# Dreycey/PhageFilter

Measured on AMD Instinct MI355X. Metric: reads/sec classified (150 bp, 1024-leaf SBT) at 1/2/4/8 MI355X; bit-exact vs CPU, higher is better.
Workload: dtype u64

## Files before the change

### include/pfq.h

```cpp
#ifndef PFQ_H
#define PFQ_H

#include <stdint.h>

#ifdef __cplusplus
extern "C" {
#endif

typedef enum pfq_status {
    PFQ_OK = 0,
    PFQ_ERR_ARG = -1,
    PFQ_ERR_IO = -2,
    PFQ_ERR_FORMAT = -3,
    PFQ_ERR_UNSUPPORTED = -4,
    PFQ_ERR_DEVICE = -5,
    PFQ_ERR_STATE = -6
} pfq_status;

typedef struct pfq_tree pfq_tree;

typedef struct pfq_info {
    uint64_t kmer_size;
    uint64_t nbits;
    uint32_t num_hashes;
// ... 157 lines not shown
                     float threshold, uint32_t flags, pfq_segments *out);
int pfq_query_frames_device(pfq_tree *tree, const uint8_t *d_seq, const uint64_t *d_offsets, uint64_t n_seqs, uint64_t total_bytes,
                            uint32_t frame, uint32_t step, float threshold, uint32_t flags, void *stream, pfq_segments *out);

#define PFQ_TEXT_FASTA 0
#define PFQ_TEXT_FASTQ 1
#define PFQ_TEXT_FINAL 1u
#define PFQ_TEXT_WANT_RECORDS 2u
enum { PFQ_TEXT_END = 0, PFQ_TEXT_LIMIT = 1, PFQ_TEXT_MORE = 2, PFQ_TEXT_SLOW = 3 };
typedef struct pfq_text {
    uint64_t n_records;
    uint64_t consumed;
    uint64_t n_bases;
    uint32_t stop;
    const uint64_t *rec_begin;
} pfq_text;
int pfq_text_parse(pfq_tree *tree, const uint8_t *text, uint64_t len, uint64_t limit, int format, uint32_t flags, pfq_text *out);
int pfq_text_query(pfq_tree *tree, float threshold, uint32_t flags, pfq_hits *hits);
int pfq_debug_text_csr(pfq_tree *tree, uint8_t *seq_out, uint64_t *off_out);

#define PFQ_PREP_PAIRED 1u
#define PFQ_PREP_WANT_READS 2u
enum { PFQ_PREP_KEPT = 0, PFQ_PREP_SHORT = 1, PFQ_PREP_N = 2, PFQ_PREP_COMPLEXITY = 3, PFQ_PREP_MATE = 4 };
typedef struct pfq_prep_params {
    uint32_t trim_quality;
    uint32_t trim_window;
    uint32_t poly_x;
    uint32_t min_length;
    uint32_t max_n;
    uint32_t min_complexity;
    uint32_t flags;
} pfq_prep_params;
typedef struct pfq_prep {
    uint64_t n_reads, n_kept, bases_in, bases_kept, n_trimmed;
    uint64_t n_reason[5];
    const uint32_t *begin, *len, *reason;
    const uint32_t *kept;
} pfq_prep;
int pfq_prep_reads(pfq_tree *tree, const uint8_t *seq, const uint8_t *qual, const uint64_t *offsets, const uint8_t *has_qual,
                   uint64_t n_reads, const pfq_prep_params *params, pfq_prep *out);
int pfq_prep_query(pfq_tree *tree, float threshold, uint32_t flags, pfq_hits *hits);
int pfq_debug_prep_csr(pfq_tree *tree, uint8_t *seq_out, uint64_t *off_out);
int pfq_debug_last_prep(pfq_tree *tree, double *ms);

typedef struct pfq_similarity {
    uint64_t n_a, n_b;
    const uint32_t *shared_bits;
    const uint64_t *bits_a, *bits_b;
    const double *kmers_a, *kmers_b;
    const double *shared_kmers, *jaccard;
} pfq_similarity;
int pfq_tree_similarity(pfq_tree *a, const uint32_t *leaves_a, uint64_t n_a,
                        pfq_tree *b, const uint32_t *leaves_b, uint64_t n_b, pfq_similarity *out);

int pfq_tree_recluster(pfq_tree *src, pfq_tree **out);
typedef struct pfq_merge {
    uint32_t node, left, right, round, n_leaves, pad_;
    uint64_t score_sum, pairs;
} pfq_merge;
int pfq_tree_merges(pfq_tree *tree, const pfq_merge **merges, uint64_t *n, uint32_t *rounds);

int pfq_leaf_counts(pfq_tree *tree, const char *const **tax_ids, const uint64_t **counts, uint64_t *n_leaves);
int pfq_save_leaf_counts(pfq_tree *tree, const char *csv_path);

int pfq_leaf_counts_export(pfq_tree *tree, uint64_t *d_dst, void *stream);
int pfq_leaf_counts_import(pfq_tree *tree, const uint64_t *d_src, void *stream);
int pfq_leaf_counts_reset(pfq_tree *tree);
int pfq_leaf_counts_export_delta(pfq_tree *tree, uint64_t *d_dst, void *stream);
int pfq_leaf_counts_import_delta(pfq_tree *tree, const uint64_t *d_src, void *stream);

int pfq_device_count(int *n);

int pfq_trees_allreduce_counts(pfq_tree *const *trees, uint32_t n_trees);
uint32_t pfq_last_allreduce_ranks(void);


int pfq_set_option(pfq_tree *tree, const char *name, const char *value);

#define PFQ_CAPACITY_N 12
int pfq_debug_last_capacity(pfq_tree *tree, uint64_t *out, uint64_t n);

int pfq_tile_lists_info(pfq_tree *tree, uint64_t out[4]);
int pfq_debug_tile_list(pfq_tree *tree, uint64_t col, uint64_t tile, uint32_t *out, uint64_t n);


typedef struct pfq_stats {
    uint64_t n_reads, n_candidates, n_hits, n_allhit_reads;
    uint64_t algorithmic_bytes;
    uint32_t path;
    uint32_t n_slices;
    uint32_t tile_mode;
    uint32_t n_fallback_pairs;
    uint64_t n_chunks, tile_entries;
    uint32_t tile_passes_launched, tile_passes_needed;
    uint32_t leaf_groups;
    uint32_t coarse_cols;
    uint32_t coarse_probes;
    uint32_t tile_bin_build;
    uint64_t group_reads;
    uint32_t pair_stage;
} pfq_stats;
int pfq_last_stats(pfq_tree *tree, pfq_stats *out);
int pfq_set_path(pfq_tree *tree, int path);

typedef struct pfq_profile {
    uint64_t calls;
    double classify_ms;
    double bucket_ms;
    double bin_ms;
    double test_ms;
    double verify_ms;
    double finalize_ms;
} pfq_profile;
int pfq_profile_begin(pfq_tree *tree, uint32_t max_calls);
int pfq_profile_end(pfq_tree *tree, pfq_profile *out);

int pfq_debug_kmer_indices(pfq_tree *tree, const uint8_t *seq, uint64_t len, uint64_t *out_idx, uint64_t *n_kmers);
int pfq_debug_last_similarity(pfq_tree *a, double *kernel_ms, uint32_t *slices);
int pfq_debug_last_recluster(pfq_tree *src, double *ms, uint64_t *nn_bytes, uint32_t *rounds);
int pfq_debug_node_filter(pfq_tree *tree, uint64_t node, uint64_t *out_words, uint64_t n_words);

int pfq_synth_genomes_device(uint8_t *d_out, uint64_t n_genomes, uint64_t genome_len, uint64_t seed_base,
                             void *stream);
int pfq_synth_reads_device(uint8_t *d_out, uint64_t first_read, uint64_t n_reads, uint64_t read_len,
                           const uint8_t *d_genomes, uint64_t genome_len, uint64_t n_genomes, uint64_t seed,
                           void *stream);

int pfq_host_alloc(uint64_t bytes, void **out);
int pfq_host_free(void *p);

const char *pfq_last_error(void);
const char *pfq_version(void);

#ifdef __cplusplus
}
#endif
#endif
```

### phagefilter_amd/_ffi.py

```python
from __future__ import annotations

import ctypes as C
import os

_HERE = os.path.dirname(os.path.abspath(__file__))
LIB_PATH = os.environ.get("PFQ_LIBPFQ") or os.path.join(_HERE, "libpfq.so")

SYMBOLS = [
    "pfq_tree_open", "pfq_tree_open_subtree", "pfq_db_shard_count", "pfq_tree_create", "pfq_tree_insert", "pfq_tree_build_balanced", "pfq_tree_build_balanced_device",
    "pfq_tree_build_balanced_subtree_device", "pfq_trees_allreduce_counts", "pfq_last_allreduce_ranks", "pfq_device_count", "pfq_set_option", "pfq_tree_save", "pfq_tree_info",
    "pfq_tree_prune", "pfq_tree_close", "pfq_query_batch", "pfq_query_batch_device", "pfq_last_hit_scores", "pfq_leaf_counts",
    "pfq_tree_clades", "pfq_clade_counts", "pfq_last_lca",
    "pfq_tree_set_taxonomy", "pfq_tree_taxa", "pfq_taxon_counts", "pfq_last_taxa", "pfq_last_best_rows", "pfq_db_leaf_ids", "pfq_taxonomy_read", "pfq_taxonomy_nodes",
    "pfq_abundance_estimate", "pfq_abundance_reset", "pfq_abundance_absorb",
    "pfq_coverage_get", "pfq_coverage_reset", "pfq_coverage_absorb",
    "pfq_tree_set_sweep", "pfq_sweep_get", "pfq_sweep_reset", "pfq_sweep_absorb",
    "pfq_query_frames", "pfq_query_frames_device",
    "pfq_text_parse", "pfq_text_query", "pfq_debug_text_csr",
    "pfq_prep_reads", "pfq_prep_query", "pfq_debug_prep_csr", "pfq_debug_last_prep",
    "pfq_tree_similarity", "pfq_tree_recluster", "pfq_tree_merges",
    "pfq_save_leaf_counts", "pfq_leaf_counts_export", "pfq_leaf_counts_import", "pfq_leaf_counts_reset",
    "pfq_leaf_counts_export_delta", "pfq_leaf_counts_import_delta",
    "pfq_last_stats", "pfq_set_path", "pfq_profile_begin", "pfq_profile_end", "pfq_debug_kmer_indices", "pfq_debug_node_filter", "pfq_debug_last_capacity", "pfq_debug_last_similarity", "pfq_debug_last_recluster",
    "pfq_tile_lists_info", "pfq_debug_tile_list",
    "pfq_synth_genomes_device",
    "pfq_synth_reads_device", "pfq_host_alloc", "pfq_host_free", "pfq_last_error", "pfq_version",
]


class PfqError(RuntimeError):
    def __init__(self, code: int, msg: str):
        super().__init__(f"libpfq error {code}: {msg}")
        self.code = code


class Info(C.Structure):
    _fields_ = [("kmer_size", C.c_uint64), ("nbits", C.c_uint64), ("num_hashes", C.c_uint32),
                ("largest_expected_genome", C.c_uint32), ("false_pos_rate", C.c_float),
                ("superset_verified", C.c_uint32), ("seed1", C.c_uint64), ("seed2", C.c_uint64),
                ("n_nodes", C.c_uint64), ("n_leaves", C.c_uint64), ("n_filters", C.c_uint64),
                ("device_bytes", C.c_uint64), ("shard_first_leaf", C.c_uint64), ("tree_leaves", C.c_uint64)]


class Hits(C.Structure):
    _fields_ = [("n_reads", C.c_uint64), ("offsets", C.POINTER(C.c_uint64)), ("leaves", C.POINTER(C.c_uint32))]


class Stats(C.Structure):
    _fields_ = [("n_reads", C.c_uint64), ("n_candidates", C.c_uint64), ("n_hits", C.c_uint64),
                ("n_allhit_reads", C.c_uint64), ("algorithmic_bytes", C.c_uint64), ("path", C.c_uint32),
                ("n_slices", C.c_uint32), ("tile_mode", C.c_uint32), ("n_fallback_pairs", C.c_uint32),
                ("n_chunks", C.c_uint64), ("tile_entries", C.c_uint64), ("tile_passes_launched", C.c_uint32),
                ("tile_passes_needed", C.c_uint32), ("leaf_groups", C.c_uint32), ("coarse_cols", C.c_uint32),
                ("coarse_probes", C.c_uint32), ("tile_bin_build", C.c_uint32), ("group_reads", C.c_uint64),
                ("pair_stage", C.c_uint32)]


class Profile(C.Structure):
    _fields_ = [("calls", C.c_uint64), ("classify_ms", C.c_double), ("bucket_ms", C.c_double), ("bin_ms", C.c_double),
                ("test_ms", C.c_double), ("verify_ms", C.c_double), ("finalize_ms", C.c_double)]


class Clade(C.Structure):
    _fields_ = [("parent", C.c_uint32), ("depth", C.c_uint32), ("first_leaf", C.c_uint32), ("n_leaves", C.c_uint32),
                ("name", C.c_char_p)]


class Taxon(C.Structure):
    _fields_ = [("parent", C.c_uint32), ("depth", C.c_uint32), ("first_rank", C.c_uint32), ("n_leaves", C.c_uint32),
                ("leaf", C.c_uint32), ("name", C.c_char_p)]


class TaxonomyFile(C.Structure):
    _fields_ = [("n_taxa", C.c_uint64), ("taxon_parent", C.POINTER(C.c_uint32)), ("taxon_names", C.POINTER(C.c_char_p)),
                ("n_leaves", C.c_uint64), ("leaf_taxon", C.POINTER(C.c_uint32)), ("lines_considered", C.c_uint64),
                ("lines_other", C.c_uint64), ("leaves_without_line", C.c_uint64)]


class Abundance(C.Structure):
    _fields_ = [("n_leaves", C.c_uint64), ("mass", C.POINTER(C.c_uint64)), ("unique", C.POINTER(C.c_uint64)),
                ("n_units", C.c_uint64), ("n_unhit", C.c_uint64), ("n_unique", C.c_uint64), ("n_ambiguous", C.c_uint64),
                ("n_all_leaves", C.c_uint64), ("n_entries", C.c_uint64), ("last_delta", C.c_uint64),
                ("iterations", C.c_uint32), ("converged", C.c_uint32)]


class Coverage(C.Structure):
    _fields_ = [("n_leaves", C.c_uint64), ("n_units", C.c_uint64), ("precision", C.c_uint32),
                ("registers", C.POINTER(C.c_uint8)),
                ("units", C.POINTER(C.c_uint64)), ("matched", C.POINTER(C.c_uint64)), ("filter_bits", C.POINTER(C.c_uint64)),
                ("distinct", C.POINTER(C.c_double)), ("genome_kmers", C.POINTER(C.c_double))]


class Sweep(C.Structure):
    _fields_ = [("n_thresholds", C.c_uint32), ("thresholds", C.POINTER(C.c_float)), ("n_leaves", C.c_uint64), ("n_units", C.c_uint64),
                ("leaf_units", C.POINTER(C.c_uint64)), ("leaf_unique", C.POINTER(C.c_uint64)),
                ("units_hit", C.POINTER(C.c_uint64)), ("units_unique", C.POINTER(C.c_uint64)), ("entries", C.POINTER(C.c_uint64)),
                ("genomes_hit", C.POINTER(C.c_uint64))]


class Segment(C.Structure):
    _fields_ = [(f, C.c_uint32) for f in ("leaf", "first_frame", "n_frames", "begin", "end", "match_begin", "match_end", "kmers",
                                          "matched", "longest_run")]


class Segments(C.Structure):
    _fields_ = [("n_seqs", C.c_uint64), ("n_frames", C.c_uint64), ("offsets", C.POINTER(C.c_uint64)), ("seg", C.POINTER(Segment))]


class Text(C.Structure):
    _fields_ = [("n_records", C.c_uint64), ("consumed", C.c_uint64), ("n_bases", C.c_uint64), ("stop", C.c_uint32),
                ("rec_begin", C.POINTER(C.c_uint64))]


class PrepParams(C.Structure):
    _fields_ = [(f, C.c_uint32) for f in ("trim_quality", "trim_window", "poly_x", "min_length", "max_n", "min_complexity", "flags")]


class Prep(C.Structure):
    _fields_ = [("n_reads", C.c_uint64), ("n_kept", C.c_uint64), ("bases_in", C.c_uint64), ("bases_kept", C.c_uint64),
                ("n_trimmed", C.c_uint64), ("n_reason", C.c_uint64 * 5),
                ("begin", C.POINTER(C.c_uint32)), ("len", C.POINTER(C.c_uint32)), ("reason", C.POINTER(C.c_uint32)),
                ("kept", C.POINTER(C.c_uint32))]


class Similarity(C.Structure):
    _fields_ = [("n_a", C.c_uint64), ("n_b", C.c_uint64), ("shared_bits", C.POINTER(C.c_uint32)),
                ("bits_a", C.POINTER(C.c_uint64)), ("bits_b", C.POINTER(C.c_uint64)),
                ("kmers_a", C.POINTER(C.c_double)), ("kmers_b", C.POINTER(C.c_double)),
                ("shared_kmers", C.POINTER(C.c_double)), ("jaccard", C.POINTER(C.c_double))]


class Merge(C.Structure):
    _fields_ = [("node", C.c_uint32), ("left", C.c_uint32), ("right", C.c_uint32), ("round", C.c_uint32), ("n_leaves", C.c_uint32),
                ("pad_", C.c_uint32), ("score_sum", C.c_uint64), ("pairs", C.c_uint64)]


WANT_HITS = 1
WANT_SCORES = 2
# ... 31 lines not shown
    L.pfq_version.restype = C.c_char_p
    L.pfq_tree_open.argtypes = [C.c_char_p, C.c_int, C.POINTER(vp)]
    L.pfq_tree_open_subtree.argtypes = [C.c_char_p, C.c_int, C.c_uint64, C.c_uint64, C.POINTER(vp)]
    L.pfq_db_shard_count.argtypes = [C.c_char_p, C.c_uint64, u64p]
    L.pfq_tree_build_balanced.argtypes = [vp, vp, C.c_uint64, C.POINTER(C.c_char_p), C.c_uint64, C.c_uint64,
                                          C.c_uint32, C.c_uint64, C.c_uint64, C.c_float, C.c_uint32, C.c_int,
                                          C.POINTER(vp)]
    L.pfq_tree_build_balanced_device.argtypes = [vp, C.c_uint64, C.c_uint64, C.POINTER(C.c_char_p), C.c_uint64,
                                                 C.c_uint64, C.c_uint32, C.c_uint64, C.c_uint64, C.c_float, C.c_uint32,
                                                 C.c_int, C.POINTER(vp)]
    L.pfq_tree_build_balanced_subtree_device.argtypes = [vp, C.c_uint64, C.c_uint64, C.POINTER(C.c_char_p), C.c_uint64,
                                                         C.c_uint64, C.c_uint32, C.c_uint64, C.c_uint64, C.c_float, C.c_uint32,
                                                         C.c_uint64, C.c_uint64, C.c_int, C.POINTER(vp)]
    L.pfq_trees_allreduce_counts.argtypes = [C.POINTER(vp), C.c_uint32]
    L.pfq_last_allreduce_ranks.restype = C.c_uint32
    L.pfq_set_option.argtypes = [vp, C.c_char_p, C.c_char_p]
    L.pfq_tree_create.argtypes = [C.c_uint64, C.c_float, C.c_uint32, C.c_uint64, C.c_uint64, C.c_uint64, C.c_int, C.POINTER(vp)]
    L.pfq_tree_insert.argtypes = [vp, vp, C.c_uint64, C.c_char_p, C.c_char_p]
    L.pfq_host_alloc.argtypes = [C.c_uint64, C.POINTER(vp)]
    L.pfq_host_free.argtypes = [vp]
    L.pfq_tree_save.argtypes = [vp, C.c_char_p]
    L.pfq_tree_info.argtypes = [vp, C.POINTER(Info)]
    L.pfq_tree_prune.argtypes = [vp, C.c_uint64]
    L.pfq_tree_close.argtypes = [vp]
    L.pfq_tree_close.restype = None
    L.pfq_query_batch.argtypes = [vp, vp, vp, C.c_uint64, C.c_float, C.c_uint32, C.POINTER(Hits)]
    L.pfq_query_batch_device.argtypes = [vp, vp, vp, C.c_uint64, C.c_uint64, C.c_float, C.c_uint32, vp, C.POINTER(Hits)]
    L.pfq_last_hit_scores.argtypes = [vp, C.POINTER(C.POINTER(C.c_uint32)), u64p]
    L.pfq_tree_clades.argtypes = [vp, C.POINTER(C.POINTER(Clade)), u64p]
    L.pfq_clade_counts.argtypes = [vp, C.POINTER(u64p), C.POINTER(u64p), u64p]
    L.pfq_last_lca.argtypes = [vp, C.POINTER(C.POINTER(C.c_uint32)), u64p]
    u32p = C.POINTER(C.c_uint32)
    L.pfq_tree_set_taxonomy.argtypes = [vp, C.c_uint64, vp, C.POINTER(C.c_char_p), vp]
    L.pfq_tree_taxa.argtypes = [vp, C.POINTER(C.POINTER(Taxon)), u64p]
    L.pfq_taxon_counts.argtypes = [vp, C.POINTER(u64p), C.POINTER(u64p), C.POINTER(u64p), u64p]
    L.pfq_last_taxa.argtypes = [vp, C.POINTER(u32p), u64p]
    L.pfq_last_best_rows.argtypes = [vp, C.POINTER(Hits)]
    L.pfq_db_leaf_ids.argtypes = [C.c_char_p, C.POINTER(C.POINTER(C.c_char_p)), u64p]
    L.pfq_taxonomy_read.argtypes = [C.c_char_p, C.POINTER(C.c_char_p), C.c_uint64, C.POINTER(TaxonomyFile)]
    L.pfq_taxonomy_nodes.argtypes = [C.c_uint64, C.POINTER(C.c_char_p), C.c_uint64, vp, C.POINTER(C.c_char_p), vp,
                                     C.POINTER(C.POINTER(Taxon)), u64p]
    L.pfq_abundance_estimate.argtypes = [vp, C.c_uint32, C.c_uint64, C.POINTER(Abundance)]
    L.pfq_abundance_reset.argtypes = [vp]
    L.pfq_abundance_absorb.argtypes = [vp, vp]
    L.pfq_coverage_get.argtypes = [vp, C.POINTER(Coverage)]
    L.pfq_coverage_reset.argtypes = [vp]
    L.pfq_coverage_absorb.argtypes = [vp, vp]
    L.pfq_tree_set_sweep.argtypes = [vp, C.POINTER(C.c_float), C.c_uint32]
    L.pfq_sweep_get.argtypes = [vp, C.POINTER(Sweep)]
    L.pfq_sweep_reset.argtypes = [vp]
    L.pfq_sweep_absorb.argtypes = [vp, vp]
    L.pfq_query_frames.argtypes = [vp, vp, vp, C.c_uint64, C.c_uint32, C.c_uint32, C.c_float, C.c_uint32, C.POINTER(Segments)]
    L.pfq_query_frames_device.argtypes = [vp, vp, vp, C.c_uint64, C.c_uint64, C.c_uint32, C.c_uint32, C.c_float, C.c_uint32, vp,
                                          C.POINTER(Segments)]
    L.pfq_text_parse.argtypes = [vp, vp, C.c_uint64, C.c_uint64, C.c_int, C.c_uint32, C.POINTER(Text)]
    L.pfq_text_query.argtypes = [vp, C.c_float, C.c_uint32, C.POINTER(Hits)]
    L.pfq_debug_text_csr.argtypes = [vp, vp, vp]
    L.pfq_prep_reads.argtypes = [vp, vp, vp, vp, vp, C.c_uint64, C.POINTER(PrepParams), C.POINTER(Prep)]
    L.pfq_prep_query.argtypes = [vp, C.c_float, C.c_uint32, C.POINTER(Hits)]
    L.pfq_debug_prep_csr.argtypes = [vp, vp, vp]
    L.pfq_debug_last_prep.argtypes = [vp, C.POINTER(C.c_double)]
    L.pfq_tree_similarity.argtypes = [vp, vp, C.c_uint64, vp, vp, C.c_uint64, C.POINTER(Similarity)]
    L.pfq_debug_last_similarity.argtypes = [vp, C.POINTER(C.c_double), C.POINTER(C.c_uint32)]
    L.pfq_tree_recluster.argtypes = [vp, C.POINTER(vp)]
    L.pfq_tree_merges.argtypes = [vp, C.POINTER(C.POINTER(Merge)), u64p, C.POINTER(C.c_uint32)]
    L.pfq_debug_last_recluster.argtypes = [vp, C.POINTER(C.c_double), u64p, C.POINTER(C.c_uint32)]
    L.pfq_leaf_counts.argtypes = [vp, C.POINTER(C.POINTER(C.c_char_p)), C.POINTER(u64p), u64p]
    L.pfq_save_leaf_counts.argtypes = [vp, C.c_char_p]
    L.pfq_leaf_counts_export.argtypes = [vp, vp, vp]
    L.pfq_leaf_counts_import.argtypes = [vp, vp, vp]
    L.pfq_leaf_counts_export_delta.argtypes = [vp, vp, vp]
    L.pfq_leaf_counts_import_delta.argtypes = [vp, vp, vp]
    L.pfq_leaf_counts_reset.argtypes = [vp]
    L.pfq_last_stats.argtypes = [vp, C.POINTER(Stats)]
    L.pfq_set_path.argtypes = [vp, C.c_int]
    L.pfq_profile_begin.argtypes = [vp, C.c_uint32]
    L.pfq_profile_end.argtypes = [vp, C.POINTER(Profile)]
    L.pfq_debug_kmer_indices.argtypes = [vp, vp, C.c_uint64, vp, u64p]
    L.pfq_debug_node_filter.argtypes = [vp, C.c_uint64, vp, C.c_uint64]
    L.pfq_debug_last_capacity.argtypes = [vp, vp, C.c_uint64]
    if hasattr(L, "pfq_tile_lists_info"):
        L.pfq_tile_lists_info.argtypes = [vp, vp]
        L.pfq_debug_tile_list.argtypes = [vp, C.c_uint64, C.c_uint64, vp, C.c_uint64]
    L.pfq_synth_genomes_device.argtypes = [vp, C.c_uint64, C.c_uint64, C.c_uint64, vp]
    L.pfq_synth_reads_device.argtypes = [vp, C.c_uint64, C.c_uint64, C.c_uint64, vp, C.c_uint64, C.c_uint64,
                                         C.c_uint64, vp]
    _lib = L
    return L


def check(rc: int) -> None:
    if rc != 0:
        raise PfqError(rc, lib().pfq_last_error().decode(errors="replace"))


def source_stamp() -> str:
    import glob
    import hashlib
    h = hashlib.sha256()
    csrc = os.path.join(_HERE, "csrc")
    files = sorted(glob.glob(os.path.join(csrc, "*.hip")) + glob.glob(os.path.join(csrc, "*.cpp")) +
                   glob.glob(os.path.join(csrc, "*.h")) + [os.path.join(os.path.dirname(_HERE), "include", "pfq.h")])
    for f in files:
        h.update(os.path.basename(f).encode())
        with open(f, "rb") as fh:
            h.update(fh.read())
    return h.hexdigest()[:16]
```

### phagefilter_amd/csrc/pfq_host.cpp

```cpp
#include <hip/hip_runtime.h>
#include <rccl/rccl.h>
#include <dlfcn.h>

#include <algorithm>
#include <thread>
#include <mutex>
#include <atomic>
#include <cerrno>
#include <cmath>
#include <cstdio>
#include <cstring>
#include <fstream>
#include <map>
#include <memory>
#include <string>
#include <unordered_set>
#include <vector>

#include "../../include/pfq.h"
#include "pfq_kernels.h"
#include "pfq_taxonomy.h"

namespace {

thread_local std::string g_err;
int fail(int code, const std::string &msg) {
    g_err = msg;
    return code;
}
#define HIP_TRY(expr)                                                                                        \
    do {                                                                                                     \
        hipError_t e_ = (expr);                                                                              \
        if (e_ != hipSuccess)                                                                                \
            return fail(PFQ_ERR_DEVICE, std::string(#expr) + ": " + hipGetErrorString(e_) + " (" __FILE__ ":" + \
                                            std::to_string(__LINE__) + ")");                                 \
    } while (0)
#define PFQ_TRY(expr)              \
    do {                           \
        int rc_ = (expr);          \
        if (rc_ != PFQ_OK) return rc_; \
    } while (0)

struct Node {
    int32_t left = -1, right = -1, parent = -1;
    std::string bf_path;
    bool has_tax = false;
    std::string tax_id;
    uint64_t mapped_reads = 0;
    uint64_t base_reads = 0;
    uint32_t filter = 0;
    uint32_t depth = 0;
    bool is_leaf() const { return left < 0 && right < 0; }
};

template <typename T>
struct DevBuf {
    T *p = nullptr;
    size_t n = 0;
    ~DevBuf() { release(); }
    void release() {
        if (p) (void)hipFree(p);
        p = nullptr;
        n = 0;
    }
    hipError_t ensure(size_t want) {
        if (want <= n) return hipSuccess;
        release();
        hipError_t e = hipMalloc(&p, want * sizeof(T));
        if (e == hipSuccess) n = want;
        return e;
    }
    size_t bytes() const { return n * sizeof(T); }
};
template <typename T>
struct HostBuf {
    T *p = nullptr;
    size_t cap = 0;
    ~HostBuf() { if (p) (void)hipHostFree(p); }
    hipError_t ensure(size_t want) {
        const size_t bytes = want * sizeof(T), grown = bytes + bytes / 4 + 4096;
        if (bytes <= cap) return hipSuccess;
        if (p) (void)hipHostFree(p);
        p = nullptr;
        cap = 0;
        hipError_t e = hipHostMalloc((void **)&p, grown, hipHostMallocDefault);
        if (e == hipSuccess) cap = grown;
        return e;
    }
};

struct Knobs {
    long long record_gb = -1, tile_gb = -1, tile_entries = -1, slice_kb = -1;
    long long verify_blocks = -1, verify_chunk = -1, verify_sub = -1, verify_threads = -1, bin_blocks = -1, test_blocks = -1;
    long long tile = -1, tile_counts = -1, no_tail_batch = -1, split_records = -1, bin_narrow = -1, bin_wide = -1, bin_debug = -1, block = -1, batch_emit = -1;
    long long coarse = -1, coarse_cols = -1, coarse_probes = -1, group_log2 = -1, screen_recs = -1, coarse_min_leaves = -1, greedy_host = -1;
    long long pair_slots = -1, guard_slots = -1, miss_words = -1, kmiss_bytes = -1, hit_slots = -1;
    long long abund_slots = -1, abund_blocks = -1, abund_lds = -1;
    long long cover_p = -1, cover_blocks = -1;
    long long frame_piece = -1;
    long long sim_slices = -1, sim_naive = -1, sim_time = -1;
    long long cluster_time = -1;
    long long text_tile = -1;
    long long sweep_lds = -1;
    long long tile_lists = -1;
    long long tile_stream = -1;
};
struct KnobName {
    const char *name;
    long long Knobs::*field;
};
const KnobName KNOBS[] = {
    {"PFQ_RECORD_GB", &Knobs::record_gb},       {"PFQ_TILE_GB", &Knobs::tile_gb},
    {"PFQ_TILE_ENTRIES", &Knobs::tile_entries}, {"PFQ_SLICE_KB", &Knobs::slice_kb},
    {"PFQ_VERIFY_BLOCKS", &Knobs::verify_blocks}, {"PFQ_VERIFY_CHUNK", &Knobs::verify_chunk},
    {"PFQ_VERIFY_SUB", &Knobs::verify_sub},     {"PFQ_VERIFY_THREADS", &Knobs::verify_threads},
    {"PFQ_BIN_BLOCKS", &Knobs::bin_blocks},     {"PFQ_TEST_BLOCKS", &Knobs::test_blocks},
    {"PFQ_TILE", &Knobs::tile},                 {"PFQ_TILE_COUNTS", &Knobs::tile_counts},
    {"PFQ_NO_TAIL_BATCH", &Knobs::no_tail_batch}, {"PFQ_BIN_NARROW", &Knobs::bin_narrow},
    {"PFQ_BIN_WIDE", &Knobs::bin_wide},         {"PFQ_SPLIT_RECORDS", &Knobs::split_records},
#ifdef PFQ_EXPERIMENTS
    {"PFQ_BIN_DEBUG", &Knobs::bin_debug},
#endif
    {"PFQ_BLOCK", &Knobs::block},               {"PFQ_BATCH_EMIT", &Knobs::batch_emit},
    {"PFQ_COARSE", &Knobs::coarse},             {"PFQ_COARSE_COLS", &Knobs::coarse_cols},
    {"PFQ_COARSE_PROBES", &Knobs::coarse_probes}, {"PFQ_GROUP_LOG2", &Knobs::group_log2},
    {"PFQ_SCREEN_RECS", &Knobs::screen_recs},   {"PFQ_COARSE_MIN_LEAVES", &Knobs::coarse_min_leaves},
    {"PFQ_GREEDY_HOST", &Knobs::greedy_host},
    {"PFQ_PAIR_SLOTS", &Knobs::pair_slots},     {"PFQ_GUARD_SLOTS", &Knobs::guard_slots},
    {"PFQ_MISS_WORDS", &Knobs::miss_words},     {"PFQ_KMISS_BYTES", &Knobs::kmiss_bytes},
    {"PFQ_HIT_SLOTS", &Knobs::hit_slots},
    {"PFQ_ABUND_SLOTS", &Knobs::abund_slots},   {"PFQ_ABUND_BLOCKS", &Knobs::abund_blocks},
    {"PFQ_ABUND_LDS", &Knobs::abund_lds},
    {"PFQ_COVER_P", &Knobs::cover_p},           {"PFQ_COVER_BLOCKS", &Knobs::cover_blocks},
    {"PFQ_FRAME_PIECE", &Knobs::frame_piece},
    {"PFQ_SIM_SLICES", &Knobs::sim_slices},     {"PFQ_SIM_NAIVE", &Knobs::sim_naive},
    {"PFQ_SIM_TIME", &Knobs::sim_time},         {"PFQ_CLUSTER_TIME", &Knobs::cluster_time},
    {"PFQ_TEXT_TILE", &Knobs::text_tile},       {"PFQ_SWEEP_LDS", &Knobs::sweep_lds},
    {"PFQ_TILE_LISTS", &Knobs::tile_lists},     {"PFQ_TILE_STREAM", &Knobs::tile_stream},
};
bool set_knob(Knobs &k, const char *name, const char *value) {
    for (const KnobName &kn : KNOBS)
        if (!strcmp(kn.name, name)) {
            k.*(kn.field) = (value && *value) ? strtoll(value, nullptr, 10) : -1;
            return true;
        }
    return false;
}
Knobs knobs_from_env() {
    Knobs k;
    for (const KnobName &kn : KNOBS)
        if (const char *e = getenv(kn.name)) set_knob(k, kn.name, e);
    return k;
}

}

namespace {
std::atomic<long> g_open_trees{0};
void release_communicators();
}

enum CursorSlot {
    CUR_HIT = 0,
    CUR_PAIR = 1,
    CUR_TILE_ENTRIES = 2,
    CUR_CHUNKS_FLAGGED = 3,
    CUR_LONG = 4,
    CUR_MISS_WORDS = 5,
    CUR_DIRTY = 6,
    CUR_OPEN = 7,
    CUR_GUARD = 8,
    CUR_KMISS = 9,
    CUR_TAIL_SHAPES = 10,
    CUR_TAIL_WORK = 11,
    CUR_TILE_LIST = 12,
    CUR_TILE_DENSE = 13,
    CUR_N = 14,
    CUR_ALLOC = 16,
};
static_assert(CUR_N <= CUR_ALLOC, "an attempt clears CUR_ALLOC slots");
static_assert(CUR_HIT == 0 && CUR_PAIR == 1, "read_hits reads slots 0 and 1 with one 16-byte copy");
static_assert(CUR_TAIL_WORK == CUR_TAIL_SHAPES + 1, "k_tail_records finds its work counter at shapes[2]");
static_assert(CUR_TILE_DENSE == CUR_TILE_LIST + 1, "k_tile_test finds its dense counter at tile_list_stats[1]");
enum HintSlot {
    HINT_PAIRS = 0,
    HINT_TILE_ENTRIES = 1,
    HINT_DIRTY = 2,
    HINT_SORTED = 3,
    HINT_CANDIDATES = 4,
    HINT_PLAN = 5,
    HINT_N = 8,
};
static_assert(CUR_TILE_ENTRIES == CUR_PAIR + 1 && HINT_TILE_ENTRIES == HINT_PAIRS + 1, "one 16-byte copy fills both hints");

struct pfq_tree {
    pfq_tree() { ++g_open_trees; }
    pfq_tree(const pfq_tree &) = delete;
    ~pfq_tree() {
        if (--g_open_trees == 0) release_communicators();
    }
    int device = 0;
    Knobs knobs = knobs_from_env();
    std::vector<Node> nodes;
    int32_t root = -1;
    float false_pos_rate = 0.001f;
    uint32_t largest_expected_genome = 0;
    uint64_t kmer_size = 0, nbits = 0, seed1 = 0, seed2 = 0, n_words = 0;
    uint32_t num_hashes = 0;
    std::vector<std::string> filter_paths;
    std::unordered_set<std::string> path_set;
    std::vector<uint8_t> edge_ok;
    bool superset_all = true;
    uint64_t shard_first_leaf = 0, tree_leaves = 0;
    bool is_shard = false;
    unsigned long long *h_pair_cursor = nullptr;
    hipEvent_t hint_ev = nullptr;
    uint64_t hint_reads = 0, hint_entry_cap = 0, passes_hint = 1;
    double pairs_per_read = 1.0, hits_per_read = 1.0;
    double dirty_frac = 1.0;
    bool hint_counts = false;
    uint32_t last_sub_log2 = 0;
    bool topology_dirty = false;
    uint64_t internal_counter = 0;
    size_t n_rows = 0, row_capacity = 0;
    DevBuf<uint32_t> d_build;
    DevBuf<unsigned long long> d_dist;
    DevBuf<pfq::TopoNode> d_topo;
    DevBuf<int> d_walk;
    bool topo_on_device = false;
    bool topo_pending = false;
    DevBuf<uint8_t> d_gseq[4];
    hipEvent_t gseq_free[4] = {nullptr, nullptr, nullptr, nullptr};
    hipEvent_t gseq_copied[4] = {nullptr, nullptr, nullptr, nullptr};
    uint8_t *h_gseq[4] = {nullptr, nullptr, nullptr, nullptr};
    size_t h_gseq_n[4] = {0, 0, 0, 0};
    uint32_t gseq_next = 0;
    int greedy_blocks = 0;
    uint32_t walk_seq = 0;
    int insert_err = PFQ_OK;
    std::string insert_err_msg;

    pfq::HashParams hp{};
    DevBuf<uint64_t> d_bits;
    bool layout_valid = false;
    std::vector<int32_t> leaves;
    std::vector<uint32_t> col_row;
    std::vector<uint32_t> guard_off, guard_col;
    uint32_t rw = 1, rw_log2 = 0, n_cols = 0;
    uint64_t leaf_cap = 0, guard_cap = 0;
    uint32_t n_groups = 1;
    uint32_t group_log2 = 11;
    uint64_t group_stride = 0;
    bool coarse_valid = false;
    uint32_t coarse_cols = 0, coarse_rw = 0, coarse_rw_log2 = 0;
    double coarse_fill = 0.0;
    DevBuf<uint32_t> d_Sc, d_cgrp, d_glists, d_glong;
    DevBuf<unsigned int> d_gcur;
    uint32_t last_coarse_cols = 0, last_coarse_probes = 0, last_leaf_groups = 0;
    DevBuf<uint32_t> d_S, d_col_row, d_guard_off, d_guard_col;
    DevBuf<uint32_t> d_tile_list_row, d_tile_lists;
    uint32_t tile_list_cols = 0;
    void drop_tile_lists() {
        d_tile_list_row.release();
        d_tile_lists.release();
        tile_list_cols = 0;
    }
    DevBuf<uint32_t> d_owner, d_owner_sorted, d_gfail;
    DevBuf<unsigned long long> d_counts;
    DevBuf<unsigned long long> d_counts_base, d_counts_delta;
    DevBuf<unsigned long long> d_stats, d_cursors;
    unsigned int *cur_lo(CursorSlot s) const { return reinterpret_cast<unsigned int *>(d_cursors.p + s); }
    unsigned int *cur_hi(CursorSlot s) const { return cur_lo(s) + 1; }
    DevBuf<uint32_t> d_entries, d_pair_chunk, d_leaf_chunk0, d_flag_list;
    DevBuf<pfq::ChunkDesc> d_chunks;
    DevBuf<unsigned int> d_gfill, d_binq;
    DevBuf<uint8_t> d_kmiss;
    DevBuf<uint8_t> d_kall;
    DevBuf<uint8_t> d_T, d_failb;
    bool tables_valid = false;
    double cand_per_read = 1.0;
    bool have_cand_hint = false;
    uint32_t last_block_mode = 0;
    DevBuf<uint32_t> d_round_k0, d_n_rounds, d_pair_kpos;
    uint32_t last_tile_mode = 0, last_passes = 1;
    uint32_t last_sort = 0;
    bool last_tile_stream = false;
    uint32_t last_tile_bin = 0;
    DevBuf<uint2> d_hit_pairs, d_pairs, d_sorted;
    DevBuf<uint32_t> d_bucket, d_fail;
    DevBuf<unsigned int> d_queue;
    DevBuf<uint8_t> d_allhit, d_seq, d_seq2;
    DevBuf<uint64_t> d_off2;
    hipStream_t copy_stream = nullptr;
    hipEvent_t in_free[2] = {nullptr, nullptr};
    bool in_used[2] = {false, false};
    int in_slot = 0;
    DevBuf<unsigned long long> d_miss_words;
    DevBuf<uint32_t> d_miss_pos, d_bucket_w;
    DevBuf<uint32_t> d_long;
    DevBuf<uint4> d_recs;
    DevBuf<uint4> d_meta;
    DevBuf<uint64_t> d_off;
    DevBuf<unsigned long long> d_counts_snapshot;
    hipStream_t last_stream = nullptr;
    bool have_last_stream = false;
    hipEvent_t last_done = nullptr;
    int force_path = -1;
    std::vector<hipEvent_t> prof_ev;
    size_t prof_cap = 0, prof_used = 0;
    std::vector<uint8_t> prof_bucketed;
    uint32_t last_path = 0, last_slices = 1;
    uint64_t last_n_reads = 0;
    uint64_t last_pair_cap = 0, last_guard_cap = 0, last_miss_cap = 0, last_kmiss_cap = 0, last_hit_cap0 = 0, last_hit_cursor0 = 0;
    uint64_t last_nb = 0;
    uint32_t last_attempts = 0;
    std::vector<std::string> out_tax;
    std::vector<const char *> out_tax_ptr;
    std::vector<uint64_t> out_counts;
    DevBuf<uint32_t> d_hit_cnt, d_hit_leaves;
    DevBuf<unsigned long long> d_hit_sums, d_hit_off;
    HostBuf<uint64_t> h_hit_off;
    HostBuf<uint32_t> h_hit_leaves;
    DevBuf<uint32_t> d_hit_scores;
    HostBuf<uint32_t> h_hit_scores;
    bool scores_valid = false;
    uint64_t scores_n = 0;
    DevBuf<unsigned long long> d_pair_sink, d_frag_off, d_pair_misc;
    DevBuf<uint32_t> d_frag_leaves, d_pair_long;
    bool lca_valid = false;
    std::vector<pfq_clade> clades;
    std::vector<std::string> clade_names;
    uint32_t top_clade = 0;
    DevBuf<uint32_t> d_leaf_clade, d_gap_min, d_lca, d_lca_long;
    DevBuf<unsigned long long> d_clade_here, d_lca_misc;
    DevBuf<uint2> d_lca_span;
    std::vector<uint64_t> out_here, out_below;
    DevBuf<unsigned long long> d_ab_start, d_ab_unique, d_ab_cur, d_ab_a, d_ab_b, d_ab_delta;
    DevBuf<uint32_t> d_ab_len, d_ab_entries;
    uint64_t ab_rows = 0, ab_entries = 0, ab_units = 0, ab_unhit = 0, ab_unique = 0, ab_all = 0;
    bool ab_incomplete = false;
    std::vector<uint64_t> out_mass, out_unique;
    DevBuf<uint8_t> d_cov_regs;
    DevBuf<unsigned long long> d_cov_cnt;
    uint32_t cov_p = 0;
    uint64_t cov_units = 0;
    bool cov_bits_valid = false;
    std::vector<uint64_t> cov_bits, out_cov_units, out_cov_matched;
    std::vector<uint8_t> out_cov_regs;
    std::vector<double> out_cov_distinct, out_cov_genome;
    DevBuf<uint32_t> d_fr_cnt, d_fr_def, d_fr_seq, d_fr_start, d_fr_segseq, d_fr_queue;
    DevBuf<unsigned long long> d_fr_seq0, d_fr_defoff, d_fr_sums, d_fr_segpos, d_fr_seqseg, d_fr_pieceoff, d_fr_misc;
    DevBuf<uint64_t> d_fr_foff;
    DevBuf<uint8_t> d_fr_bytes;
    DevBuf<pfq::Segment> d_fr_segs;
    DevBuf<pfq::FramePart> d_fr_parts;
    HostBuf<uint64_t> h_fr_off;
    HostBuf<pfq_segment> h_fr_segs;
    std::vector<uint32_t> out_sim_shared;
    std::vector<uint64_t> out_sim_bits_a, out_sim_bits_b;
    std::vector<double> out_sim_kmers_a, out_sim_kmers_b, out_sim_shared_kmers, out_sim_jaccard;
    float sim_kernel_ms = 0.0f;
    uint32_t sim_slices = 0;
    std::vector<pfq_merge> merges;
    uint32_t merge_rounds = 0;
    float cluster_ms[3] = {0.0f, 0.0f, 0.0f};
    uint64_t cluster_nn_bytes = 0;
// ... 1241 lines not shown
                t.tables_valid = true;
            }
            HIP_TRY(hipMemsetAsync(t.d_failb.p, 0, t.d_failb.n, st));
        }
        return PFQ_OK;
    }
    int guards_and_tails() {
        ga = pfq::GuardArgs{};
        if (guard_pairs) {
            ga.pairs = t.d_pairs.p + t.leaf_cap;
            ga.cap = t.guard_cap;
            if (kn.guard_slots >= 0) ga.cap = std::min<uint64_t>(ga.cap, (uint64_t)kn.guard_slots);
            t.last_guard_cap = ga.cap;
            ga.cursor = t.d_cursors.p + CUR_GUARD;
            ga.slot0 = (uint32_t)t.leaf_cap;
            ga.owner = t.d_owner.p;
            ga.gfail = t.d_gfail.p;
            pfq::launch_expand_guards(a, ga, 2048, st);
        }
        if (a.batch_tails || a.split_recs) pfq::launch_tail_records(a, t.cur_lo(CUR_TAIL_SHAPES), 2048, st);
        if (ev) HIP_TRY(hipEventRecord(ev[1], st));
        return PFQ_OK;
    }
    int bucket_sort() {
        pfq::launch_bucket_scan(cnt, off, cur, (uint32_t)nb, st);
        if (pair_miss) pfq::launch_bucket_scan(cntw, offw, curw, (uint32_t)nb, st);
        t.last_sort = pfq::launch_bucket_scatter(t.d_pairs.p, t.d_cursors.p + CUR_PAIR, a.pair_cap, off, cur, (uint32_t)nb, sub_log2, t.d_sorted.p,
                                                 recs ? t.d_meta.p : nullptr, d_off, block_mode ? nullptr : t.d_col_row.p, offw, curw,
                                                 pair_miss ? t.d_miss_pos.p : nullptr, (uint32_t)t.kmer_size,
                                                 guard_pairs ? t.d_owner.p : nullptr, guard_pairs ? t.d_owner_sorted.p : nullptr,
                                                 block_mode ? 2u : 0u, st);
        if (guard_pairs)
            pfq::launch_bucket_scatter(ga.pairs, ga.cursor, ga.cap, off, cur, (uint32_t)nb, sub_log2, t.d_sorted.p,
                                       recs ? t.d_meta.p : nullptr, d_off, t.d_col_row.p, offw, curw,
                                       counts_mode ? t.d_miss_pos.p : nullptr, (uint32_t)t.kmer_size,
                                       t.d_owner.p + t.leaf_cap, t.d_owner_sorted.p, 0u, st);
        if (ev) HIP_TRY(hipEventRecord(ev[2], st));
        return PFQ_OK;
    }
    int setup_verify() {
        v = pfq::VerifyArgs{};
        v.hp = t.hp;
        v.seq = d_seq;
        v.off = d_off;
        v.bits = t.d_bits.p;
        v.col_row = t.d_col_row.p;
        v.n_words = t.n_words;
        v.sorted = t.d_sorted.p;
        v.n_pairs_ptr = off + nb;
        v.fail = t.d_fail.p;
        v.recs = recs;
        v.miss_words = pair_miss ? t.d_miss_words.p : nullptr;
        v.miss_pos = pair_miss ? t.d_miss_pos.p : nullptr;
        v.meta = t.d_meta.p;
        v.n_slices = n_slices;
        uint64_t sb = (t.n_words * 64 + n_slices - 1) / n_slices;
        v.slice_bits = (uint32_t)((sb + 63) & ~63ull);
        v.queue = t.d_queue.p;
        vblocks = 512;
        v.chunk = 1;
        if (kn.verify_blocks >= 0) vblocks = std::max(8, (int)kn.verify_blocks & ~7);
        if (kn.verify_chunk >= 0) v.chunk = (uint32_t)std::max(1, (int)kn.verify_chunk);
        v.n_sub = 8;
        if (kn.verify_sub >= 0) v.n_sub = (uint32_t)std::min(16, std::max(1, (int)kn.verify_sub));
        vthreads = 512;
        if (kn.verify_threads >= 0) vthreads = std::min(1024, std::max(64, (int)kn.verify_threads & ~63));
        if (!recs) { vthreads = 256; vblocks = 1024; v.chunk = 4; }
        return PFQ_OK;
    }
    int tile_stage() {
        const uint32_t tile_log2 = block_mode ? pfq::TILE_LOG2_BLOCK : (counts_mode ? pfq::TILE_LOG2_COUNTS : pfq::TILE_LOG2);
        const uint32_t n_tiles = (uint32_t)((t.n_words * 64 + (1ull << tile_log2) - 1) >> tile_log2);
        const uint32_t chunk_log2 = pfq::CHUNK_PAIRS_LOG2;
        bool tile_counts = true;
        if (kn.tile_counts >= 0) tile_counts = kn.tile_counts != 0;
        bool tile_mode = recs && (!counts_mode || tile_counts) && (block_mode || n_tiles < 256);
        if (kn.tile >= 0) tile_mode = tile_mode && kn.tile != 0;
        if (hipMemGetInfo(&mem_free, &mem_total) != hipSuccess) { (void)hipGetLastError(); mem_free = 0; }
        uint64_t tile_budget = std::min<uint64_t>(64ull << 30, (uint64_t)((double)(mem_free + t.d_entries.bytes()) * 0.8));
        if (kn.tile_gb >= 0) tile_budget = (uint64_t)kn.tile_gb << 30;
        t.last_tile_mode = 0;
        t.last_tile_bin = 0;
        t.last_tile_stream = false;
        if (tile_mode) {
            const uint64_t max_chunks = nc + ((t.leaf_cap + t.guard_cap) >> chunk_log2) + 2;
            uint64_t want = (uint64_t)((double)total_bytes * t.num_hashes * 1.13 * std::max(1.0, t.pairs_per_read)) +
                            max_chunks * n_tiles * 544ull;
            if (want * 4 > tile_budget) want = tile_budget / 4;
            if (kn.tile_entries >= 0) want = std::max<uint64_t>(1, (uint64_t)kn.tile_entries);
            uint64_t kmiss_cap = counts_mode ? std::min<uint64_t>(((uint64_t)((double)total_bytes * std::max(1.0, 1.3 * t.pairs_per_read)) + 16 * max_chunks + 64) * (block_mode ? 8u : 1u),
                                                                      block_mode ? (48ull << 30) : 0xfffffff0ull) & ~15ull : 0;
            if (counts_mode && kn.kmiss_bytes >= 0) kmiss_cap = std::min<uint64_t>(kmiss_cap, (uint64_t)kn.kmiss_bytes & ~15ull);
            bool ok = soft_ensure(t.d_entries, want) && soft_ensure(t.d_pair_chunk, t.d_pairs.n) && soft_ensure(t.d_flag_list, t.d_pairs.n) &&
                      soft_ensure(t.d_leaf_chunk0, nc + 1) && soft_ensure(t.d_chunks, max_chunks) && soft_ensure(t.d_gfill, max_chunks * n_tiles) && soft_ensure(t.d_binq, 256);
            if (ok && counts_mode)
                ok = soft_ensure(t.d_kmiss, kmiss_cap) && soft_ensure(t.d_round_k0, max_chunks * pfq::MAX_ROUNDS) &&
                     soft_ensure(t.d_n_rounds, max_chunks) && soft_ensure(t.d_pair_kpos, t.d_pairs.n);
            if (ok && counts_mode && block_mode) ok = soft_ensure(t.d_kall, (kmiss_cap >> 3) + 64);
            if (!ok) {
                tile_mode = false;
            } else {
                HIP_TRY(hipMemsetAsync(t.d_gfill.p, 0, max_chunks * n_tiles * 4, st));
                HIP_TRY(hipMemsetAsync(t.d_binq.p, 0, 256 * 4, st));
                pfq::TileArgs ta{};
                ta.hp = t.hp;
                ta.bits = t.d_bits.p;
                ta.n_words = t.n_words;
                ta.chunk_log2 = chunk_log2;
                if (block_mode) {
                    ta.blocks = 1;
                    if (counts_mode) ta.kall = t.d_kall.p;
                    ta.bits = reinterpret_cast<const uint64_t *>(t.d_T.p);
                    ta.n_words = t.n_words * 8;
                    ta.failb = t.d_failb.p;
                }
                ta.recs = recs;
                ta.meta = t.d_meta.p;
                ta.col_row = t.d_col_row.p;
                ta.bucket_off = off;
                ta.sub_log2 = sub_log2;
                ta.n_leaves = (uint32_t)(block_mode ? n_blocks : nc);
                ta.n_tiles = n_tiles;
                ta.chunks = t.d_chunks.p;
                ta.max_chunks = (uint32_t)max_chunks;
                ta.leaf_chunk0 = t.d_leaf_chunk0.p;
                ta.pair_chunk = t.d_pair_chunk.p;
                ta.n_chunks = t.cur_lo(CUR_CHUNKS_FLAGGED);
                ta.n_flagged = t.cur_hi(CUR_CHUNKS_FLAGGED);
                ta.flag_list = t.d_flag_list.p;
                ta.flag_cap = (uint32_t)std::min<uint64_t>(t.d_flag_list.n, 0xffffffffu);
                ta.entry_cursor = t.d_cursors.p + CUR_TILE_ENTRIES;
                ta.entry_cap = std::min<uint64_t>(want, t.d_entries.n) & ~31ull;
                ta.entries = t.d_entries.p;
                ta.gfill = t.d_gfill.p;
                ta.fail = t.d_fail.p;
                ta.n_pairs_ptr = off + nb;
                if (!counts_mode && !block_mode) {
                    ta.tile_list_stats = t.d_cursors.p + CUR_TILE_LIST;
                    if (t.tile_list_cols && kn.tile_lists != 0) {
                        ta.tile_list_row = t.d_tile_list_row.p;
                        ta.tile_lists = t.d_tile_lists.p;
                        ta.tile_stream = t.tile_list_cols == t.n_cols && kn.tile_stream != 0;
                    }
                }
                if (counts_mode) {
                    ta.counts = 1;
                    ta.threshold = threshold;
                    ta.kmiss = t.d_kmiss.p;
                    ta.kmiss_cap = kmiss_cap;
                    t.last_kmiss_cap = kmiss_cap;
                    ta.kmiss_used = t.d_cursors.p + CUR_KMISS;
                    ta.round_k0 = t.d_round_k0.p;
                    ta.n_rounds = t.d_n_rounds.p;
                    ta.pair_kpos = t.d_pair_kpos.p;
                    HIP_TRY(hipMemsetAsync(t.d_n_rounds.p, 0, max_chunks * 4, st));
                }
                int bin_blocks = 512, test_blocks = 512;
                if (kn.bin_blocks >= 0) bin_blocks = std::max(1, (int)kn.bin_blocks);
                if (kn.test_blocks >= 0) test_blocks = std::max(1, (int)kn.test_blocks);
                ta.bin_shape = kn.bin_narrow > 0 ? (uint32_t)kn.bin_narrow : (kn.bin_wide > 0 ? 2u : 0u);
                ta.debug = kn.bin_debug > 0 ? (uint32_t)kn.bin_debug : 0u;
                pfq::launch_tile_plan(ta, st);
                uint64_t n_passes = std::min<uint64_t>(std::max<uint64_t>(1, t.passes_hint), 256);
                if (block_mode) {
                    HIP_TRY(hipMemcpyAsync(t.h_pair_cursor + HINT_PLAN, t.d_cursors.p + CUR_TILE_ENTRIES, 8, hipMemcpyDeviceToHost, st));
                    HIP_TRY(hipStreamSynchronize(st));
                    n_passes = ta.entry_cap ? std::min<uint64_t>(std::max<uint64_t>(1, (t.h_pair_cursor[HINT_PLAN] + ta.entry_cap - 1) / ta.entry_cap), 256) : 1;
                }
                for (uint64_t p = 0; p < n_passes; ++p) {
                    ta.pass = (uint32_t)p;
                    ta.bin_queue = t.d_binq.p + p;
                    t.last_tile_bin = pfq::launch_tile_bin(ta, bin_blocks, st);
                    if (p == 0 && ev) HIP_TRY(hipEventRecord(ev[3], st));
                    pfq::launch_tile_test(ta, test_blocks, st);
                    t.last_tile_stream = ta.tile_stream != 0;
                }
                v.pair_chunk = t.d_pair_chunk.p;
                v.chunks = t.d_chunks.p;
                v.entry_cursor = t.d_cursors.p + CUR_TILE_ENTRIES;
                v.entry_cap = ta.entry_cap;
                v.launched_passes = (uint32_t)n_passes;
                if (pair_miss) {
                    pfq::FinalizeArgs pf{};
                    pf.hp = t.hp;
                    pf.threshold = threshold;
                    pf.fail = t.d_fail.p;
                    binned_miss(pf, (uint32_t)n_passes);
                    pfq::launch_prefix_open(pf, t.d_meta.p, off + nb, t.d_fail.p, st);
                }
                t.hint_entry_cap = ta.entry_cap;
                t.last_passes = (uint32_t)std::max<uint64_t>(n_passes, 1);
                if (ev) HIP_TRY(hipEventRecord(ev[4], st));
                v.only_flagged = 1;
                v.n_flagged = ta.n_flagged;
                v.flag_list = t.d_flag_list.p;
                v.flag_cap = ta.flag_cap;
                t.last_tile_mode = 1;
            }
        }
        if (ev && !t.last_tile_mode) {
            HIP_TRY(hipEventRecord(ev[3], st));
            HIP_TRY(hipEventRecord(ev[4], st));
        }
        return PFQ_OK;
    }
    void binned_miss(pfq::FinalizeArgs &f, uint32_t launched_passes) const {
        f.kmiss = t.d_kmiss.p;
        f.pair_kpos = t.d_pair_kpos.p;
        f.pair_chunk = t.d_pair_chunk.p;
        f.chunks = t.d_chunks.p;
        f.launched_passes = launched_passes;
    }
    pfq::FinalizeArgs finalize_args() const {
        pfq::FinalizeArgs f{};
        f.hp = t.hp;
        f.off = d_off;
        f.sorted = t.d_sorted.p;
        f.bucket_off = off;
        f.sub_log2 = sub_log2;
        f.threshold = threshold;
        f.counts = count_dst();
        f.hit_pairs = a.hit_pairs;
        f.hit_cap = hit_cap;
        f.hit_cursor = t.d_cursors.p + CUR_HIT;
        f.stats = t.d_stats.p;
        return f;
    }
    int finish_blocks() {
        a.S = t.d_S.p;
        a.col0 = 0;
        a.n_leaves = (uint32_t)std::min<size_t>(2048, nl);
        if (counts_mode && t.last_tile_mode) {
            pfq::FinalizeArgs cf{};
            cf.hp = t.hp;
            cf.off = d_off;
            cf.sorted = t.d_sorted.p;
            cf.threshold = threshold;
            cf.fail = t.d_fail.p;
            cf.kall = t.d_kall.p;
            binned_miss(cf, v.launched_passes);
            pfq::launch_block_count(cf, off + nb, t.d_failb.p, st);
        }
        pfq::launch_block_fallback(a, t.d_sorted.p, off + nb, t.d_fail.p, t.d_failb.p, t.d_pair_chunk.p,
                                   t.last_tile_mode ? t.d_chunks.p : nullptr, v.launched_passes,
                                   t.last_tile_mode ? v.n_flagged : nullptr, t.last_tile_mode ? v.flag_list : nullptr, v.flag_cap, st);
        if (with_guards) pfq::launch_block_guards(a, t.d_sorted.p, off + nb, t.d_failb.p, st);
        if (ev) HIP_TRY(hipEventRecord(ev[5], st));
        pfq::FinalizeArgs f = finalize_args();
        f.failb = t.d_failb.p;
        f.c0 = 0;
        f.c1 = (uint32_t)nc;
        pfq::launch_finalize(f, st);
        if (ev) HIP_TRY(hipEventRecord(ev[6], st));
        t.last_block_mode = 1;
        if (t.last_tile_mode) t.last_tile_mode = 2;
        t.hint_counts = false;
        return PFQ_OK;
    }
    int finish_pairs() {
// ... 2732 lines not shown
            const ncclResult_t rc0 = r.CommInitAll(fresh.data(), (int)devs.size(), devs.data());
            if (rc0 != ncclSuccess) return fail(PFQ_ERR_DEVICE, std::string("ncclCommInitAll: ") + r.GetErrorString(rc0));
            it = comm_cache.emplace(devs, std::move(fresh)).first;
        }
        std::vector<ncclComm_t> &comms = it->second;
        ncclResult_t rc = r.GroupStart();
        for (size_t i = 0; i < devs.size() && rc == ncclSuccess; ++i) {
            (void)hipSetDevice(devs[i]);
            unsigned long long *buf = by_dev[devs[i]][0]->d_counts_delta.p;
            rc = r.AllReduce(buf, buf, nl, ncclUint64, ncclSum, comms[i], nullptr);
        }
        const ncclResult_t rc_end = r.GroupEnd();
        if (rc == ncclSuccess) rc = rc_end;
        hipError_t he = hipSuccess;
        for (size_t i = 0; i < devs.size(); ++i) {
            (void)hipSetDevice(devs[i]);
            const hipError_t e = hipDeviceSynchronize();
            if (he == hipSuccess) he = e;
        }
        if (rc != ncclSuccess || he != hipSuccess) {
            for (auto c : comms) (void)r.CommDestroy(c);
            comm_cache.erase(it);
        }
        if (rc != ncclSuccess) return fail(PFQ_ERR_DEVICE, std::string("ncclAllReduce: ") + r.GetErrorString(rc));
        if (he != hipSuccess) return fail(PFQ_ERR_DEVICE, std::string("all-reduce of the leaf counters: ") + hipGetErrorString(he));
        g_last_ranks = (uint32_t)devs.size();
    }
    for (auto &kv : by_dev) {
        HIP_TRY(hipSetDevice(kv.first));
        const unsigned long long *total = kv.second[0]->d_counts_delta.p;
        for (size_t q = 0; q < kv.second.size(); ++q) {
            pfq_tree &t = *kv.second[q];
            pfq::launch_counts_op(t.d_counts.p, t.d_counts_base.p, total, nl, false, nullptr);
            HIP_TRY(hipMemcpyAsync(t.d_counts_base.p, t.d_counts.p, (size_t)nl * 8, hipMemcpyDeviceToDevice, nullptr));
        }
        HIP_TRY(hipGetLastError());
        HIP_TRY(hipDeviceSynchronize());
    }
    return PFQ_OK;
}

int pfq_leaf_counts_reset(pfq_tree *tree) {
    if (!tree) return fail(PFQ_ERR_ARG, "null argument");
    PFQ_TRY(use_device(tree->device));
    PFQ_TRY(build_layout(*tree));
    HIP_TRY(hipDeviceSynchronize());
    if (!tree->leaves.empty()) {
        HIP_TRY(hipMemset(tree->d_counts.p, 0, tree->leaves.size() * 8));
        HIP_TRY(hipMemset(tree->d_counts_base.p, 0, tree->leaves.size() * 8));
        if (tree->lca_valid) HIP_TRY(hipMemset(tree->d_clade_here.p, 0, tree->clades.size() * 8));
        PFQ_TRY(tax_zero(*tree));
    }
    for (auto &nd : tree->nodes) nd.mapped_reads = nd.base_reads = 0;
    abund_clear(*tree);
    cover_clear(*tree);
    PFQ_TRY(sweep_zero(*tree));
    return PFQ_OK;
}

int pfq_last_stats(pfq_tree *tree, pfq_stats *out) {
    if (!tree || !out) return fail(PFQ_ERR_ARG, "null argument");
    PFQ_TRY(use_device(tree->device));
    pfq_tree &t = *tree;
    memset(out, 0, sizeof *out);
    if (!t.d_stats.p) return PFQ_OK;
    PFQ_TRY(wait_last_call(t));
    unsigned long long h[pfq::ST_N];
    HIP_TRY(hipMemcpy(h, t.d_stats.p, sizeof h, hipMemcpyDeviceToHost));
    out->n_reads = t.last_n_reads;
    out->n_candidates = h[pfq::ST_CANDIDATES];
    out->n_hits = h[pfq::ST_HITS];
    out->n_allhit_reads = h[pfq::ST_ALLHIT];
    out->algorithmic_bytes = h[pfq::ST_ALG_BYTES];
    out->path = t.last_path;
    out->n_slices = t.last_slices;
    out->tile_mode = t.last_tile_mode;
    out->tile_bin_build = t.last_tile_bin;
    if (t.d_cursors.p) {
        unsigned long long c[CUR_TAIL_SHAPES + 1];
        HIP_TRY(hipMemcpy(c, t.d_cursors.p, sizeof c, hipMemcpyDeviceToHost));
        const uint32_t shapes = t.last_path ? (uint32_t)c[CUR_TAIL_SHAPES] : 0u;
        out->pair_stage = t.last_sort | ((shapes & 7u) << 4) | ((shapes & pfq::TAIL_SHAPE_FULL) ? 4u : 0u) |
                          ((t.last_path && h[pfq::ST_BATCHED]) ? 8u : 0u) | ((t.last_path && t.last_tile_mode && t.last_tile_stream) ? 0x80u : 0u);
        out->n_chunks = (uint32_t)c[CUR_CHUNKS_FLAGGED];
        out->n_fallback_pairs = (uint32_t)(c[CUR_CHUNKS_FLAGGED] >> 32);
        out->tile_entries = c[CUR_TILE_ENTRIES];
        if (t.last_tile_mode && t.hint_entry_cap) {
            out->tile_passes_launched = t.last_passes;
            out->tile_passes_needed = (uint32_t)std::max<uint64_t>(1, (c[CUR_TILE_ENTRIES] + t.hint_entry_cap - 1) / t.hint_entry_cap);
        }
    }
    out->leaf_groups = t.last_leaf_groups;
    out->coarse_cols = t.last_coarse_cols;
    out->coarse_probes = t.last_coarse_probes;
    out->group_reads = h[pfq::ST_LISTED];
    return PFQ_OK;
}
int pfq_profile_begin(pfq_tree *tree, uint32_t max_calls) {
    if (!tree) return fail(PFQ_ERR_ARG, "null argument");
    PFQ_TRY(use_device(tree->device));
    pfq_tree &t = *tree;
    while (t.prof_ev.size() < PROF_EV * (size_t)max_calls) {
        hipEvent_t e;
        HIP_TRY(hipEventCreate(&e));
        t.prof_ev.push_back(e);
    }
    t.prof_cap = max_calls;
    t.prof_used = 0;
    t.prof_bucketed.assign(max_calls, 0);
    return PFQ_OK;
}
int pfq_profile_end(pfq_tree *tree, pfq_profile *out) {
    if (!tree || !out) return fail(PFQ_ERR_ARG, "null argument");
    PFQ_TRY(use_device(tree->device));
    pfq_tree &t = *tree;
    memset(out, 0, sizeof *out);
    PFQ_TRY(wait_last_call(t));
    for (size_t c = 0; c < t.prof_used; ++c) {
        hipEvent_t *ev = &t.prof_ev[PROF_EV * c];
        float ms = 0;
        HIP_TRY(hipEventElapsedTime(&ms, ev[0], ev[1]));
        out->classify_ms += ms;
        if (t.prof_bucketed[c]) {
            HIP_TRY(hipEventElapsedTime(&ms, ev[1], ev[2]));
            out->bucket_ms += ms;
            HIP_TRY(hipEventElapsedTime(&ms, ev[2], ev[3]));
            out->bin_ms += ms;
            HIP_TRY(hipEventElapsedTime(&ms, ev[3], ev[4]));
            out->test_ms += ms;
            HIP_TRY(hipEventElapsedTime(&ms, ev[4], ev[5]));
            out->verify_ms += ms;
            HIP_TRY(hipEventElapsedTime(&ms, ev[5], ev[6]));
            out->finalize_ms += ms;
        }
    }
    out->calls = t.prof_used;
    t.prof_cap = t.prof_used = 0;
    return PFQ_OK;
}
int pfq_set_option(pfq_tree *tree, const char *name, const char *value) {
    if (!tree || !name) return fail(PFQ_ERR_ARG, "null argument");
    if (!strcmp(name, "PFQ_COVER_P")) {
        Knobs k = tree->knobs;
        set_knob(k, name, value);
        if (k.cover_p != -1 && (k.cover_p < (long long)pfq::COVER_P_MIN || k.cover_p > (long long)pfq::COVER_P_MAX))
            return fail(PFQ_ERR_ARG, std::string("PFQ_COVER_P must be 4..16, not ") + value);
        if (tree->d_cov_regs.p && cover_precision(k) != tree->cov_p) {
            if (tree->cov_units)
                return fail(PFQ_ERR_STATE, "PFQ_COVER_P cannot change while the coverage sketch holds units (precision " + std::to_string(tree->cov_p) +
                                           "); pfq_coverage_reset empties it");
            PFQ_TRY(use_device(tree->device));
            HIP_TRY(hipDeviceSynchronize());
            cover_clear(*tree);
        }
    }
    if (!strcmp(name, "PFQ_TEXT_TILE") && value && *value) {
        const long long v = strtoll(value, nullptr, 10);
        if (v < (long long)pfq::TEXT_TILE_MIN || v > (long long)pfq::TEXT_TILE_DEFAULT || (v & (v - 1)))
            return fail(PFQ_ERR_ARG, std::string("PFQ_TEXT_TILE must be a power of two from 256 to 8192, not ") + value);
    }
    if (!strcmp(name, "PFQ_FRAME_PIECE") && value && *value) {
        const long long v = strtoll(value, nullptr, 10);
        if (v <= 0 || v % 64 || v > (1ll << 30)) return fail(PFQ_ERR_ARG, std::string("PFQ_FRAME_PIECE must be a positive multiple of 64 up to 2^30, not ") + value);
    }
    if (!set_knob(tree->knobs, name, value)) return fail(PFQ_ERR_ARG, std::string("unknown option ") + name);
    if (!strcmp(name, "PFQ_COARSE") || !strcmp(name, "PFQ_COARSE_COLS") || !strcmp(name, "PFQ_GROUP_LOG2") || !strcmp(name, "PFQ_COARSE_MIN_LEAVES") ||
        !strcmp(name, "PFQ_TILE_LISTS")) {
        if (tree->layout_valid) {
            PFQ_TRY(use_device(tree->device));
            PFQ_TRY(sync_counts_to_nodes(*tree));
            tree->layout_valid = false;
            tree->drop_tile_lists();
        }
    }
    return PFQ_OK;
}
int pfq_set_path(pfq_tree *tree, int path) {
    if (!tree || path < -1 || path > 1) return fail(PFQ_ERR_ARG, "bad argument");
    tree->force_path = path;
    return PFQ_OK;
}

int pfq_debug_last_capacity(pfq_tree *tree, uint64_t *out, uint64_t n) {
    if (!tree || (n && !out)) return fail(PFQ_ERR_ARG, "null argument");
    PFQ_TRY(use_device(tree->device));
    pfq_tree &t = *tree;
    uint64_t v[PFQ_CAPACITY_N] = {};
    if (t.d_cursors.p) {
        PFQ_TRY(wait_last_call(t));
        unsigned long long c[CUR_KMISS + 1];
        HIP_TRY(hipMemcpy(c, t.d_cursors.p, sizeof c, hipMemcpyDeviceToHost));
        uint32_t sorted = 0;
        if (t.last_nb && t.d_bucket.n > 2 * t.last_nb) HIP_TRY(hipMemcpy(&sorted, t.d_bucket.p + 2 * t.last_nb, 4, hipMemcpyDeviceToHost));
        const uint64_t w[PFQ_CAPACITY_N] = {c[CUR_PAIR], t.last_pair_cap, c[CUR_GUARD], t.last_guard_cap, c[CUR_MISS_WORDS], t.last_miss_cap, c[CUR_KMISS], t.last_kmiss_cap,
                                            t.last_hit_cursor0, t.last_hit_cap0, t.last_attempts, sorted};
        if (t.last_path) memcpy(v, w, sizeof v);
        else v[8] = w[8], v[9] = w[9], v[10] = w[10];
    }
    for (uint64_t i = 0; i < n && i < PFQ_CAPACITY_N; ++i) out[i] = v[i];
    return PFQ_OK;
}

int pfq_tile_lists_info(pfq_tree *tree, uint64_t out[4]) {
    if (!tree || !out) return fail(PFQ_ERR_ARG, "null argument");
    PFQ_TRY(use_device(tree->device));
    pfq_tree &t = *tree;
    PFQ_TRY(build_layout(t));
    out[0] = t.tile_list_cols;
    out[1] = t.tile_list_cols ? t.d_tile_lists.bytes() : 0;
    out[2] = out[3] = 0;
    if (t.d_cursors.p) {
        PFQ_TRY(wait_last_call(t));
        unsigned long long c[2];
        HIP_TRY(hipMemcpy(c, t.d_cursors.p + CUR_TILE_LIST, sizeof c, hipMemcpyDeviceToHost));
        out[2] = c[0];
        out[3] = c[1];
    }
    return PFQ_OK;
}
int pfq_debug_tile_list(pfq_tree *tree, uint64_t col, uint64_t tile, uint32_t *out, uint64_t n) {
    if (!tree || (n && !out)) return fail(PFQ_ERR_ARG, "null argument");
    PFQ_TRY(use_device(tree->device));
    pfq_tree &t = *tree;
    PFQ_TRY(build_layout(t));
    const uint64_t n_tiles = (t.n_words * 64 + (1ull << pfq::TILE_LOG2) - 1) >> pfq::TILE_LOG2;
    if (col >= t.n_cols || tile >= n_tiles) return fail(PFQ_ERR_ARG, "column / tile out of range");
    uint32_t row = pfq::TILE_LIST_NONE;
    if (t.tile_list_cols) HIP_TRY(hipMemcpy(&row, t.d_tile_list_row.p + col, 4, hipMemcpyDeviceToHost));
    if (row == pfq::TILE_LIST_NONE) return fail(PFQ_ERR_STATE, "column " + std::to_string(col) + " has no position slots (its tiles are loaded dense)");
    HIP_TRY(hipMemcpy(out, t.d_tile_lists.p + (row * n_tiles + tile) * pfq::TILE_LIST_CAP, std::min<uint64_t>(n, pfq::TILE_LIST_CAP) * 4, hipMemcpyDeviceToHost));
    return PFQ_OK;
}

int pfq_debug_kmer_indices(pfq_tree *tree, const uint8_t *seq, uint64_t len, uint64_t *out_idx, uint64_t *n_kmers) {
    if (!tree || !n_kmers || (len && !seq)) return fail(PFQ_ERR_ARG, "null argument");
    PFQ_TRY(use_device(tree->device));
    pfq_tree &t = *tree;
    uint64_t n = (t.kmer_size >= 1 && len >= t.kmer_size) ? len - t.kmer_size + 1 : 0;
    *n_kmers = n;
    if (!n || !out_idx) return PFQ_OK;
    DevBuf<uint8_t> d_s;
    DevBuf<uint64_t> d_o;
    HIP_TRY(d_s.ensure(len + 16));
    HIP_TRY(d_o.ensure(n * t.num_hashes));
    HIP_TRY(hipMemcpy(d_s.p, seq, len, hipMemcpyHostToDevice));
    pfq::launch_debug_indices(t.hp, d_s.p, len, d_o.p, nullptr);
    HIP_TRY(hipGetLastError());
    HIP_TRY(hipMemcpy(out_idx, d_o.p, n * t.num_hashes * 8, hipMemcpyDeviceToHost));
    return PFQ_OK;
}

int pfq_debug_node_filter(pfq_tree *tree, uint64_t node, uint64_t *out_words, uint64_t n_words) {
    if (!tree || !out_words) return fail(PFQ_ERR_ARG, "null argument");
    PFQ_TRY(use_device(tree->device));
    PFQ_TRY(finish_topology(*tree));
    if (node >= tree->nodes.size() || n_words != tree->n_words) return fail(PFQ_ERR_ARG, "node / n_words out of range");
    HIP_TRY(hipMemcpy(out_words, tree->d_bits.p + (uint64_t)tree->nodes[node].filter * tree->n_words, n_words * 8,
                      hipMemcpyDeviceToHost));
    return PFQ_OK;
}

int pfq_synth_genomes_device(uint8_t *d_out, uint64_t n_genomes, uint64_t genome_len, uint64_t seed_base, void *stream) {
    if (!d_out) return fail(PFQ_ERR_ARG, "null argument");
    pfq::launch_synth_genomes(d_out, n_genomes, genome_len, seed_base, (hipStream_t)stream);
    HIP_TRY(hipGetLastError());
    return PFQ_OK;
}
int pfq_synth_reads_device(uint8_t *d_out, uint64_t first_read, uint64_t n_reads, uint64_t read_len, const uint8_t *d_genomes,
                           uint64_t genome_len, uint64_t n_genomes, uint64_t seed, void *stream) {
    if (!d_out) return fail(PFQ_ERR_ARG, "null argument");
    pfq::launch_synth_reads(d_out, first_read, n_reads, read_len, d_genomes, genome_len, n_genomes, seed, (hipStream_t)stream);
    HIP_TRY(hipGetLastError());
    return PFQ_OK;
}

}
```

### phagefilter_amd/csrc/pfq_kernels.h

```cpp
#pragma once
#include <hip/hip_runtime.h>
#include <stdint.h>

#include "pfq_device.h"

namespace pfq {

#ifdef PFQ_EXPERIMENTS
#define PFQ_DEBUG_BITS(a) ((a).debug)
#else
#define PFQ_DEBUG_BITS(a) 0u
#endif
constexpr uint32_t PAIR_RESERVE = 32, MISS_RESERVE = 256;
enum StatSlot { ST_CANDIDATES = 0, ST_HITS = 1, ST_ALLHIT = 2, ST_ALG_BYTES = 3, ST_DEFERRED = 4, ST_LISTED = 5 , ST_BATCHED = 6 , ST_N = 8 };

struct QueryArgs {
    HashParams hp;
    const uint8_t *seq;
    const uint64_t *off;
    uint64_t n_reads;
    float threshold;
    const uint32_t *S;
    const uint32_t *S_all;
    uint64_t group_stride;
// ... 46 lines not shown
    uint32_t list_cap;
    uint32_t n_probes;
    uint32_t scr_extra;
    uint32_t total_leaves;
};
void launch_coarse(const QueryArgs &a, const CoarseArgs &ca, bool counts_mode, int blocks, hipStream_t st);
void launch_row_popcount(const uint64_t *bits, uint64_t n_words, const uint32_t *d_rows, uint32_t n_rows, unsigned long long *d_out, hipStream_t st);

struct GuardArgs {
    uint2 *pairs;
    uint64_t cap;
    unsigned long long *cursor;
    uint32_t slot0;
    uint32_t *owner;
    uint32_t *gfail;
};
void launch_expand_guards(const QueryArgs &a, const GuardArgs &ga, int blocks, hipStream_t st);

struct ChunkDesc;
struct VerifyArgs {
    HashParams hp;
    const uint8_t *seq;
    const uint64_t *off;
    const uint64_t *bits;
    const uint32_t *col_row;
    uint64_t n_words;
    const uint2 *sorted;
    const uint4 *meta;
    const uint32_t *n_pairs_ptr;
    uint32_t *fail;
    uint32_t n_slices, slice_bits;
    unsigned int *queue;
    uint32_t n_sub;
    uint32_t only_flagged;
    uint32_t flag_cap;
    const uint32_t *pair_chunk;
    const struct ChunkDesc *chunks;
    const unsigned long long *entry_cursor;
    uint64_t entry_cap;
    uint32_t launched_passes;
    const unsigned int *n_flagged;
    const uint32_t *flag_list;
    const uint4 *recs;
    unsigned long long *miss_words;
    const uint32_t *miss_pos;
    uint32_t chunk;
};

struct FinalizeArgs {
    HashParams hp;
    const uint64_t *off;
    const uint2 *sorted;
    const uint32_t *bucket_off;
    uint32_t sub_log2;
    const uint32_t *fail;
    const unsigned long long *miss_words;
    const uint32_t *miss_pos;
    float threshold;
    uint32_t c0, c1;
    uint32_t guards;
    const uint32_t *owner_sorted;
    uint32_t *gfail;
    unsigned long long *counts;
    uint2 *hit_pairs;
    uint64_t hit_cap;
    unsigned long long *hit_cursor;
    unsigned long long *stats;
    unsigned long long *n_dirty;
    const uint8_t *failb;
    const uint8_t *kmiss;
    const uint8_t *kall;
    const uint32_t *pair_kpos;
    const uint32_t *pair_chunk;
    const ChunkDesc *chunks;
    uint32_t launched_passes;
};

constexpr uint32_t TILE_LOG2 = 20;
constexpr uint32_t CHUNK_PAIRS_LOG2 = 10;
constexpr uint32_t MAX_TILES = 1024;
constexpr uint32_t TILE_LOG2_COUNTS = 19;
constexpr uint32_t ROUND_KMERS_LOG2 = 11;
constexpr uint32_t MAX_ROUNDS = 256;
constexpr uint32_t TILE_LOG2_BLOCK = 17;
constexpr uint32_t BLOCK_LEAVES_LOG2 = 3;
struct ChunkDesc {
    uint32_t row;
    uint32_t first;
    uint32_t n;
    uint32_t cap;
    uint64_t base;
    uint32_t leaf;
    uint32_t pass;
    uint32_t kbase;
    uint32_t kwords;
    uint32_t mask;
    uint32_t pad_;
};
struct TileArgs {
    uint32_t pass;
    HashParams hp;
    const uint64_t *bits;
    uint64_t n_words;
    const uint4 *recs;
    const uint4 *meta;
    const uint32_t *col_row;
    const uint32_t *bucket_off;
    uint32_t sub_log2, n_leaves, n_tiles;
    uint32_t bin_shape;
    uint32_t debug;
    ChunkDesc *chunks;
    uint32_t max_chunks;
    uint32_t *leaf_chunk0;
    uint32_t *pair_chunk;
    unsigned int *n_chunks;
    unsigned long long *entry_cursor;
    uint64_t entry_cap;
    uint32_t *entries;
    unsigned int *gfill;
    unsigned int *bin_queue;
    uint32_t *fail;
    unsigned int *n_flagged;
    uint32_t *flag_list;
    uint32_t flag_cap;
    const uint32_t *n_pairs_ptr;
    uint32_t blocks;
    uint32_t chunk_log2;
    uint8_t *failb;
    float threshold;
    uint32_t counts;
    uint8_t *kmiss;
    uint64_t kmiss_cap;
    unsigned long long *kmiss_used;
    uint8_t *kall;
    uint32_t *round_k0;
    uint32_t *n_rounds;
    uint32_t *pair_kpos;
    const uint32_t *tile_list_row;
    const uint32_t *tile_lists;
    unsigned long long *tile_list_stats;
    uint32_t tile_stream;
};
constexpr uint32_t TILE_LIST_CAP = 8192;
constexpr uint32_t TILE_LIST_NONE = 0xffffffffu;
void launch_tile_list_count(const uint64_t *bits, uint64_t n_words, const uint32_t *col_row, uint32_t n_cols, uint32_t n_tiles, uint32_t *col_max,
                            hipStream_t st);
void launch_tile_list_fill(const uint64_t *bits, uint64_t n_words, const uint32_t *col_row, const uint32_t *list_cols, uint32_t n_list_cols, uint32_t n_tiles,
                           uint32_t *lists, hipStream_t st);
void launch_tile_plan(const TileArgs &a, hipStream_t st);
uint32_t launch_tile_bin(const TileArgs &a, int blocks, hipStream_t st);
void launch_tile_test(const TileArgs &a, int blocks, hipStream_t st);

void launch_classify(const QueryArgs &a, bool defer, bool counts_mode, int blocks, hipStream_t st);
constexpr uint32_t TAIL_SHAPE_4 = 1, TAIL_SHAPE_16 = 2, TAIL_SHAPE_32 = 4, TAIL_SHAPE_FULL = 8;
void launch_tail_records(const QueryArgs &a, unsigned int *shapes, int blocks, hipStream_t st);
void launch_bucket_scan(const uint32_t *bucket_cnt, uint32_t *bucket_off, uint32_t *bucket_cur, uint32_t n, hipStream_t st);
constexpr uint32_t SORT_SLICED = 1, SORT_PER_PAIR = 2;
uint32_t launch_bucket_scatter(const uint2 *pairs, const unsigned long long *n_pairs_ptr, uint64_t pair_cap,
                               const uint32_t *bucket_off, uint32_t *bucket_cur, uint32_t n_buckets, uint32_t sub_log2, uint2 *sorted,
                               uint4 *meta, const uint64_t *read_off, const uint32_t *col_row, const uint32_t *words_off,
                               uint32_t *words_cur, uint32_t *miss_pos, uint32_t kmer_size, const uint32_t *owner,
                               uint32_t *owner_sorted, uint32_t key_mode, hipStream_t st);
void launch_block_tables(const uint64_t *bits, uint64_t n_words, const uint32_t *d_col_row, uint32_t n_leaves, uint8_t *T, hipStream_t st);
void launch_block_fallback(const QueryArgs &a, const uint2 *sorted, const uint32_t *n_pairs_ptr, const uint32_t *fail, uint8_t *failb,
                           const uint32_t *pair_chunk, const ChunkDesc *chunks, uint32_t launched_passes, const unsigned int *n_flagged,
                           const uint32_t *flag_list, uint32_t flag_cap, hipStream_t st);
void launch_block_count(const FinalizeArgs &a, const uint32_t *n_pairs_ptr, uint8_t *failb, hipStream_t st);
void launch_block_guards(const QueryArgs &a, const uint2 *sorted, const uint32_t *n_pairs_ptr, uint8_t *failb, hipStream_t st);
void launch_verify(const VerifyArgs &a, int blocks, int threads, hipStream_t st);
void launch_collect_open(const uint32_t *fail, const uint32_t *n_pairs_ptr, uint32_t *list, uint32_t cap, unsigned int *n_out, hipStream_t st);
void launch_finalize(const FinalizeArgs &a, hipStream_t st);
void launch_prefix_open(const FinalizeArgs &a, const uint4 *meta, const uint32_t *n_pairs_ptr, uint32_t *fail, hipStream_t st);

void launch_insert(const HashParams &hp, const uint8_t *d_genomes, const uint64_t *d_goff, uint32_t n_genomes,
                   const uint32_t *d_leaf_row, uint64_t *bits, uint64_t n_words, hipStream_t st);
void launch_insert_one(const HashParams &hp, const uint8_t *d_genome, uint64_t len, uint32_t row, uint64_t *bits, uint64_t n_words, hipStream_t st);
struct TopoNode {
    int32_t left, right;
    uint32_t row;
    uint32_t pad_;
};
constexpr int GREEDY_MAX_BLOCKS = 256;
constexpr uint32_t GREEDY_SYNC_STRIDE = 4096, GREEDY_SYNC_LINES = 49;
void launch_greedy_insert(uint64_t *bits, uint64_t n_words, TopoNode *topo, int *state, unsigned long long *sync, int leaf_node, int internal_node,
                          uint32_t new_row, uint32_t int_row, uint32_t seq, int blocks, hipStream_t st);
void launch_union(uint64_t *bits, uint64_t n_words, const uint32_t *d_triples, uint32_t n_triples, hipStream_t st);
constexpr uint32_t INSERT_STEP_BLOCKS = 1024;
void launch_insert_step(uint64_t *bits, uint64_t n_words, uint32_t cur_row, uint32_t new_row, uint32_t left_row,
                        uint32_t right_row, unsigned long long *d_out, hipStream_t st);
void launch_superset(const uint64_t *bits, uint64_t n_words, const uint32_t *d_edges , uint32_t n_edges,
                     uint32_t *d_fail, hipStream_t st);
void launch_transpose(const uint64_t *bits, uint64_t n_words, const uint32_t *d_col_row, uint32_t n_cols, uint32_t *S,
                      uint32_t rw, uint64_t group_stride, uint32_t group_log2, hipStream_t st);
void launch_counts_op(unsigned long long *dst, const unsigned long long *a, const unsigned long long *b, uint32_t n, bool subtract, hipStream_t st);
void launch_hits_csr(const uint2 *d_pairs, uint64_t n_pairs, const uint8_t *d_allhit, uint64_t n_reads, uint32_t n_leaves, bool any_allhit,
                     uint32_t *d_cnt, unsigned long long *d_sums, unsigned long long *d_off, hipStream_t st);
void launch_hits_fill(const uint2 *d_pairs, uint64_t n_pairs, const uint8_t *d_allhit, uint64_t n_reads, const unsigned long long *d_off,
                      uint32_t *d_cnt, uint32_t *d_leaves, hipStream_t st);
void launch_hit_scores(const HashParams &hp, const uint8_t *d_seq, const uint64_t *d_off, uint64_t n_reads, float threshold,
                       const unsigned long long *d_hit_off, const uint32_t *d_hit_leaves, const uint32_t *d_col_row, const uint64_t *d_bits,
                       uint64_t n_words, uint32_t *d_scores, hipStream_t st);
void launch_pair_combine(const unsigned long long *d_hit_off, const uint32_t *d_hit_leaves, const uint8_t *d_allhit, uint64_t n_frag, bool both,
                         uint32_t n_leaves, bool list_all, uint32_t *d_cnt, uint32_t *d_long, unsigned long long *d_misc, unsigned long long *d_sums,
                         unsigned long long *d_frag_off, hipStream_t st);
void launch_pair_fill(const unsigned long long *d_hit_off, const uint32_t *d_hit_leaves, const uint8_t *d_allhit, uint64_t n_frag, bool both,
                      uint32_t n_leaves, const uint32_t *d_long, const unsigned long long *d_misc, const unsigned long long *d_frag_off,
                      uint32_t *d_frag_leaves, hipStream_t st);
void launch_pair_leaf_counts(const uint32_t *d_frag_leaves, const unsigned long long *d_total, const unsigned long long *d_misc, uint32_t n_leaves,
                             uint64_t max_entries, unsigned long long *d_counts, hipStream_t st);
void launch_pair_scores(const HashParams &hp, const uint8_t *d_seq, const uint64_t *d_off, uint64_t n_frag, float threshold, bool both,
                        const unsigned long long *d_frag_off, const uint32_t *d_frag_leaves, const uint32_t *d_col_row, const uint64_t *d_bits,
                        uint64_t n_words, uint32_t *d_scores, hipStream_t st);
constexpr uint32_t LCA_NO_CLADE = 0xffffffffu;
struct LcaTables {
    uint32_t n_leaves, n_clades, top_clade;
    const uint32_t *leaf_clade, *gap_min;
    unsigned long long *here;
};
void launch_lca_pairs(const uint2 *d_pairs, uint64_t n_pairs, const uint8_t *d_allhit, uint64_t n_reads, uint2 *d_span, const LcaTables &tb,
                      uint32_t *d_lca, hipStream_t st);
void launch_lca_rows(const unsigned long long *d_off, const uint32_t *d_leaves, uint64_t n_units, const uint8_t *d_allhit, int pair_mode,
                     const LcaTables &tb, uint32_t *d_lca, hipStream_t st);
void launch_lca_best(const unsigned long long *d_off, const uint32_t *d_leaves, const uint32_t *d_scores, uint64_t n_units, uint2 *d_span,
                     uint32_t *d_long, unsigned long long *d_n_long, const LcaTables &tb, uint32_t *d_lca, hipStream_t st);
void launch_best_rows(const unsigned long long *d_off, const uint32_t *d_leaves, const uint32_t *d_scores, uint64_t n_units, uint32_t *d_cnt,
// ... 180 lines not shown
```

### phagefilter_amd/csrc/pfq_kernels.hip

```cpp
#include "pfq_kernels.h"

#include <atomic>

namespace pfq {

__device__ __forceinline__ uint32_t xcc_id() { return __builtin_amdgcn_s_getreg((31u << 11) | 20u) & 0xFu; }

__device__ __forceinline__ void lds_barrier() {
    __builtin_amdgcn_fence(__ATOMIC_RELEASE, "workgroup", "local");
    __builtin_amdgcn_s_barrier();
    __builtin_amdgcn_fence(__ATOMIC_ACQUIRE, "workgroup", "local");
}

__device__ __forceinline__ unsigned long long bcast_u64(unsigned long long v, int src) {
    return ((unsigned long long)bcast_u32((uint32_t)(v >> 32), src) << 32) | bcast_u32((uint32_t)v, src);
}

constexpr uint32_t SCREEN_ROUNDS = 2;
constexpr uint32_t SCREEN_KMERS = 4;
constexpr uint32_t PAIR_CHUNK = 32;
static_assert(PAIR_CHUNK == PAIR_RESERVE && 256u == MISS_RESERVE, "the host sizes the buffers' slack by these");
constexpr uint32_t SCREEN_EXTRA = 8;
constexpr uint32_t NPLANES = 16;

// ... 1824 lines not shown
            for (int dd = 1; dd < 64; dd <<= 1) {
                const unsigned long long o = __shfl_up(incl, dd);
                if ((int)lane >= dd) incl += o;
            }
            if (have) {
                if ((run + incl) * 16u <= a.kmiss_cap) a.chunks[c].kbase = (uint32_t)(run + incl - need);
                else a.chunks[c].cap = 0;
            }
            run += __shfl(incl, 63);
        }
        if (lane == 0) *a.kmiss_used = run * 16u < a.kmiss_cap ? run * 16u : a.kmiss_cap;
    }
    unsigned long long total = 0;
    for (uint32_t c = lane; c < n_chunks; c += 64) total += (unsigned long long)a.chunks[c].cap * a.n_tiles;
    for (int dd = 32; dd > 0; dd >>= 1) total += __shfl_xor(total, dd);
    if (total <= a.entry_cap) {
        unsigned long long run = 0;
        for (uint32_t c0 = 0; c0 < n_chunks; c0 += 64) {
            const uint32_t c = c0 + lane;
            const uint32_t cap = c < n_chunks ? a.chunks[c].cap : 0u;
            const unsigned long long need = (unsigned long long)cap * a.n_tiles;
            unsigned long long incl = need;
            for (int dd = 1; dd < 64; dd <<= 1) {
                const unsigned long long o = __shfl_up(incl, dd);
                if ((int)lane >= dd) incl += o;
            }
            if (cap) {
                a.chunks[c].base = run + incl - need;
                a.chunks[c].pass = 0;
            }
            run += __shfl(incl, 63);
        }
        if (lane == 0) *a.entry_cursor = run;
        return;
    }
    unsigned long long off = 0;
    uint32_t pass = 0;
    for (uint32_t c0 = 0; c0 < n_chunks; c0 += 64) {
        const uint32_t c = c0 + lane;
        const uint32_t cap = c < n_chunks ? a.chunks[c].cap : 0u;
        const unsigned long long need = (unsigned long long)cap * a.n_tiles;
        unsigned long long my_off = 0;
        uint32_t my_pass = 0;
        for (int i = 0; i < 64; ++i) {
            const unsigned long long ni = ((unsigned long long)bcast_u32((uint32_t)(need >> 32), i) << 32) | bcast_u32((uint32_t)need, i);
            if (ni == 0) continue;
            if (off + ni > a.entry_cap) {
                ++pass;
                off = 0;
            }
            if ((int)lane == i) {
                my_off = off;
                my_pass = pass;
            }
            off += ni;
        }
        if (cap) {
            a.chunks[c].base = my_off;
            a.chunks[c].pass = my_pass;
        }
    }
    if (lane == 0) *a.entry_cursor = (unsigned long long)pass * a.entry_cap + off;
}
__global__ void __launch_bounds__(256) k_zero16(uint4 *p, const unsigned long long *n_bytes) {
    const uint64_t n = (*n_bytes + 15) >> 4;
    for (uint64_t i = (uint64_t)blockIdx.x * blockDim.x + threadIdx.x; i < n; i += (uint64_t)gridDim.x * blockDim.x) p[i] = make_uint4(0, 0, 0, 0);
}
void launch_tile_plan(const TileArgs &a, hipStream_t st) {
    if (!a.n_leaves) return;
    hipLaunchKernelGGL(k_tile_plan, dim3(a.n_leaves), dim3(256), 0, st, a);
    hipLaunchKernelGGL(k_tile_assign, dim3(1), dim3(64), 0, st, a);
    if (a.counts) hipLaunchKernelGGL(k_zero16, dim3(2048), dim3(256), 0, st, reinterpret_cast<uint4 *>(a.kmiss), a.kmiss_used);
    if (a.counts && a.blocks) (void)hipMemsetAsync(a.kall, 0, (a.kmiss_cap >> 3) + 16, st);
}

constexpr uint32_t ENTRY_PAD = 0xffffffffu;
constexpr uint32_t ROUND_PAIRS = 32;
__device__ __forceinline__ void flag_fallback(const TileArgs &a, uint32_t e) {
    if (!(atomicOr(&a.fail[e], 2u) & 2u)) {
        const uint32_t pos = atomicAdd(a.n_flagged, 1u);
        if (pos < a.flag_cap) a.flag_list[pos] = e;
    }
}
template <uint32_t BIN_WAVES, uint32_t BIN_CAP, uint32_t MODE>
__global__ void __launch_bounds__(BIN_WAVES * 64) k_tile_bin(TileArgs a) {
    constexpr bool COUNTS = MODE == 1 || MODE == 3, BLK = MODE == 2;
    constexpr uint32_t TL = MODE == 1 ? TILE_LOG2_COUNTS : (MODE >= 2 ? TILE_LOG2_BLOCK : TILE_LOG2);
    constexpr uint32_t BIN_STRIDE = BIN_CAP + 4;
    constexpr uint32_t WPI = 2;
    const uint32_t NT = (a.n_tiles + 63u) & ~63u;
    const uint32_t DUMMY = NT;
    extern __shared__ uint32_t s_dyn[];
    __shared__ uint32_t s_chunk;
    uint32_t *cnt = s_dyn, *fillp = s_dyn + NT + 64, *bins = fillp + NT;
    const uint32_t lane = lane_id(), wave = threadIdx.x >> 6;
    const uint32_t d = (uint32_t)a.hp.nbits, dw = d - (uint32_t)a.hp.w64, k = a.hp.k, nh = a.hp.num_hashes;
    const uint32_t n_chunks = *a.n_chunks < a.max_chunks ? *a.n_chunks : a.max_chunks;
    uint32_t KB = (uint32_t)(((uint64_t)(BIN_CAP < 128 ? BIN_CAP / 2 : BIN_CAP - BIN_CAP / 4) * a.n_tiles) / nh);
    if (KB > WPI * BIN_WAVES * WIN_KMERS) KB = WPI * BIN_WAVES * WIN_KMERS;
    if (COUNTS && KB > (1u << ROUND_KMERS_LOG2)) KB = 1u << ROUND_KMERS_LOG2;
    if (KB == 0) KB = 1;
    for (uint32_t t = threadIdx.x; t < NT + 64; t += blockDim.x) cnt[t] = 0;
    while (true) {
        __syncthreads();
        if (threadIdx.x == 0) s_chunk = atomicAdd(a.bin_queue, 1u);
        for (uint32_t t = threadIdx.x; t < NT; t += blockDim.x) fillp[t] = 0;
        __syncthreads();
        const uint32_t c = s_chunk;
        if (c >= n_chunks) break;
        const ChunkDesc dsc = a.chunks[c];
        if (dsc.cap == 0) {
            if (a.pass == 0)
                for (uint32_t i = threadIdx.x; i < dsc.n; i += blockDim.x) flag_fallback(a, dsc.first + i);
            continue;
        }
        if (dsc.pass != a.pass) continue;
        uint32_t *bucket0 = a.entries + dsc.base;
        const uint32_t KBc = (BLK && dsc.n < 512u && KB > 3u) ? KB / 4u : KB;
        struct Round {
            uint32_t p, P, K, incl, start;
            unsigned long long koff, qb;
            bool partial;
        };
        auto compose = [&](uint32_t p, unsigned long long koff, const uint4 &m) {
            Round r;
            r.p = p;
            r.koff = koff;
            const bool cand = lane < ROUND_PAIRS && p + lane < dsc.n;
            const uint32_t n_all = cand ? m.z - k + 1u : 0u, n_bin = (MODE == 1 && cand) ? prefix_kmers(a.threshold, n_all, k) : n_all;
            const unsigned long long n64 = cand ? (unsigned long long)n_bin - (lane == 0 ? koff : 0ull) : 0ull;
            const uint32_t n_l = (uint32_t)(n64 > KBc ? KBc + 1u : n64);
            uint32_t incl = n_l;
            for (uint32_t sft = 1; sft < ROUND_PAIRS; sft <<= 1) {
                const uint32_t o = (uint32_t)__shfl_up((int)incl, (int)sft);
                if (lane >= sft) incl += o;
            }
            r.incl = incl;
            r.start = incl - n_l;
            r.P = (uint32_t)__popcll(ballot64(cand && incl <= KBc));
            r.partial = r.P == 0 && p < dsc.n;
            if (r.partial) {
                r.P = 1;
                r.K = KBc;
            } else r.K = r.P ? bcast_u32(incl, (int)r.P - 1) : 0u;
            r.qb = (((unsigned long long)m.y << 32) | m.x) + (lane == 0 ? koff : 0ull) - (unsigned long long)(incl - n_l);
            return r;
        };
        auto load_meta = [&](uint32_t p) {
            const uint32_t i = p + lane % ROUND_PAIRS;
            return a.meta[dsc.first + (i < dsc.n ? i : dsc.n - 1u)];
        };
        auto load_recs = [&](const Round &r, uint4 (&rec)[WPI], uint32_t (&local)[WPI], bool (&valid)[WPI]) {
#pragma unroll
            for (uint32_t u = 0; u < WPI; ++u) {
                const uint32_t f0 = (wave + u * BIN_WAVES) * WIN_KMERS, f = f0 + lane;
                valid[u] = f < r.K;
                uint32_t j0 = (uint32_t)__popcll(ballot64(lane < r.P && r.incl <= f0));
                if (j0 >= r.P) j0 = r.P ? r.P - 1 : 0;
                uint32_t j = j0;
                unsigned long long qb = bcast_u64(r.qb, (int)j0);
                for (uint32_t t = j0; t + 1 < r.P; ++t) {
                    const uint32_t e = bcast_u32(r.incl, (int)t);
                    if (e > f0 + 63u) break;
                    const unsigned long long qn = bcast_u64(r.qb, (int)t + 1);
                    if (f >= e) {
                        j = t + 1;
                        qb = qn;
                    }
                }
                rec[u] = a.recs[valid[u] ? qb + f : bcast_u64(r.qb, 0)];
                local[u] = (COUNTS ? f : r.p + j) << TL;
            }
        };
        auto settle = [&](uint4 (&rec)[WPI], const bool (&valid)[WPI], uint4 &m) {
#pragma unroll
            for (uint32_t u = 0; u < WPI; ++u) {
                asm volatile("" : "+v"(rec[u].x), "+v"(rec[u].y), "+v"(rec[u].z), "+v"(rec[u].w));
                if (!valid[u]) rec[u] = make_uint4(0, 0, 0, 0);
            }
            asm volatile("" : "+v"(m.x), "+v"(m.y), "+v"(m.z));
        };
        uint4 m_nxt = load_meta(0);
        Round cur = compose(0, 0, m_nxt);
        uint4 rec[WPI];
        uint32_t local[WPI];
        bool valid[WPI];
        load_recs(cur, rec, local, valid);
        {
            const uint32_t p1 = cur.partial ? cur.p : cur.p + cur.P;
            m_nxt = load_meta(p1);
        }
        settle(rec, valid, m_nxt);
        uint32_t rho = 0, k0 = 0;
        while (cur.p < dsc.n) {
            if (COUNTS) {
                if (rho >= MAX_ROUNDS) {
                    for (uint32_t i = cur.p + threadIdx.x; i < dsc.n; i += blockDim.x) flag_fallback(a, dsc.first + i);
                    break;
                }
                if (threadIdx.x == 0) a.round_k0[(uint64_t)c * MAX_ROUNDS + rho] = k0;
                if (wave == 0 && lane < cur.P && (lane > 0 || cur.koff == 0)) a.pair_kpos[dsc.first + cur.p + lane] = k0 + (cur.partial ? 0u : cur.start);
            }
            const uint32_t p1 = cur.partial ? cur.p : cur.p + cur.P;
            const Round nxt = compose(p1, cur.partial ? cur.koff + KBc : 0ull, m_nxt);
            uint4 rec_n[WPI];
            uint32_t local_n[WPI];
            bool valid_n[WPI];
            load_recs(nxt, rec_n, local_n, valid_n);
            m_nxt = load_meta(nxt.partial ? nxt.p : nxt.p + nxt.P);
            if (!(PFQ_DEBUG_BITS(a) & 2u)) {
                RecordIter1 rit[WPI];
                uint32_t cbase[WPI];
#pragma unroll
                for (uint32_t u = 0; u < WPI; ++u) {
                    rit[u].init(rec[u], d, dw);
                    cbase[u] = valid[u] ? 0u : DUMMY + lane;
                }
                auto put = [&](const uint32_t (&ix)[WPI]) {
                    uint32_t tile[WPI], slot[WPI];
#pragma unroll
                    for (uint32_t u = 0; u < WPI; ++u) tile[u] = ix[u] >> TL;
#pragma unroll
                    for (uint32_t u = 0; u < WPI; ++u) slot[u] = atomicAdd(&cnt[cbase[u] + tile[u]], 1u);
#pragma unroll
                    for (uint32_t u = 0; u < WPI; ++u)
                        if (valid[u]) bins[tile[u] * BIN_STRIDE + min(slot[u], BIN_CAP - 1u)] = local[u] | (ix[u] & ((1u << TL) - 1u));
                    if (BLK) {
#pragma unroll
                        for (uint32_t u = 0; u < WPI; ++u)
                            if (valid[u] && slot[u] >= BIN_CAP && !(PFQ_DEBUG_BITS(a) & 8u)) flag_fallback(a, dsc.first + (local[u] >> TL));
                    }
                };
                uint32_t ix[WPI];
#pragma unroll
                for (uint32_t u = 0; u < WPI; ++u) ix[u] = rit[u].i0;
                put(ix);
                if (nh > 1) {
#pragma unroll
                    for (uint32_t u = 0; u < WPI; ++u) ix[u] = rit[u].g;
                    put(ix);
                }
                if (nh > 2) {
#pragma unroll
                    for (uint32_t u = 0; u < WPI; ++u) ix[u] = rit[u].x;
                    put(ix);
                }
                for (uint32_t i = 3; i < nh; ++i) {
#pragma unroll
                    for (uint32_t u = 0; u < WPI; ++u) ix[u] = rit[u].step(d);
                    put(ix);
                }
            }
            lds_barrier();
            const uint32_t flush_p = cur.p, flush_P = cur.P, flush_K = cur.K;
            cur = nxt;
            settle(rec_n, valid_n, m_nxt);
#pragma unroll
            for (uint32_t u = 0; u < WPI; ++u) {
                rec[u] = rec_n[u];
                local[u] = local_n[u];
                valid[u] = valid_n[u];
            }
            constexpr uint32_t LPT = BIN_CAP <= 256 ? 8 : 16, TPW = 64 / LPT, STEP = LPT * 4;
            for (uint32_t t0 = wave * TPW; t0 < a.n_tiles; t0 += BIN_WAVES * TPW) {
                const uint32_t t = t0 + lane / LPT, sl = lane % LPT;
                const bool have = t < a.n_tiles;
                const uint32_t cn = have ? cnt[t] : 0u, pos = have ? fillp[t] : 0u;
                const uint32_t cc = cn < BIN_CAP ? cn : BIN_CAP, c4 = (cc + 3u) & ~3u;
                uint32_t *row = bins + t * BIN_STRIDE;
                if (sl < c4 - cc) row[cc + sl] = COUNTS ? row[cc - 1u] : ENTRY_PAD;
                __builtin_amdgcn_wave_barrier();
                const uint32_t room = pos < dsc.cap ? dsc.cap - pos : 0u, wr = c4 < room ? c4 : room;
                uint32_t *dst = bucket0 + (uint64_t)(have ? t : 0u) * dsc.cap + pos;
                constexpr uint32_t FB = BIN_CAP < 128 ? 2 : 5;
                const uint32_t wr_eff = (PFQ_DEBUG_BITS(a) & 1u) ? 0u : wr;
                for (uint32_t i0 = sl * 4u; i0 < wr; i0 += STEP * FB) {
                    uint4 v[FB];
#pragma unroll
                    for (uint32_t u = 0; u < FB; ++u)
                        v[u] = *reinterpret_cast<const uint4 *>(row + min(i0 + u * STEP, BIN_STRIDE - 4u));
#pragma unroll
                    for (uint32_t u = 0; u < FB; ++u)
                        asm volatile("" : "+v"(v[u].x), "+v"(v[u].y), "+v"(v[u].z), "+v"(v[u].w));
                    if (COUNTS) {
#pragma unroll
                        for (uint32_t u = 0; u < FB; ++u) {
                            v[u].x |= (rho & 3u) << 30;
                            v[u].y |= ((rho >> 2) & 3u) << 30;
                            v[u].z |= ((rho >> 4) & 3u) << 30;
                            v[u].w |= ((rho >> 6) & 3u) << 30;
                        }
                    }
#pragma unroll
                    for (uint32_t u = 0; u < FB; ++u)
                        if (i0 + u * STEP < wr_eff) *reinterpret_cast<uint4 *>(dst + i0 + u * STEP) = v[u];
                }
                if (!COUNTS && !(PFQ_DEBUG_BITS(a) & 16u))
                    for (uint32_t i = wr + sl; i < cc; i += LPT) flag_fallback(a, dsc.first + (row[i] >> TL));
                if (!BLK && (cn > BIN_CAP || (COUNTS && wr < cc))) {
                    for (uint32_t i = sl; i < flush_P; i += LPT) flag_fallback(a, dsc.first + flush_p + i);
                }
                __builtin_amdgcn_wave_barrier();
                if (have && sl == 0 && cn) {
                    fillp[t] = pos + c4;
                    cnt[t] = 0;
                }
            }
            lds_barrier();
            k0 += flush_K;
            ++rho;
        }
        if (COUNTS && threadIdx.x == 0) a.n_rounds[c] = rho;
        for (uint32_t t = threadIdx.x; t < a.n_tiles; t += blockDim.x) a.gfill[(uint64_t)c * a.n_tiles + t] = fillp[t];
    }
}
static bool first_on_device(std::atomic<uint64_t> &done) {
    int dev = 0;
    (void)hipGetDevice(&dev);
    const uint64_t bit = 1ull << (dev & 63);
    return !(done.fetch_or(bit) & bit);
}
template <uint32_t W, uint32_t CAP>
static void launch_tile_bin_shape(const TileArgs &a, int blocks, size_t lds, hipStream_t st) {
    static std::atomic<uint64_t> attr_done{0};
    if (first_on_device(attr_done)) {
        (void)hipFuncSetAttribute(reinterpret_cast<const void *>(k_tile_bin<W, CAP, 0>), hipFuncAttributeMaxDynamicSharedMemorySize, 150 * 1024);
        (void)hipFuncSetAttribute(reinterpret_cast<const void *>(k_tile_bin<W, CAP, 1>), hipFuncAttributeMaxDynamicSharedMemorySize, 150 * 1024);
        (void)hipFuncSetAttribute(reinterpret_cast<const void *>(k_tile_bin<W, CAP, 2>), hipFuncAttributeMaxDynamicSharedMemorySize, 150 * 1024);
        (void)hipFuncSetAttribute(reinterpret_cast<const void *>(k_tile_bin<W, CAP, 3>), hipFuncAttributeMaxDynamicSharedMemorySize, 150 * 1024);
    }
    if (a.counts && a.blocks) hipLaunchKernelGGL((k_tile_bin<W, CAP, 3>), dim3(blocks), dim3(W * 64), lds, st, a);
    else if (a.counts) hipLaunchKernelGGL((k_tile_bin<W, CAP, 1>), dim3(blocks), dim3(W * 64), lds, st, a);
    else if (a.blocks) hipLaunchKernelGGL((k_tile_bin<W, CAP, 2>), dim3(blocks), dim3(W * 64), lds, st, a);
    else hipLaunchKernelGGL((k_tile_bin<W, CAP, 0>), dim3(blocks), dim3(W * 64), lds, st, a);
}
uint32_t launch_tile_bin(const TileArgs &a, int blocks, hipStream_t st) {
    const size_t nt = (a.n_tiles + 63u) & ~63u;
    auto lds_of = [&](size_t cap) { return (2 * nt + 64 + (size_t)a.n_tiles * (cap + 4)) * 4; };
    if (a.bin_shape == 3 && lds_of(256) <= 74 * 1024) {
        launch_tile_bin_shape<8, 256>(a, blocks, lds_of(256), st);
        return 8u << 16 | 256u;
    } else if (lds_of(2048) <= 148 * 1024 && a.bin_shape == 0) {
        launch_tile_bin_shape<16, 2048>(a, (blocks + 1) / 2, lds_of(2048), st);
        return 16u << 16 | 2048u;
    } else if (lds_of(1024) <= 148 * 1024 && a.bin_shape == 0) {
        launch_tile_bin_shape<16, 1024>(a, (blocks + 1) / 2, lds_of(1024), st);
        return 16u << 16 | 1024u;
    } else if (lds_of(512) <= 148 * 1024 && a.bin_shape == 0) {
        launch_tile_bin_shape<16, 512>(a, (blocks + 1) / 2, lds_of(512), st);
        return 16u << 16 | 512u;
    } else if (lds_of(256) <= 148 * 1024 && a.bin_shape != 1) {
        launch_tile_bin_shape<16, 256>(a, (blocks + 1) / 2, lds_of(256), st);
        return 16u << 16 | 256u;
    } else if (lds_of(128) <= 148 * 1024) {
        launch_tile_bin_shape<8, 128>(a, blocks, lds_of(128), st);
        return 8u << 16 | 128u;
    } else {
        launch_tile_bin_shape<16, 60>(a, (blocks + 1) / 2, lds_of(60), st);
        return 16u << 16 | 60u;
    }
}

constexpr uint32_t TEST_LOADS = 4;
constexpr uint32_t TEST_GROUP = 32;
template <uint32_t MODE, uint32_t DEPTH = 0, bool CARRY = false>
__global__ void __launch_bounds__(1024) k_tile_test(TileArgs a) {
    constexpr bool SLOTS = DEPTH != 0;
    static_assert(!SLOTS || MODE == 0, "the slots-only build is a build of MODE 0");
    constexpr uint32_t NSET = SLOTS ? 3 : 2;
    constexpr bool COUNTS = MODE == 1 || MODE == 3, BLK = MODE == 2, BLKC = MODE == 3;
    constexpr uint32_t TL = MODE == 1 ? TILE_LOG2_COUNTS : (MODE >= 2 ? TILE_LOG2_BLOCK : TILE_LOG2);
    constexpr uint32_t TILE_BYTES = MODE >= 2 ? (1u << TL) : (1u << (TL - 3));
    constexpr uint32_t TV = TILE_BYTES / 8192u;
    constexpr uint32_t CL = CHUNK_PAIRS_LOG2;
    constexpr uint32_t TG = (BLK || BLKC) ? 16 : TEST_GROUP;
    constexpr uint32_t RK = COUNTS ? MAX_ROUNDS : 1u;
    extern __shared__ uint32_t s_tile[];
    __shared__ uint32_t s_pref[NSET][TG + 1], s_first[NSET][TG], s_misc[NSET][2], s_kbase[2][TG], s_mask[2][TG];
    const uint32_t n_cols = a.n_leaves;
    auto col_of = [&](uint32_t li) { return li; };
    __shared__ uint32_t s_failed[COUNTS ? 1 : (BLK ? (TG << (CL - 2)) : (TG << (CL - 5)))];
    constexpr uint32_t N_FAILED = COUNTS ? 0 : (BLK ? (TG << (CL - 2)) : (TG << (CL - 5)));
    __shared__ uint32_t s_rk0[COUNTS ? TG : 1][RK];
    __shared__ unsigned long long s_base[NSET][TG];
    const uint32_t tile_words = TILE_BYTES / 4u;
    const uint64_t n_words32 = a.n_words * 2;
    const uint64_t n_tasks = (uint64_t)n_cols * a.n_tiles;
    const uint32_t n_chunks = *a.n_chunks < a.max_chunks ? *a.n_chunks : a.max_chunks;
    auto chunk0_of = [&](uint32_t col) {
        if constexpr (SLOTS) return ((const __attribute__((address_space(4))) uint32_t *)a.leaf_chunk0)[col];
        else return a.leaf_chunk0[col_of(col)];
    };
    auto valid_task = [&](uint64_t task) {
        while (task < n_tasks && chunk0_of((uint32_t)(task / a.n_tiles)) == 0xffffffffu) task += gridDim.x;
        return task;
    };
    auto describe = [&](uint32_t buf, uint32_t leaf, uint32_t t, uint32_t g0) {
        const uint32_t i = threadIdx.x, c = g0 + i;
        ChunkDesc dsc{};
        const bool mine = i < TG && c < n_chunks && (dsc = a.chunks[c], dsc.leaf == leaf);
        const bool usable = mine && dsc.cap != 0 && dsc.pass == a.pass;
        uint32_t fill = usable ? a.gfill[(uint64_t)c * a.n_tiles + t] : 0u;
        if (fill > dsc.cap) fill = dsc.cap;
        uint32_t incl = fill;
        for (uint32_t sft = 1; sft < TG; sft <<= 1) {
            const uint32_t o = (uint32_t)__shfl_up((int)incl, (int)sft);
            if (i >= sft) incl += o;
        }
        if (i < TG) {
            s_pref[buf][i + 1] = incl;
            s_first[buf][i] = dsc.first;
            s_kbase[buf][i] = dsc.kbase;
            s_mask[buf][i] = dsc.mask;
            s_base[buf][i] = dsc.base + (uint64_t)t * dsc.cap;
        }
        const uint64_t mm = ballot64(mine);
        if (i == 0) {
            s_pref[buf][0] = 0;
            s_misc[buf][0] = (uint32_t)__popcll(mm);
        }
    };
    auto tile_loads = [&](uint32_t leaf, uint32_t t, uint2 (&v)[TV]) {
        const uint32_t *src = reinterpret_cast<const uint32_t *>(a.bits + (uint64_t)((BLK || BLKC) ? leaf : a.col_row[leaf]) * a.n_words);
        const uint64_t w0 = (uint64_t)t * tile_words;
#pragma unroll
        for (uint32_t u = 0; u < TV; ++u) {
            const uint32_t i = threadIdx.x * 2 + u * 2048u;
            v[u] = (w0 + i + 1 < n_words32) ? *reinterpret_cast<const uint2 *>(src + w0 + i) : make_uint2(0, 0);
        }
    };
    auto tile_store = [&](const uint2 (&v)[TV]) {
#pragma unroll
        for (uint32_t u = 0; u < TV; ++u) *reinterpret_cast<uint2 *>(s_tile + threadIdx.x * 2 + u * 2048u) = v[u];
        if (!COUNTS)
            for (uint32_t i = threadIdx.x; i < N_FAILED; i += blockDim.x) s_failed[i] = 0;
    };
    constexpr bool LISTS = MODE == 0;
    const bool lists_on = LISTS && a.tile_list_row != nullptr && a.tile_lists != nullptr;
    auto list_row = [&](uint32_t leaf) { return lists_on ? a.tile_list_row[leaf] : TILE_LIST_NONE; };
    auto list_loads = [&](uint32_t lrow, uint32_t t, uint2 (&v)[TV]) {
        const uint4 *slot = reinterpret_cast<const uint4 *>(a.tile_lists + ((uint64_t)lrow * a.n_tiles + t) * TILE_LIST_CAP);
        const uint4 l0 = slot[threadIdx.x], l1 = slot[TILE_LIST_CAP / 8u + threadIdx.x];
        v[0] = make_uint2(l0.x, l0.y);
        v[1] = make_uint2(l0.z, l0.w);
        v[2] = make_uint2(l1.x, l1.y);
        v[3] = make_uint2(l1.z, l1.w);
    };
    uint32_t pl[8] = {TILE_LIST_NONE, TILE_LIST_NONE, TILE_LIST_NONE, TILE_LIST_NONE, TILE_LIST_NONE, TILE_LIST_NONE, TILE_LIST_NONE, TILE_LIST_NONE};
    bool cur_list = false;
    uint32_t n_list = 0, n_dense = 0;
    auto list_store = [&](const uint2 (&v)[TV]) {
        if (cur_list) {
#pragma unroll
            for (uint32_t j = 0; j < 8; ++j)
                if (pl[j] < (1u << TL)) atomicAnd(&s_tile[pl[j] >> 5], ~(1u << (pl[j] & 31u)));
        } else {
#pragma unroll
            for (uint32_t u = 0; u < TV; ++u) *reinterpret_cast<uint2 *>(s_tile + threadIdx.x * 2 + u * 2048u) = make_uint2(0, 0);
        }
        for (uint32_t i = threadIdx.x; i < N_FAILED; i += blockDim.x) s_failed[i] = 0;
        __syncthreads();
#pragma unroll
        for (uint32_t j = 0; j < 4; ++j) {
            pl[2 * j] = v[j].x;
            pl[2 * j + 1] = v[j].y;
        }
#pragma unroll
        for (uint32_t j = 0; j < 8; ++j)
            if (pl[j] < (1u << TL)) atomicOr(&s_tile[pl[j] >> 5], 1u << (pl[j] & 31u));
        cur_list = true;
        ++n_list;
    };
    constexpr uint32_t RK_TPC = 1024u / TG, RK_V = TG / 16u;
    auto rk_loads = [&](uint32_t g0, uint4 (&rk)[2]) {
        const uint32_t c = g0 + threadIdx.x / RK_TPC, r0 = (threadIdx.x % RK_TPC) * 4u * RK_V;
        rk[0] = rk[1] = make_uint4(0, 0, 0, 0);
        if (COUNTS && c < n_chunks && r0 < a.n_rounds[c]) {
            const uint4 *src = reinterpret_cast<const uint4 *>(a.round_k0 + (uint64_t)c * MAX_ROUNDS + r0);
            rk[0] = src[0];
            if (RK_V > 1) rk[1] = src[1];
        }
    };
    auto rk_store = [&](const uint4 (&rk)[2]) {
        if (COUNTS) {
            static_assert(!COUNTS || TG == 32 || TG == 16, "1024 threads fetch 256 rounds of TG chunks in one or two 16-byte loads each");
            uint4 *dst = reinterpret_cast<uint4 *>(&s_rk0[threadIdx.x / RK_TPC][(threadIdx.x % RK_TPC) * 4u * RK_V]);
            dst[0] = rk[0];
            if (RK_V > 1) dst[1] = rk[1];
        }
    };
    auto stream = [&](uint32_t buf) {
        const uint32_t total = s_pref[buf][TG];
        uint32_t ci = 0;
        for (uint32_t v0 = threadIdx.x * 4u; v0 < total; v0 += blockDim.x * 4u * TEST_LOADS) {
            uint4 en[TEST_LOADS];
            uint32_t first[TEST_LOADS], cidx[TEST_LOADS];
            bool have[TEST_LOADS];
#pragma unroll
            for (uint32_t u = 0; u < TEST_LOADS; ++u) {
                const uint32_t v = v0 + u * blockDim.x * 4u;
                en[u] = make_uint4(ENTRY_PAD, ENTRY_PAD, ENTRY_PAD, ENTRY_PAD);
                first[u] = 0;
                cidx[u] = 0;
                have[u] = v < total;
                if (have[u]) {
                    while (v >= s_pref[buf][ci + 1]) ++ci;
                    en[u] = *reinterpret_cast<const uint4 *>(a.entries + s_base[buf][ci] + (v - s_pref[buf][ci]));
                    first[u] = s_first[buf][ci];
                    cidx[u] = COUNTS ? ci : ci << CL;
                }
            }
#pragma unroll
            for (uint32_t u = 0; u < TEST_LOADS; ++u) {
                const uint32_t ev[4] = {en[u].x, en[u].y, en[u].z, en[u].w};
                if (BLKC) {
                    if (!have[u]) continue;
                    const uint32_t mk = s_mask[buf][cidx[u]];
                    uint32_t bad[4], any = 0;
#pragma unroll
                    for (uint32_t c = 0; c < 4; ++c) {
                        bad[c] = mk & ~(uint32_t)reinterpret_cast<const uint8_t *>(s_tile)[ev[c] & ((1u << TL) - 1u)];
                        any |= bad[c];
                    }
                    if (any) {
                        const uint32_t rho = (ev[0] >> 30) | ((ev[1] >> 30) << 2) | ((ev[2] >> 30) << 4) | ((ev[3] >> 30) << 6);
                        const uint64_t k0 = (uint64_t)s_kbase[buf][cidx[u]] * 16u + (uint64_t)s_rk0[cidx[u]][rho] * 8u;
#pragma unroll
                        for (uint32_t c = 0; c < 4; ++c) {
                            if (!bad[c]) continue;
                            const uint64_t kq = (k0 >> 3) + ((ev[c] >> TL) & ((1u << ROUND_KMERS_LOG2) - 1u));
                            if (bad[c] == mk) a.kall[kq] = 1;
                            else
                                for (uint32_t m = bad[c]; m; m &= m - 1u) a.kmiss[kq * 8u + (uint32_t)__ffs((int)m) - 1u] = 1;
                        }
                    }
                } else if (COUNTS) {
                    if (!have[u]) continue;
                    uint32_t bad = 0;
#pragma unroll
                    for (uint32_t c = 0; c < 4; ++c) {
                        const uint32_t off = ev[c] & ((1u << TL) - 1u);
                        bad |= (((s_tile[off >> 5] >> (off & 31u)) & 1u) ^ 1u) << c;
                    }
                    if (bad) {
                        const uint32_t rho = (ev[0] >> 30) | ((ev[1] >> 30) << 2) | ((ev[2] >> 30) << 4) | ((ev[3] >> 30) << 6);
                        const uint32_t kb = s_rk0[cidx[u]][rho], wb = s_kbase[buf][cidx[u]];
#pragma unroll
                        for (uint32_t c = 0; c < 4; ++c) {
                            if (!((bad >> c) & 1u)) continue;
                            a.kmiss[(uint64_t)wb * 16u + kb + ((ev[c] >> TL) & ((1u << ROUND_KMERS_LOG2) - 1u))] = 1;
                        }
                    }
                } else if (BLK) {
                    if (!have[u]) continue;
#pragma unroll
                    for (uint32_t c = 0; c < 4; ++c) {
                        const uint32_t off = ev[c] & ((1u << TL) - 1u);
                        const uint32_t bad = ev[c] != ENTRY_PAD ? s_mask[buf][cidx[u] >> CL] & ~(uint32_t)reinterpret_cast<const uint8_t *>(s_tile)[off] : 0u;
                        if (bad) {
                            const uint32_t lp = (ev[c] >> TL) & ((1u << CL) - 1u), fb = cidx[u] + lp, sh = 8u * (fb & 3u);
                            if (bad & ~(s_failed[fb >> 2] >> sh)) {
                                const uint32_t fresh = bad & ~(atomicOr(&s_failed[fb >> 2], bad << sh) >> sh);
                                for (uint32_t m = fresh; m; m &= m - 1u) a.failb[((uint64_t)(first[u] + lp) << 3) + (uint32_t)__ffs((int)m) - 1u] = 1;
                            }
                        }
                    }
                } else {
#pragma unroll
                    for (uint32_t c = 0; c < 4; ++c) {
                        const uint32_t off = ev[c] & ((1u << TL) - 1u);
                        if (ev[c] != ENTRY_PAD && !((s_tile[off >> 5] >> (off & 31u)) & 1u)) {
                            const uint32_t lp = ev[c] >> TL, fb = cidx[u] + lp;
                            if (!(atomicOr(&s_failed[fb >> 5], 1u << (fb & 31u)) & (1u << (fb & 31u)))) atomicOr(&a.fail[first[u] + lp], 1u);
                        }
                    }
                }
            }
        }
    };

    if constexpr (SLOTS) {
        constexpr uint32_t STEP = 1024u * 4u * TEST_LOADS;
        uint4 en[DEPTH][TEST_LOADS];
        uint32_t pk[DEPTH];
        uint32_t ci = 0;
#pragma unroll
        for (uint32_t j = 0; j < DEPTH; ++j) {
            pk[j] = 0;
#pragma unroll
            for (uint32_t u = 0; u < TEST_LOADS; ++u) en[j][u] = make_uint4(ENTRY_PAD, ENTRY_PAD, ENTRY_PAD, ENTRY_PAD);
        }
        auto issue = [&](uint32_t j, uint32_t set, uint32_t step, uint32_t total) {
            uint32_t word = 0;
#pragma unroll
            for (uint32_t u = 0; u < TEST_LOADS; ++u) {
                const uint32_t v = step * STEP + u * 4096u + threadIdx.x * 4u;
                const bool have = v < total;
                if (have)
                    while (v >= s_pref[set][ci + 1]) ++ci;
                const uint64_t at = have ? s_base[set][ci] + (v - s_pref[set][ci]) : 0ull;
                en[j][u] = *reinterpret_cast<const uint4 *>(a.entries + at);
                word |= (have ? 0x80u | ci : 0u) << (8u * u);
            }
            pk[j] = word;
        };
        auto test = [&](uint32_t j, uint32_t set) {
#pragma unroll
            for (uint32_t u = 0; u < TEST_LOADS; ++u) {
                const uint32_t w = pk[j] >> (8u * u);
                if (!(w & 0x80u)) continue;
                const uint32_t ev[4] = {en[j][u].x, en[j][u].y, en[j][u].z, en[j][u].w};
#pragma unroll
                for (uint32_t c = 0; c < 4; ++c) {
                    const uint32_t off = ev[c] & ((1u << TL) - 1u);
                    if (ev[c] != ENTRY_PAD && !((s_tile[off >> 5] >> (off & 31u)) & 1u)) {
                        const uint32_t b = w & 31u, lp = ev[c] >> TL, fb = (b << CL) + lp;
                        if (!(atomicOr(&s_failed[fb >> 5], 1u << (fb & 31u)) & (1u << (fb & 31u)))) atomicOr(&a.fail[s_first[set][b] + lp], 1u);
                    }
                }
            }
        };
        static_assert(TEST_GROUP <= 32, "a step's word has 5 bits per bucket");
        struct Described {
            uint32_t first, cap, base_lo, base_hi, leaf, pass;
            uint32_t fill;
            bool in;
        };
        static_assert(sizeof(ChunkDesc) == 48 && offsetof(ChunkDesc, first) == 4 && offsetof(ChunkDesc, cap) == 12 && offsetof(ChunkDesc, base) == 16 &&
                          offsetof(ChunkDesc, leaf) == 24 && offsetof(ChunkDesc, pass) == 28,
                      "describe_loads reads a ChunkDesc as 32-bit words");
        auto describe_loads = [&](uint32_t t, uint32_t g) {
            Described d{};
            const uint32_t i = threadIdx.x < TG ? threadIdx.x : 0u;
            d.in = threadIdx.x < TG && g + i < n_chunks;
            const uint32_t c = g + i < n_chunks ? g + i : n_chunks - 1u;
            const uint32_t *w = reinterpret_cast<const uint32_t *>(a.chunks + c);
            d.first = w[1], d.cap = w[3], d.base_lo = w[4], d.base_hi = w[5], d.leaf = w[6], d.pass = w[7];
            d.fill = a.gfill[(uint64_t)c * a.n_tiles + t];
            return d;
        };
        auto describe_put = [&](uint32_t set, uint32_t leaf, uint32_t t, const Described &d) {
            const uint32_t i = threadIdx.x;
            const bool mine = d.in && d.leaf == leaf;
            const bool usable = mine && d.cap != 0 && d.pass == a.pass;
            uint32_t fill = usable ? d.fill : 0u;
            if (fill > d.cap) fill = d.cap;
            uint32_t incl = fill;
            for (uint32_t sft = 1; sft < TG; sft <<= 1) {
                const uint32_t o = (uint32_t)__shfl_up((int)incl, (int)sft);
                if (i >= sft) incl += o;
            }
            if (i < TG) {
                s_pref[set][i + 1] = incl;
                s_first[set][i] = d.first;
                const uint32_t lo = d.base_lo + t * d.cap, hi = d.base_hi + __umulhi(t, d.cap) + (lo < d.base_lo ? 1u : 0u);
                uint32_t *dst = reinterpret_cast<uint32_t *>(&s_base[set][i]);
                dst[0] = lo;
                dst[1] = hi;
            }
            const uint64_t mm = ballot64(mine);
            if (i == 0) {
                s_pref[set][0] = 0;
                s_misc[set][0] = (uint32_t)__popcll(mm);
            }
        };
        auto unit_after = [&](uint64_t task, uint32_t g, bool more, uint64_t &ntask, uint32_t &ng) {
            ntask = more ? task : valid_task(task + gridDim.x);
            if (ntask >= n_tasks) return false;
            ng = more ? g + TG : chunk0_of((uint32_t)(ntask / a.n_tiles));
            return true;
        };
        auto leaf_of = [&](uint64_t task) { return (uint32_t)(task / a.n_tiles); };
        auto tile_of = [&](uint64_t task) { return (uint32_t)(task % a.n_tiles); };
        uint64_t task0 = valid_task(blockIdx.x), task1 = 0, task2 = 0;
        if (task0 >= n_tasks) return;
        uint32_t g0 = chunk0_of(leaf_of(task0)), g1 = 0, g2 = 0, d0 = 0, d1 = 1, d2 = 2;
        bool have1;
        {
            uint2 v[TV];
            list_loads(leaf_of(task0), tile_of(task0), v);
            const Described d = describe_loads(tile_of(task0), g0);
            if (threadIdx.x < 64) describe_put(d0, leaf_of(task0), tile_of(task0), d);
            list_store(v);
            __syncthreads();
            have1 = unit_after(task0, g0, s_misc[d0][0] == TG, task1, g1);
            const Described d1st = describe_loads(have1 ? tile_of(task1) : 0u, have1 ? g1 : 0u);
            if (have1 && threadIdx.x < 64) describe_put(d1, leaf_of(task1), tile_of(task1), d1st);
            __syncthreads();
        }
        uint32_t total0 = s_pref[d0][TG];
#pragma unroll
        for (uint32_t j = 0; j < DEPTH; ++j) issue(j, d0, j, total0);
        while (true) {
            const bool have2 = have1 && unit_after(task1, g1, s_misc[d1][0] == TG, task2, g2);
            const bool tile1 = have1 && task1 != task0;
            uint2 vn[TV];
            if (tile1) list_loads(leaf_of(task1), tile_of(task1), vn);
            const Described dn = describe_loads(have2 ? tile_of(task2) : 0u, have2 ? g2 : 0u);
            const uint32_t total1 = (CARRY && have1) ? s_pref[d1][TG] : 0u;
            const uint32_t steps0 = (total0 + STEP - 1u) / STEP;
            for (uint32_t s = 0; s < steps0 || s == 0; s += DEPTH) {
                const bool last = s + DEPTH >= steps0;
                if (last) ci = 0;
#pragma unroll
                for (uint32_t j = 0; j < DEPTH; ++j) {
                    test(j, d0);
                    issue(j, last ? d1 : d0, last ? j : s + DEPTH + j, last ? total1 : total0);
                }
            }
            if (have2 && threadIdx.x < 64) describe_put(d2, leaf_of(task2), tile_of(task2), dn);
            __syncthreads();
            if (!have1) break;
            if (tile1) list_store(vn);
            else
                for (uint32_t i = threadIdx.x; i < N_FAILED; i += blockDim.x) s_failed[i] = 0;
            __syncthreads();
            task0 = task1, g0 = g1, task1 = task2, g1 = g2, have1 = have2;
            const uint32_t d = d0;
            d0 = d1, d1 = d2, d2 = d;
            total0 = s_pref[d0][TG];
            if (!CARRY) {
                ci = 0;
#pragma unroll
                for (uint32_t j = 0; j < DEPTH; ++j) issue(j, d0, j, total0);
            }
        }
        if (a.tile_list_stats && threadIdx.x == 0 && n_list) atomicAdd(&a.tile_list_stats[0], (unsigned long long)n_list);
        return;
    }
    uint64_t task = valid_task(blockIdx.x);
    if (task >= n_tasks) return;
    uint32_t buf = 0, g0 = a.leaf_chunk0[col_of((uint32_t)(task / a.n_tiles))];
    {
        const uint32_t leaf = col_of((uint32_t)(task / a.n_tiles)), t = (uint32_t)(task % a.n_tiles);
        const uint32_t lrow = list_row(leaf);
        uint2 v[TV];
        uint4 rk[2];
        if (LISTS && lrow != TILE_LIST_NONE) list_loads(lrow, t, v);
        else tile_loads(leaf, t, v);
        rk_loads(g0, rk);
        if (threadIdx.x < 64) describe(0, leaf, t, g0);
        if (LISTS && lrow != TILE_LIST_NONE) list_store(v);
        else {
            tile_store(v);
            ++n_dense;
        }
        rk_store(rk);
        __syncthreads();
    }
    while (true) {
        const bool more = s_misc[buf][0] == TG;
        const uint64_t ntask = more ? task : valid_task(task + gridDim.x);
        const bool have_n = ntask < n_tasks;
        const uint32_t nleaf = have_n ? col_of((uint32_t)(ntask / a.n_tiles)) : 0u, nt = have_n ? (uint32_t)(ntask % a.n_tiles) : 0u;
        const uint32_t ng0 = more ? g0 + TG : (have_n ? a.leaf_chunk0[nleaf] : 0u);
        const bool nlist = LISTS && have_n && !more && list_row(nleaf) != TILE_LIST_NONE;
        uint2 vn[TV];
        uint4 rkn[2];
        if (nlist) list_loads(a.tile_list_row[nleaf], nt, vn);
        else if (have_n && !more) tile_loads(nleaf, nt, vn);
        if (have_n) rk_loads(ng0, rkn);
        if (have_n && threadIdx.x < 64) describe(buf ^ 1u, nleaf, nt, ng0);
        stream(buf);
        __syncthreads();
        if (!have_n) break;
        if (nlist) list_store(vn);
        else if (!more) {
            tile_store(vn);
            cur_list = false;
            ++n_dense;
        } else if (!COUNTS)
            for (uint32_t i = threadIdx.x; i < N_FAILED; i += blockDim.x) s_failed[i] = 0;
        rk_store(rkn);
        __syncthreads();
        task = ntask;
        g0 = ng0;
        buf ^= 1u;
    }
    if (LISTS && a.tile_list_stats && threadIdx.x == 0) {
        if (n_list) atomicAdd(&a.tile_list_stats[0], (unsigned long long)n_list);
        if (n_dense) atomicAdd(&a.tile_list_stats[1], (unsigned long long)n_dense);
    }
}
#ifndef PFQ_STREAM_DEPTH
#define PFQ_STREAM_DEPTH 2
#endif
#ifndef PFQ_STREAM_CARRY
#define PFQ_STREAM_CARRY 1
#endif
void launch_tile_test(const TileArgs &a, int blocks, hipStream_t st) {
    static std::atomic<uint64_t> attr_done{0};
    const auto k_stream = k_tile_test<0, PFQ_STREAM_DEPTH, PFQ_STREAM_CARRY != 0>;
    if (first_on_device(attr_done)) {
        (void)hipFuncSetAttribute(reinterpret_cast<const void *>(k_tile_test<0>), hipFuncAttributeMaxDynamicSharedMemorySize, 150 * 1024);
        (void)hipFuncSetAttribute(reinterpret_cast<const void *>(k_stream), hipFuncAttributeMaxDynamicSharedMemorySize, 150 * 1024);
        (void)hipFuncSetAttribute(reinterpret_cast<const void *>(k_tile_test<1>), hipFuncAttributeMaxDynamicSharedMemorySize, 1 << (TILE_LOG2_COUNTS - 3));
        (void)hipFuncSetAttribute(reinterpret_cast<const void *>(k_tile_test<2>), hipFuncAttributeMaxDynamicSharedMemorySize, 1 << TILE_LOG2_BLOCK);
        (void)hipFuncSetAttribute(reinterpret_cast<const void *>(k_tile_test<3>), hipFuncAttributeMaxDynamicSharedMemorySize, 1 << TILE_LOG2_BLOCK);
    }
    const dim3 g((blocks + 1) / 2), b(1024);
    if (a.counts && a.blocks) hipLaunchKernelGGL(k_tile_test<3>, g, b, (size_t)(1u << TILE_LOG2_BLOCK), st, a);
    else if (a.counts) hipLaunchKernelGGL(k_tile_test<1>, g, b, (size_t)(1u << (TILE_LOG2_COUNTS - 3)), st, a);
    else if (a.blocks) hipLaunchKernelGGL(k_tile_test<2>, g, b, (size_t)(1u << TILE_LOG2_BLOCK), st, a);
    else if (a.tile_stream && a.tile_list_row && a.tile_lists) hipLaunchKernelGGL(k_stream, g, b, (size_t)(1u << (TILE_LOG2 - 3)), st, a);
    else hipLaunchKernelGGL(k_tile_test<0>, g, b, (size_t)(1u << (TILE_LOG2 - 3)), st, a);
}

__global__ void __launch_bounds__(256) k_collect_open(const uint32_t *fail, const uint32_t *n_pairs_ptr, uint32_t *list,
                                                      uint32_t cap, unsigned int *n_out) {
    __shared__ uint32_t s_w[4], s_base;
    const uint32_t n = *n_pairs_ptr, lane = lane_id(), wave = threadIdx.x >> 6;
    const uint32_t per = ((n + gridDim.x - 1) / gridDim.x + 255u) & ~255u;
    const uint32_t lo = blockIdx.x * per, hi = lo + per < n ? lo + per : n;
    if (lo >= n) return;
    uint32_t c = 0;
    for (uint32_t e = lo + threadIdx.x; e < hi; e += 256) c += fail[e] != 0u;
    for (int d = 32; d > 0; d >>= 1) c += __shfl_down(c, d);
    if (lane == 0) s_w[wave] = c;
    __syncthreads();
    if (threadIdx.x == 0) {
        const uint32_t tot = s_w[0] + s_w[1] + s_w[2] + s_w[3];
        s_base = tot ? atomicAdd(n_out, tot) : 0u;
    }
    __syncthreads();
    uint32_t run = s_base;
    if (s_w[0] + s_w[1] + s_w[2] + s_w[3] == 0) return;
    __syncthreads();
    for (uint32_t e0 = lo; e0 < hi; e0 += 256) {
        const uint32_t e = e0 + threadIdx.x;
        const bool open = e < hi && fail[e] != 0u;
        const uint64_t b = ballot64(open);
        if (lane == 0) s_w[wave] = (uint32_t)__popcll(b);
        __syncthreads();
        uint32_t before = 0, all = 0;
        for (uint32_t w = 0; w < 4; ++w) {
            before += w < wave ? s_w[w] : 0u;
            all += s_w[w];
        }
        const uint32_t pos = run + before + (uint32_t)__popcll(b & ((1ull << lane) - 1ull));
        if (open && pos < cap) list[pos] = e;
        run += all;
        __syncthreads();
    }
}
void launch_collect_open(const uint32_t *fail, const uint32_t *n_pairs_ptr, uint32_t *list, uint32_t cap, unsigned int *n_out, hipStream_t st) {
    hipLaunchKernelGGL(k_collect_open, dim3(512), dim3(256), 0, st, fail, n_pairs_ptr, list, cap, n_out);
}
void launch_verify(const VerifyArgs &a, int blocks, int threads, hipStream_t st) {
    if (a.recs) hipLaunchKernelGGL(k_verify_rec, dim3(blocks), dim3(threads), 0, st, a);
    else hipLaunchKernelGGL(k_verify, dim3(blocks), dim3(256), 0, st, a);
}

__global__ void __launch_bounds__(256) k_block_tables(const uint64_t *bits, uint64_t n_words, const uint32_t *col_row, uint32_t n_leaves, uint8_t *T) {
    const uint32_t lane = lane_id(), wave = threadIdx.x >> 6, b = blockIdx.y;
    uint8_t *dst = T + (uint64_t)b * n_words * 64;
    const uint64_t *src[8];
#pragma unroll
    for (uint32_t j = 0; j < 8; ++j) src[j] = (8u * b + j < n_leaves) ? bits + (uint64_t)col_row[8u * b + j] * n_words : nullptr;
    for (uint64_t w = (uint64_t)blockIdx.x * WAVES_PER_BLOCK + wave; w < n_words; w += (uint64_t)gridDim.x * WAVES_PER_BLOCK) {
        uint32_t byte = 0;
#pragma unroll
        for (uint32_t j = 0; j < 8; ++j) {
            const uint64_t v = src[j] ? src[j][w] : 0ull;
            byte |= (uint32_t)((v >> lane) & 1ull) << j;
        }
        dst[w * 64 + lane] = (uint8_t)byte;
    }
}
void launch_block_tables(const uint64_t *bits, uint64_t n_words, const uint32_t *d_col_row, uint32_t n_leaves, uint8_t *T, hipStream_t st) {
    if (!n_leaves) return;
    uint64_t bx = (n_words + 3) / 4;
    if (bx > 1024) bx = 1024;
    hipLaunchKernelGGL(k_block_tables, dim3((uint32_t)bx, (n_leaves + 7) / 8), dim3(256), 0, st, bits, n_words, d_col_row, n_leaves, T);
}

__global__ void __launch_bounds__(256) k_block_fallback(QueryArgs a, const uint2 *sorted, const uint32_t *n_pairs_ptr, const uint32_t *fail, uint8_t *failb,
                                                        const uint32_t *pair_chunk, const ChunkDesc *chunks, uint32_t launched_passes,
                                                        const unsigned int *n_flagged, const uint32_t *flag_list, uint32_t flag_cap) {
    __shared__ BlockLds lds;
    fill_complement(lds.comp);
    __syncthreads();
    const uint32_t lane = lane_id(), wave = threadIdx.x >> 6, n_pairs = *n_pairs_ptr;
    const uint64_t gw = (uint64_t)blockIdx.x * WAVES_PER_BLOCK + wave, nw = (uint64_t)gridDim.x * WAVES_PER_BLOCK;
    auto certify = [&](uint64_t e, uint32_t r, uint32_t y, uint32_t j) {
        const uint64_t o0 = a.off[r], L = a.off[r + 1] - o0;
        ReadCtx rc;
        rc.read = a.seq + o0;
        rc.n = L - a.hp.k + 1;
// ... 1020 lines not shown
```

### phagefilter_amd/query.py

```python
from __future__ import annotations

import ctypes as C
from typing import Dict, List, Optional, Sequence, Set, Tuple

import numpy as np

from . import _ffi


class ResultMap:

    def __init__(self) -> None:
        self.read_map: Dict[str, Set[str]] = {}

    def add_read_map(self, read_id: str, genome_id: str) -> None:
        self.read_map.setdefault(read_id, set()).add(genome_id)

    def get_ext_id(self, read_id: str) -> str:
        return f"{read_id} |{','.join(self.read_map.get(read_id, ()))}"

    def read_mapped(self, read_id: str) -> bool:
        return read_id in self.read_map

    def empty_read_map(self) -> None:
# ... 83 lines not shown
                                      kmer_size: int, nbits: int, num_hashes: int, seed1: int, seed2: int, depth: int,
                                      index: int, false_pos_rate: float = 0.001, largest_expected_genome: int = 1000000,
                                      device: int = 0) -> "BloomTree":
        ids = (C.c_char_p * max(len(tax_ids), 1))(*[t.encode() for t in tax_ids])
        h = C.c_void_p()
        _ffi.check(_ffi.lib().pfq_tree_build_balanced_subtree_device(d_genomes, genome_len, n_genomes, ids, kmer_size,
                                                                     nbits, num_hashes, seed1, seed2, false_pos_rate,
                                                                     largest_expected_genome, depth, index, device,
                                                                     C.byref(h)))
        return cls(h, device)

    def close(self) -> None:
        if self._h:
            _ffi.lib().pfq_tree_close(self._h)
            self._h = None

    def __del__(self):
        try:
            self.close()
        except Exception:
            pass

    def save(self, directory: str) -> None:
        import os
        os.makedirs(directory, exist_ok=True)
        _ffi.check(_ffi.lib().pfq_tree_save(self._h, directory.encode()))

    def prune_tree(self, search_depth: int) -> None:
        _ffi.check(_ffi.lib().pfq_tree_prune(self._h, search_depth))

    def info(self) -> _ffi.Info:
        i = _ffi.Info()
        _ffi.check(_ffi.lib().pfq_tree_info(self._h, C.byref(i)))
        return i

    @property
    def kmer_size(self) -> int:
        return int(self.info().kmer_size)

    def get_leaf_counts(self) -> List[Tuple[str, int]]:
        ids = C.POINTER(C.c_char_p)()
        cnt = C.POINTER(C.c_uint64)()
        n = C.c_uint64()
        _ffi.check(_ffi.lib().pfq_leaf_counts(self._h, C.byref(ids), C.byref(cnt), C.byref(n)))
        return [(ids[i].decode(), int(cnt[i])) for i in range(n.value)]

    def save_leaf_counts(self, path: str) -> None:
        _ffi.check(_ffi.lib().pfq_save_leaf_counts(self._h, path.encode()))

    def reset_counts(self) -> None:
        _ffi.check(_ffi.lib().pfq_leaf_counts_reset(self._h))

    def set_option(self, name: str, value: Optional[str]) -> None:
        _ffi.check(_ffi.lib().pfq_set_option(self._h, name.encode(), None if value is None else str(value).encode()))

    def set_path(self, path: int) -> None:
        _ffi.check(_ffi.lib().pfq_set_path(self._h, path))

    def last_stats(self) -> _ffi.Stats:
        s = _ffi.Stats()
        _ffi.check(_ffi.lib().pfq_last_stats(self._h, C.byref(s)))
        return s

    CAPACITY_FIELDS = ("pair_cursor", "pair_cap", "guard_cursor", "guard_cap", "miss_cursor", "miss_cap", "kmiss_used",
                       "kmiss_cap", "hit_cursor", "hit_cap", "attempts", "pairs_sorted")

    def last_capacity(self) -> dict:
        out = np.zeros(len(self.CAPACITY_FIELDS), dtype=np.uint64)
        _ffi.check(_ffi.lib().pfq_debug_last_capacity(self._h, out.ctypes.data, out.size))
        return {k: int(v) for k, v in zip(self.CAPACITY_FIELDS, out)}

    TILE_LIST_CAP = 8192
    TILE_LIST_NONE = 0xFFFFFFFF

    def tile_lists_info(self) -> dict:
        out = np.zeros(4, dtype=np.uint64)
        _ffi.check(_ffi.lib().pfq_tile_lists_info(self._h, out.ctypes.data))
        return {k: int(v) for k, v in zip(("columns", "bytes", "list_tiles", "dense_tiles"), out)}

    def tile_list(self, col: int, tile: int) -> np.ndarray:
        out = np.zeros(self.TILE_LIST_CAP, dtype=np.uint32)
        _ffi.check(_ffi.lib().pfq_debug_tile_list(self._h, col, tile, out.ctypes.data, out.size))
        return out

    def profile_begin(self, max_calls: int) -> None:
        _ffi.check(_ffi.lib().pfq_profile_begin(self._h, max_calls))

    def profile_end(self) -> _ffi.Profile:
        p = _ffi.Profile()
        _ffi.check(_ffi.lib().pfq_profile_end(self._h, C.byref(p)))
        return p

    def kmer_indices(self, seq: bytes) -> np.ndarray:
        n = C.c_uint64()
        buf = np.frombuffer(seq + b"\0", dtype=np.uint8).copy()
        _ffi.check(_ffi.lib().pfq_debug_kmer_indices(self._h, buf.ctypes.data, len(seq), None, C.byref(n)))
        out = np.zeros((n.value, int(self.info().num_hashes)), dtype=np.uint64)
        if n.value:
            _ffi.check(_ffi.lib().pfq_debug_kmer_indices(self._h, buf.ctypes.data, len(seq), out.ctypes.data, C.byref(n)))
        return out

    def node_filter(self, node: int) -> np.ndarray:
        i = self.info()
        out = np.zeros((int(i.nbits) + 63) // 64, dtype=np.uint64)
        _ffi.check(_ffi.lib().pfq_debug_node_filter(self._h, node, out.ctypes.data, out.size))
        return out

    def query_packed(self, seq: np.ndarray, off: np.ndarray, threshold: float, want_hits: bool = False,
                     want_scores: bool = False, paired: bool = False, pair_mode: str = "either",
                     lca: Optional[str] = None, abundance: bool = False, coverage: bool = False, taxa: bool = False,
                     best: bool = False, sweep: bool = False):
        lca_flags = (_lca_flags(lca, want_hits, want_scores) | _abundance_flags(abundance, want_hits) | _coverage_flags(coverage, want_hits) |
                     _taxa_flags(taxa, want_hits) | _best_flags(best, want_hits, want_scores) | _sweep_flags(sweep, want_hits, want_scores))
        n = len(off) - 1
        seq = np.ascontiguousarray(seq, dtype=np.uint8)
        off = np.ascontiguousarray(off, dtype=np.uint64)
        hits = _ffi.Hits()
        flags = (_ffi.WANT_HITS if want_hits else 0) | (_ffi.WANT_SCORES if want_scores else 0) | _pair_flags(paired, pair_mode) | lca_flags
        _ffi.check(_ffi.lib().pfq_query_batch(self._h, seq.ctypes.data, off.ctypes.data, n, threshold, flags, C.byref(hits)))
        return self._hits_result(hits, want_hits, want_scores)

    def _hits_result(self, hits: "_ffi.Hits", want_hits: bool, want_scores: bool):
        if not want_hits:
            return None
        n = int(hits.n_reads)
        offs = np.ctypeslib.as_array(hits.offsets, shape=(n + 1,)).copy() if n else np.zeros(1, dtype=np.uint64)
        total = int(offs[-1])
        leaves = np.ctypeslib.as_array(hits.leaves, shape=(total,)).copy() if total else np.zeros(0, dtype=np.uint32)
        if not want_scores:
            return offs, leaves
        return offs, leaves, self.last_hit_scores().copy()

    def parse_text(self, data: bytes, fmt: str, limit: Optional[int] = None, final: bool = True, want_records: bool = False) -> dict:
        if fmt not in ("fasta", "fastq"):
            raise ValueError(f"fmt must be 'fasta' or 'fastq', not {fmt!r}")
        buf = np.frombuffer(bytes(data), dtype=np.uint8)
        out = _ffi.Text()
        flags = (_ffi.TEXT_FINAL if final else 0) | (_ffi.TEXT_WANT_RECORDS if want_records else 0)
        _ffi.check(_ffi.lib().pfq_text_parse(self._h, buf.ctypes.data if buf.size else None, buf.size, (1 << 64) - 1 if limit is None else limit,
                                             _ffi.TEXT_FASTQ if fmt == "fastq" else _ffi.TEXT_FASTA, flags, C.byref(out)))
        self._text_shape = (int(out.n_records), int(out.n_bases))
        n = int(out.n_records)
        return {"n_records": n, "consumed": int(out.consumed), "n_bases": int(out.n_bases),
                "stop": ("end", "limit", "more", "slow")[out.stop],
                "rec_begin": np.ctypeslib.as_array(out.rec_begin, shape=(n + 1,)).copy() if want_records else None}

    def text_csr(self) -> Tuple[np.ndarray, np.ndarray]:
        n, nb = getattr(self, "_text_shape", (0, 0))
        seq, off = np.zeros(nb, dtype=np.uint8), np.zeros(n + 1, dtype=np.uint64)
        _ffi.check(_ffi.lib().pfq_debug_text_csr(self._h, seq.ctypes.data, off.ctypes.data))
        return seq, off

    def query_text(self, threshold: float, want_hits: bool = False, want_scores: bool = False, paired: bool = False,
                   pair_mode: str = "either", lca: Optional[str] = None, abundance: bool = False, coverage: bool = False, taxa: bool = False,
                   best: bool = False, sweep: bool = False):
        lca_flags = (_lca_flags(lca, want_hits, want_scores) | _abundance_flags(abundance, want_hits) | _coverage_flags(coverage, want_hits) |
                     _taxa_flags(taxa, want_hits) | _best_flags(best, want_hits, want_scores) | _sweep_flags(sweep, want_hits, want_scores))
        hits = _ffi.Hits()
        flags = (_ffi.WANT_HITS if want_hits else 0) | (_ffi.WANT_SCORES if want_scores else 0) | _pair_flags(paired, pair_mode) | lca_flags
        _ffi.check(_ffi.lib().pfq_text_query(self._h, threshold, flags, C.byref(hits)))
        return self._hits_result(hits, want_hits, want_scores)

    PREP_REASONS = ("kept", "short", "n", "complexity", "mate")

    def prep_reads(self, seq: np.ndarray, off: np.ndarray, qual: Optional[np.ndarray] = None, has_qual: Optional[np.ndarray] = None, *,
                   trim_quality: int = 0, trim_window: int = 4, poly_x: int = 0, min_length: int = 0, max_n: Optional[int] = None,
# ... 431 lines not shown
```

Measured before the change: 476.8 million.

## Pack tile-bucket entries as 24-bit values, five per four words

Adds a packed entry format for the threshold-1 LDS-tile path. Each entry is stored as 24 bits with a per-round id byte, so five entries fit in four 32-bit words. Failures are recorded per round in byte arrays and scattered to the per-pair fail flags by a new k_pack_fail kernel. The aim is to cut the bucket write and read bandwidth between the bin and test kernels. The cost is limiting rounds to 16 pairs and 256 rounds per chunk, with overflow sent to a fallback path, plus an extra kernel launch. It also adds a debug bucket inspector and a stats flag.

After: 533.2 million (median of 6 runs). +11.8%, better.

```diff
diff --git a/include/pfq.h b/include/pfq.h
--- a/include/pfq.h
+++ b/include/pfq.h
@@ -263,6 +263,8 @@
 
 int pfq_tile_lists_info(pfq_tree *tree, uint64_t out[4]);
 int pfq_debug_tile_list(pfq_tree *tree, uint64_t col, uint64_t tile, uint32_t *out, uint64_t n);
+#define PFQ_TILE_BUCKET_WORDS 1296
+int pfq_debug_tile_bucket(pfq_tree *tree, uint64_t chunk, uint64_t tile, uint32_t *out, uint64_t cap);
 
 
 typedef struct pfq_stats {
@@ -280,6 +282,7 @@
     uint32_t tile_bin_build;
     uint64_t group_reads;
     uint32_t pair_stage;
+    uint32_t entry_pack;
 } pfq_stats;
 int pfq_last_stats(pfq_tree *tree, pfq_stats *out);
 int pfq_set_path(pfq_tree *tree, int path);
diff --git a/phagefilter_amd/_ffi.py b/phagefilter_amd/_ffi.py
--- a/phagefilter_amd/_ffi.py
+++ b/phagefilter_amd/_ffi.py
@@ -22,7 +22,7 @@
     "pfq_save_leaf_counts", "pfq_leaf_counts_export", "pfq_leaf_counts_import", "pfq_leaf_counts_reset",
     "pfq_leaf_counts_export_delta", "pfq_leaf_counts_import_delta",
     "pfq_last_stats", "pfq_set_path", "pfq_profile_begin", "pfq_profile_end", "pfq_debug_kmer_indices", "pfq_debug_node_filter", "pfq_debug_last_capacity", "pfq_debug_last_similarity", "pfq_debug_last_recluster",
-    "pfq_tile_lists_info", "pfq_debug_tile_list",
+    "pfq_tile_lists_info", "pfq_debug_tile_list", "pfq_debug_tile_bucket",
     "pfq_synth_genomes_device",
     "pfq_synth_reads_device", "pfq_host_alloc", "pfq_host_free", "pfq_last_error", "pfq_version",
 ]
@@ -53,7 +53,7 @@
                 ("n_chunks", C.c_uint64), ("tile_entries", C.c_uint64), ("tile_passes_launched", C.c_uint32),
                 ("tile_passes_needed", C.c_uint32), ("leaf_groups", C.c_uint32), ("coarse_cols", C.c_uint32),
                 ("coarse_probes", C.c_uint32), ("tile_bin_build", C.c_uint32), ("group_reads", C.c_uint64),
-                ("pair_stage", C.c_uint32)]
+                ("pair_stage", C.c_uint32), ("entry_pack", C.c_uint32)]
 
 
 class Profile(C.Structure):
@@ -251,6 +251,8 @@
     if hasattr(L, "pfq_tile_lists_info"):
         L.pfq_tile_lists_info.argtypes = [vp, vp]
         L.pfq_debug_tile_list.argtypes = [vp, C.c_uint64, C.c_uint64, vp, C.c_uint64]
+    if hasattr(L, "pfq_debug_tile_bucket"):
+        L.pfq_debug_tile_bucket.argtypes = [vp, C.c_uint64, C.c_uint64, vp, C.c_uint64]
     L.pfq_synth_genomes_device.argtypes = [vp, C.c_uint64, C.c_uint64, C.c_uint64, vp]
     L.pfq_synth_reads_device.argtypes = [vp, C.c_uint64, C.c_uint64, C.c_uint64, vp, C.c_uint64, C.c_uint64,
                                          C.c_uint64, vp]
diff --git a/phagefilter_amd/csrc/pfq_host.cpp b/phagefilter_amd/csrc/pfq_host.cpp
--- a/phagefilter_amd/csrc/pfq_host.cpp
+++ b/phagefilter_amd/csrc/pfq_host.cpp
@@ -104,6 +104,7 @@
     long long sweep_lds = -1;
     long long tile_lists = -1;
     long long tile_stream = -1;
+    long long entry_pack = -1;
 };
 struct KnobName {
     const char *name;
@@ -137,6 +138,7 @@
     {"PFQ_SIM_TIME", &Knobs::sim_time},         {"PFQ_CLUSTER_TIME", &Knobs::cluster_time},
     {"PFQ_TEXT_TILE", &Knobs::text_tile},       {"PFQ_SWEEP_LDS", &Knobs::sweep_lds},
     {"PFQ_TILE_LISTS", &Knobs::tile_lists},     {"PFQ_TILE_STREAM", &Knobs::tile_stream},
+    {"PFQ_ENTRY_PACK", &Knobs::entry_pack},
 };
 bool set_knob(Knobs &k, const char *name, const char *value) {
     for (const KnobName &kn : KNOBS)
@@ -282,6 +284,10 @@
     bool have_cand_hint = false;
     uint32_t last_block_mode = 0;
     DevBuf<uint32_t> d_round_k0, d_n_rounds, d_pair_kpos;
+    DevBuf<uint32_t> d_round_p0;
+    DevBuf<uint8_t> d_round_fail;
+    bool last_entry_pack = false;
+    uint32_t last_n_tiles = 0;
     uint32_t last_tile_mode = 0, last_passes = 1;
     uint32_t last_sort = 0;
     bool last_tile_stream = false;
@@ -1689,6 +1695,7 @@
         t.last_tile_mode = 0;
         t.last_tile_bin = 0;
         t.last_tile_stream = false;
+        t.last_entry_pack = false;
         if (tile_mode) {
             const uint64_t max_chunks = nc + ((t.leaf_cap + t.guard_cap) >> chunk_log2) + 2;
             uint64_t want = (uint64_t)((double)total_bytes * t.num_hashes * 1.13 * std::max(1.0, t.pairs_per_read)) +
@@ -1704,6 +1711,21 @@
                 ok = soft_ensure(t.d_kmiss, kmiss_cap) && soft_ensure(t.d_round_k0, max_chunks * pfq::MAX_ROUNDS) &&
                      soft_ensure(t.d_n_rounds, max_chunks) && soft_ensure(t.d_pair_kpos, t.d_pairs.n);
             if (ok && counts_mode && block_mode) ok = soft_ensure(t.d_kall, (kmiss_cap >> 3) + 64);
+            bool pack = false;
+            const uint32_t bin_shape = kn.bin_narrow > 0 ? (uint32_t)kn.bin_narrow : (kn.bin_wide > 0 ? 2u : 0u);
+            if (ok && !counts_mode && !block_mode && kn.entry_pack != 0) {
+                pfq::TileArgs shape{};
+                shape.n_tiles = n_tiles;
+                shape.bin_shape = bin_shape;
+                const uint32_t build = pfq::tile_bin_build(shape);
+                const uint64_t KB = pfq::tile_bin_kmer_budget(build >> 16, build & 0xffffu, n_tiles, t.num_hashes, false);
+                const uint64_t kmers = total_bytes > n_reads * (t.kmer_size - 1) ? total_bytes - n_reads * (t.kmer_size - 1) : 0;
+                pack = kn.entry_pack == 2 || (n_reads && kmers * pfq::PACK_PAIRS >= KB * n_reads &&
+                                              (2ull << chunk_log2) * kmers + 2 * KB * n_reads <= pfq::PACK_ROUNDS * KB * n_reads);
+                if (pack)
+                    pack = soft_ensure(t.d_round_p0, max_chunks * pfq::PACK_ROUNDS) && soft_ensure(t.d_n_rounds, max_chunks) &&
+                           soft_ensure(t.d_round_fail, max_chunks * pfq::PACK_ROUNDS * pfq::PACK_PAIRS);
+            }
             if (!ok) {
                 tile_mode = false;
             } else {
@@ -1749,6 +1771,13 @@
                         ta.tile_lists = t.d_tile_lists.p;
                         ta.tile_stream = t.tile_list_cols == t.n_cols && kn.tile_stream != 0;
                     }
+                    if (pack) {
+                        ta.entry_pack = 1;
+                        ta.round_p0 = t.d_round_p0.p;
+                        ta.round_fail = t.d_round_fail.p;
+                        ta.n_rounds = t.d_n_rounds.p;
+                        HIP_TRY(hipMemsetAsync(t.d_n_rounds.p, 0, max_chunks * 4, st));
+                    }
                 }
                 if (counts_mode) {
                     ta.counts = 1;
@@ -1765,7 +1794,7 @@
                 int bin_blocks = 512, test_blocks = 512;
                 if (kn.bin_blocks >= 0) bin_blocks = std::max(1, (int)kn.bin_blocks);
                 if (kn.test_blocks >= 0) test_blocks = std::max(1, (int)kn.test_blocks);
-                ta.bin_shape = kn.bin_narrow > 0 ? (uint32_t)kn.bin_narrow : (kn.bin_wide > 0 ? 2u : 0u);
+                ta.bin_shape = bin_shape;
                 ta.debug = kn.bin_debug > 0 ? (uint32_t)kn.bin_debug : 0u;
                 pfq::launch_tile_plan(ta, st);
                 uint64_t n_passes = std::min<uint64_t>(std::max<uint64_t>(1, t.passes_hint), 256);
@@ -1782,6 +1811,9 @@
                     pfq::launch_tile_test(ta, test_blocks, st);
                     t.last_tile_stream = ta.tile_stream != 0;
                 }
+                pfq::launch_pack_fail(ta, st);
+                t.last_entry_pack = ta.entry_pack != 0;
+                t.last_n_tiles = n_tiles;
                 v.pair_chunk = t.d_pair_chunk.p;
                 v.chunks = t.d_chunks.p;
                 v.entry_cursor = t.d_cursors.p + CUR_TILE_ENTRIES;
@@ -4680,6 +4712,7 @@
         const uint32_t shapes = t.last_path ? (uint32_t)c[CUR_TAIL_SHAPES] : 0u;
         out->pair_stage = t.last_sort | ((shapes & 7u) << 4) | ((shapes & pfq::TAIL_SHAPE_FULL) ? 4u : 0u) |
                           ((t.last_path && h[pfq::ST_BATCHED]) ? 8u : 0u) | ((t.last_path && t.last_tile_mode && t.last_tile_stream) ? 0x80u : 0u);
+        out->entry_pack = (t.last_path && t.last_tile_mode && t.last_entry_pack) ? 1u : 0u;
         out->n_chunks = (uint32_t)c[CUR_CHUNKS_FLAGGED];
         out->n_fallback_pairs = (uint32_t)(c[CUR_CHUNKS_FLAGGED] >> 32);
         out->tile_entries = c[CUR_TILE_ENTRIES];
@@ -4830,6 +4863,42 @@
     return PFQ_OK;
 }
 
+int pfq_debug_tile_bucket(pfq_tree *tree, uint64_t chunk, uint64_t tile, uint32_t *out, uint64_t cap) {
+    if (!tree || !out) return fail(PFQ_ERR_ARG, "null argument");
+    PFQ_TRY(use_device(tree->device));
+    pfq_tree &t = *tree;
+    if (!t.d_cursors.p || !t.last_tile_mode || t.last_block_mode || !t.last_n_tiles) return fail(PFQ_ERR_STATE, "the last call ran no LDS-tile pass at threshold 1");
+    if (cap < PFQ_TILE_BUCKET_WORDS) return fail(PFQ_ERR_ARG, "the buffer holds less than the header and the tables");
+    PFQ_TRY(wait_last_call(t));
+    unsigned long long n_chunks = 0;
+    HIP_TRY(hipMemcpy(&n_chunks, t.d_cursors.p + CUR_CHUNKS_FLAGGED, 8, hipMemcpyDeviceToHost));
+    n_chunks = std::min<uint64_t>(n_chunks & 0xffffffffu, t.d_chunks.n);
+    memset(out, 0, PFQ_TILE_BUCKET_WORDS * 4);
+    out[7] = (uint32_t)n_chunks;
+    if (chunk >= n_chunks || tile >= t.last_n_tiles) return fail(PFQ_ERR_ARG, "chunk / tile out of range");
+    pfq::ChunkDesc dsc;
+    HIP_TRY(hipMemcpy(&dsc, t.d_chunks.p + chunk, sizeof dsc, hipMemcpyDeviceToHost));
+    uint32_t fill = 0;
+    HIP_TRY(hipMemcpy(&fill, t.d_gfill.p + chunk * t.last_n_tiles + tile, 4, hipMemcpyDeviceToHost));
+    out[0] = fill;
+    out[1] = t.last_entry_pack ? pfq::pack_bucket_words(dsc.cap) : dsc.cap;
+    out[2] = dsc.first;
+    out[3] = dsc.n;
+    out[4] = dsc.leaf;
+    out[5] = dsc.pass;
+    out[6] = t.last_entry_pack ? 1u : 0u;
+    if (t.last_entry_pack) {
+        HIP_TRY(hipMemcpy(out + 8, t.d_n_rounds.p + chunk, 4, hipMemcpyDeviceToHost));
+        HIP_TRY(hipMemcpy(out + 16, t.d_round_p0.p + chunk * pfq::PACK_ROUNDS, pfq::PACK_ROUNDS * 4, hipMemcpyDeviceToHost));
+    }
+    std::vector<uint2> pairs(dsc.n);
+    if (dsc.n) HIP_TRY(hipMemcpy(pairs.data(), t.d_sorted.p + dsc.first, dsc.n * sizeof(uint2), hipMemcpyDeviceToHost));
+    for (uint32_t i = 0; i < dsc.n && i < (1u << pfq::CHUNK_PAIRS_LOG2); ++i) out[16 + pfq::PACK_ROUNDS + i] = pairs[i].x;
+    const uint64_t words = std::min<uint64_t>(std::min(fill, out[1]), cap - PFQ_TILE_BUCKET_WORDS);
+    if (words) HIP_TRY(hipMemcpy(out + PFQ_TILE_BUCKET_WORDS, t.d_entries.p + dsc.base + tile * dsc.cap, words * 4, hipMemcpyDeviceToHost));
+    return PFQ_OK;
+}
+
 int pfq_debug_kmer_indices(pfq_tree *tree, const uint8_t *seq, uint64_t len, uint64_t *out_idx, uint64_t *n_kmers) {
     if (!tree || !n_kmers || (len && !seq)) return fail(PFQ_ERR_ARG, "null argument");
     PFQ_TRY(use_device(tree->device));
diff --git a/phagefilter_amd/csrc/pfq_kernels.h b/phagefilter_amd/csrc/pfq_kernels.h
--- a/phagefilter_amd/csrc/pfq_kernels.h
+++ b/phagefilter_amd/csrc/pfq_kernels.h
@@ -152,6 +152,22 @@
 constexpr uint32_t TILE_LOG2_COUNTS = 19;
 constexpr uint32_t ROUND_KMERS_LOG2 = 11;
 constexpr uint32_t MAX_ROUNDS = 256;
+constexpr uint32_t PACK_PAIRS = 16;
+constexpr uint32_t PACK_ROUNDS = 256;
+#if defined(__HIPCC__)
+__host__ __device__
+#endif
+inline uint32_t pack_bucket_words(uint32_t cap) { return cap / 5u * 4u; }
+constexpr uint32_t TILE_BIN_WPI = 2;
+#if defined(__HIPCC__)
+__host__ __device__
+#endif
+inline uint32_t tile_bin_kmer_budget(uint32_t waves, uint32_t cap, uint32_t n_tiles, uint32_t num_hashes, bool counts) {
+    uint32_t kb = (uint32_t)(((uint64_t)(cap < 128 ? cap / 2 : cap - cap / 4) * n_tiles) / (num_hashes ? num_hashes : 1u));
+    if (kb > TILE_BIN_WPI * waves * 64u) kb = TILE_BIN_WPI * waves * 64u;
+    if (counts && kb > (1u << ROUND_KMERS_LOG2)) kb = 1u << ROUND_KMERS_LOG2;
+    return kb ? kb : 1u;
+}
 constexpr uint32_t TILE_LOG2_BLOCK = 17;
 constexpr uint32_t BLOCK_LEAVES_LOG2 = 3;
 struct ChunkDesc {
@@ -210,7 +226,12 @@
     const uint32_t *tile_lists;
     unsigned long long *tile_list_stats;
     uint32_t tile_stream;
-};
+    uint32_t entry_pack;
+    uint32_t *round_p0;
+    uint8_t *round_fail;
+};
+void launch_pack_fail(const TileArgs &a, hipStream_t st);
+uint32_t tile_bin_build(const TileArgs &a);
 constexpr uint32_t TILE_LIST_CAP = 8192;
 constexpr uint32_t TILE_LIST_NONE = 0xffffffffu;
 void launch_tile_list_count(const uint64_t *bits, uint64_t n_words, const uint32_t *col_row, uint32_t n_cols, uint32_t n_tiles, uint32_t *col_max,
diff --git a/phagefilter_amd/csrc/pfq_kernels.hip b/phagefilter_amd/csrc/pfq_kernels.hip
--- a/phagefilter_amd/csrc/pfq_kernels.hip
+++ b/phagefilter_amd/csrc/pfq_kernels.hip
@@ -1930,8 +1930,9 @@
         if (pos < a.flag_cap) a.flag_list[pos] = e;
     }
 }
-template <uint32_t BIN_WAVES, uint32_t BIN_CAP, uint32_t MODE>
+template <uint32_t BIN_WAVES, uint32_t BIN_CAP, uint32_t MODE, bool PACK = false>
 __global__ void __launch_bounds__(BIN_WAVES * 64) k_tile_bin(TileArgs a) {
+    static_assert(!PACK || MODE == 0, "packed entries are a format of MODE 0");
     constexpr bool COUNTS = MODE == 1 || MODE == 3, BLK = MODE == 2;
     constexpr uint32_t TL = MODE == 1 ? TILE_LOG2_COUNTS : (MODE >= 2 ? TILE_LOG2_BLOCK : TILE_LOG2);
     constexpr uint32_t BIN_STRIDE = BIN_CAP + 4;
@@ -1944,10 +1945,8 @@
     const uint32_t lane = lane_id(), wave = threadIdx.x >> 6;
     const uint32_t d = (uint32_t)a.hp.nbits, dw = d - (uint32_t)a.hp.w64, k = a.hp.k, nh = a.hp.num_hashes;
     const uint32_t n_chunks = *a.n_chunks < a.max_chunks ? *a.n_chunks : a.max_chunks;
-    uint32_t KB = (uint32_t)(((uint64_t)(BIN_CAP < 128 ? BIN_CAP / 2 : BIN_CAP - BIN_CAP / 4) * a.n_tiles) / nh);
-    if (KB > WPI * BIN_WAVES * WIN_KMERS) KB = WPI * BIN_WAVES * WIN_KMERS;
-    if (COUNTS && KB > (1u << ROUND_KMERS_LOG2)) KB = 1u << ROUND_KMERS_LOG2;
-    if (KB == 0) KB = 1;
+    const uint32_t KB = tile_bin_kmer_budget(BIN_WAVES, BIN_CAP, a.n_tiles, nh, COUNTS);
+    static_assert(WPI == TILE_BIN_WPI, "tile_bin_kmer_budget counts WPI windows a wave");
     for (uint32_t t = threadIdx.x; t < NT + 64; t += blockDim.x) cnt[t] = 0;
     while (true) {
         __syncthreads();
@@ -1974,7 +1973,7 @@
             Round r;
             r.p = p;
             r.koff = koff;
-            const bool cand = lane < ROUND_PAIRS && p + lane < dsc.n;
+            const bool cand = lane < (PACK ? PACK_PAIRS : ROUND_PAIRS) && p + lane < dsc.n;
             const uint32_t n_all = cand ? m.z - k + 1u : 0u, n_bin = (MODE == 1 && cand) ? prefix_kmers(a.threshold, n_all, k) : n_all;
             const unsigned long long n64 = cand ? (unsigned long long)n_bin - (lane == 0 ? koff : 0ull) : 0ull;
             const uint32_t n_l = (uint32_t)(n64 > KBc ? KBc + 1u : n64);
@@ -2049,6 +2048,17 @@
                 if (threadIdx.x == 0) a.round_k0[(uint64_t)c * MAX_ROUNDS + rho] = k0;
                 if (wave == 0 && lane < cur.P && (lane > 0 || cur.koff == 0)) a.pair_kpos[dsc.first + cur.p + lane] = k0 + (cur.partial ? 0u : cur.start);
             }
+            if (PACK) {
+                if (rho >= PACK_ROUNDS) {
+                    for (uint32_t i = cur.p + threadIdx.x; i < dsc.n; i += blockDim.x) flag_fallback(a, dsc.first + i);
+                    break;
+                }
+                if (threadIdx.x == 0) {
+                    a.round_p0[(uint64_t)c * PACK_ROUNDS + rho] = cur.p;
+                    static_assert(PACK_PAIRS == 16, "a round's failure bytes are one 16-byte store");
+                    *reinterpret_cast<uint4 *>(a.round_fail + ((uint64_t)c * PACK_ROUNDS + rho) * PACK_PAIRS) = make_uint4(0, 0, 0, 0);
+                }
+            }
             const uint32_t p1 = cur.partial ? cur.p : cur.p + cur.P;
             const Round nxt = compose(p1, cur.partial ? cur.koff + KBc : 0ull, m_nxt);
             uint4 rec_n[WPI];
@@ -2114,39 +2124,79 @@
                 const uint32_t t = t0 + lane / LPT, sl = lane % LPT;
                 const bool have = t < a.n_tiles;
                 const uint32_t cn = have ? cnt[t] : 0u, pos = have ? fillp[t] : 0u;
-                const uint32_t cc = cn < BIN_CAP ? cn : BIN_CAP, c4 = (cc + 3u) & ~3u;
+                const uint32_t cc = cn < BIN_CAP ? cn : BIN_CAP;
                 uint32_t *row = bins + t * BIN_STRIDE;
-                if (sl < c4 - cc) row[cc + sl] = COUNTS ? row[cc - 1u] : ENTRY_PAD;
-                __builtin_amdgcn_wave_barrier();
-                const uint32_t room = pos < dsc.cap ? dsc.cap - pos : 0u, wr = c4 < room ? c4 : room;
-                uint32_t *dst = bucket0 + (uint64_t)(have ? t : 0u) * dsc.cap + pos;
-                constexpr uint32_t FB = BIN_CAP < 128 ? 2 : 5;
-                const uint32_t wr_eff = (PFQ_DEBUG_BITS(a) & 1u) ? 0u : wr;
-                for (uint32_t i0 = sl * 4u; i0 < wr; i0 += STEP * FB) {
-                    uint4 v[FB];
-#pragma unroll
-                    for (uint32_t u = 0; u < FB; ++u)
-                        v[u] = *reinterpret_cast<const uint4 *>(row + min(i0 + u * STEP, BIN_STRIDE - 4u));
-#pragma unroll
-                    for (uint32_t u = 0; u < FB; ++u)
-                        asm volatile("" : "+v"(v[u].x), "+v"(v[u].y), "+v"(v[u].z), "+v"(v[u].w));
-                    if (COUNTS) {
+                const uint32_t c4 = PACK ? ((cc + 4u) / 5u) * 4u : (cc + 3u) & ~3u;
+                if constexpr (PACK) {
+                    const uint32_t nv = c4 >> 2;
+                    if (sl < nv * 5u - cc) row[cc + sl] = row[cc - 1u];
+                    __builtin_amdgcn_wave_barrier();
+                    const uint32_t capw = pack_bucket_words(dsc.cap);
+                    const uint32_t room = pos < capw ? capw - pos : 0u, wr = c4 < room ? c4 : room;
+                    const uint32_t wrv = wr >> 2, wr_ent = wrv * 5u < cc ? wrv * 5u : cc;
+                    uint32_t *dst = bucket0 + (uint64_t)(have ? t : 0u) * dsc.cap + pos;
+                    constexpr uint32_t FB = BIN_CAP < 128 ? 2 : 5;
+                    constexpr uint32_t VMAX = (BIN_STRIDE - 5u) / 5u;
+                    static_assert(BIN_STRIDE >= 5u * ((BIN_CAP + 4u) / 5u), "the padding of a full bin fits its row");
+                    const uint32_t wrv_eff = (PFQ_DEBUG_BITS(a) & 1u) ? 0u : wrv;
+                    const uint32_t sub = flush_p << TL, tag = (rho & (PACK_ROUNDS - 1u)) << 24;
+                    for (uint32_t v0 = sl; v0 < wrv; v0 += LPT * FB) {
+                        uint32_t e[FB][5];
 #pragma unroll
                         for (uint32_t u = 0; u < FB; ++u) {
-                            v[u].x |= (rho & 3u) << 30;
-                            v[u].y |= ((rho >> 2) & 3u) << 30;
-                            v[u].z |= ((rho >> 4) & 3u) << 30;
-                            v[u].w |= ((rho >> 6) & 3u) << 30;
+                            const uint32_t *src = row + 5u * min(v0 + u * LPT, VMAX);
+#pragma unroll
+                            for (uint32_t j = 0; j < 5; ++j) e[u][j] = src[j];
+                        }
+#pragma unroll
+                        for (uint32_t u = 0; u < FB; ++u)
+                            asm volatile("" : "+v"(e[u][0]), "+v"(e[u][1]), "+v"(e[u][2]), "+v"(e[u][3]), "+v"(e[u][4]));
+#pragma unroll
+                        for (uint32_t u = 0; u < FB; ++u) {
+                            if (v0 + u * LPT >= wrv_eff) continue;
+                            const uint32_t e0 = (e[u][0] - sub) & 0xffffffu, e1 = (e[u][1] - sub) & 0xffffffu, e2 = (e[u][2] - sub) & 0xffffffu,
+                                           e3 = (e[u][3] - sub) & 0xffffffu, e4 = (e[u][4] - sub) & 0xffffffu;
+                            *reinterpret_cast<uint4 *>(dst + 4u * (v0 + u * LPT)) =
+                                make_uint4(e0 | (e1 << 24), (e1 >> 8) | (e2 << 16), (e2 >> 16) | (e3 << 8), e4 | tag);
                         }
                     }
-#pragma unroll
-                    for (uint32_t u = 0; u < FB; ++u)
-                        if (i0 + u * STEP < wr_eff) *reinterpret_cast<uint4 *>(dst + i0 + u * STEP) = v[u];
-                }
-                if (!COUNTS && !(PFQ_DEBUG_BITS(a) & 16u))
-                    for (uint32_t i = wr + sl; i < cc; i += LPT) flag_fallback(a, dsc.first + (row[i] >> TL));
-                if (!BLK && (cn > BIN_CAP || (COUNTS && wr < cc))) {
-                    for (uint32_t i = sl; i < flush_P; i += LPT) flag_fallback(a, dsc.first + flush_p + i);
+                    if (!(PFQ_DEBUG_BITS(a) & 16u))
+                        for (uint32_t i = wr_ent + sl; i < cc; i += LPT) flag_fallback(a, dsc.first + (row[i] >> TL));
+                    if (cn > BIN_CAP)
+                        for (uint32_t i = sl; i < flush_P; i += LPT) flag_fallback(a, dsc.first + flush_p + i);
+                } else {
+                    if (sl < c4 - cc) row[cc + sl] = COUNTS ? row[cc - 1u] : ENTRY_PAD;
+                    __builtin_amdgcn_wave_barrier();
+                    const uint32_t room = pos < dsc.cap ? dsc.cap - pos : 0u, wr = c4 < room ? c4 : room;
+                    uint32_t *dst = bucket0 + (uint64_t)(have ? t : 0u) * dsc.cap + pos;
+                    constexpr uint32_t FB = BIN_CAP < 128 ? 2 : 5;
+                    const uint32_t wr_eff = (PFQ_DEBUG_BITS(a) & 1u) ? 0u : wr;
+                    for (uint32_t i0 = sl * 4u; i0 < wr; i0 += STEP * FB) {
+                        uint4 v[FB];
+#pragma unroll
+                        for (uint32_t u = 0; u < FB; ++u)
+                            v[u] = *reinterpret_cast<const uint4 *>(row + min(i0 + u * STEP, BIN_STRIDE - 4u));
+#pragma unroll
+                        for (uint32_t u = 0; u < FB; ++u)
+                            asm volatile("" : "+v"(v[u].x), "+v"(v[u].y), "+v"(v[u].z), "+v"(v[u].w));
+                        if (COUNTS) {
+#pragma unroll
+                            for (uint32_t u = 0; u < FB; ++u) {
+                                v[u].x |= (rho & 3u) << 30;
+                                v[u].y |= ((rho >> 2) & 3u) << 30;
+                                v[u].z |= ((rho >> 4) & 3u) << 30;
+                                v[u].w |= ((rho >> 6) & 3u) << 30;
+                            }
+                        }
+#pragma unroll
+                        for (uint32_t u = 0; u < FB; ++u)
+                            if (i0 + u * STEP < wr_eff) *reinterpret_cast<uint4 *>(dst + i0 + u * STEP) = v[u];
+                    }
+                    if (!COUNTS && !(PFQ_DEBUG_BITS(a) & 16u))
+                        for (uint32_t i = wr + sl; i < cc; i += LPT) flag_fallback(a, dsc.first + (row[i] >> TL));
+                    if (!BLK && (cn > BIN_CAP || (COUNTS && wr < cc))) {
+                        for (uint32_t i = sl; i < flush_P; i += LPT) flag_fallback(a, dsc.first + flush_p + i);
+                    }
                 }
                 __builtin_amdgcn_wave_barrier();
                 if (have && sl == 0 && cn) {
@@ -2158,7 +2208,7 @@
             k0 += flush_K;
             ++rho;
         }
-        if (COUNTS && threadIdx.x == 0) a.n_rounds[c] = rho;
+        if ((COUNTS || PACK) && threadIdx.x == 0) a.n_rounds[c] = rho;
         for (uint32_t t = threadIdx.x; t < a.n_tiles; t += blockDim.x) a.gfill[(uint64_t)c * a.n_tiles + t] = fillp[t];
     }
 }
@@ -2176,43 +2226,48 @@
         (void)hipFuncSetAttribute(reinterpret_cast<const void *>(k_tile_bin<W, CAP, 1>), hipFuncAttributeMaxDynamicSharedMemorySize, 150 * 1024);
         (void)hipFuncSetAttribute(reinterpret_cast<const void *>(k_tile_bin<W, CAP, 2>), hipFuncAttributeMaxDynamicSharedMemorySize, 150 * 1024);
         (void)hipFuncSetAttribute(reinterpret_cast<const void *>(k_tile_bin<W, CAP, 3>), hipFuncAttributeMaxDynamicSharedMemorySize, 150 * 1024);
+        (void)hipFuncSetAttribute(reinterpret_cast<const void *>(k_tile_bin<W, CAP, 0, true>), hipFuncAttributeMaxDynamicSharedMemorySize, 150 * 1024);
     }
     if (a.counts && a.blocks) hipLaunchKernelGGL((k_tile_bin<W, CAP, 3>), dim3(blocks), dim3(W * 64), lds, st, a);
     else if (a.counts) hipLaunchKernelGGL((k_tile_bin<W, CAP, 1>), dim3(blocks), dim3(W * 64), lds, st, a);
     else if (a.blocks) hipLaunchKernelGGL((k_tile_bin<W, CAP, 2>), dim3(blocks), dim3(W * 64), lds, st, a);
+    else if (a.entry_pack) hipLaunchKernelGGL((k_tile_bin<W, CAP, 0, true>), dim3(blocks), dim3(W * 64), lds, st, a);
     else hipLaunchKernelGGL((k_tile_bin<W, CAP, 0>), dim3(blocks), dim3(W * 64), lds, st, a);
 }
+static size_t tile_bin_lds(const TileArgs &a, size_t cap) {
+    const size_t nt = (a.n_tiles + 63u) & ~63u;
+    return (2 * nt + 64 + (size_t)a.n_tiles * (cap + 4)) * 4;
+}
+uint32_t tile_bin_build(const TileArgs &a) {
+    auto lds_of = [&](size_t cap) { return tile_bin_lds(a, cap); };
+    if (a.bin_shape == 3 && lds_of(256) <= 74 * 1024) return 8u << 16 | 256u;
+    if (lds_of(2048) <= 148 * 1024 && a.bin_shape == 0) return 16u << 16 | 2048u;
+    if (lds_of(1024) <= 148 * 1024 && a.bin_shape == 0) return 16u << 16 | 1024u;
+    if (lds_of(512) <= 148 * 1024 && a.bin_shape == 0) return 16u << 16 | 512u;
+    if (lds_of(256) <= 148 * 1024 && a.bin_shape != 1) return 16u << 16 | 256u;
+    if (lds_of(128) <= 148 * 1024) return 8u << 16 | 128u;
+    return 16u << 16 | 60u;
+}
 uint32_t launch_tile_bin(const TileArgs &a, int blocks, hipStream_t st) {
-    const size_t nt = (a.n_tiles + 63u) & ~63u;
-    auto lds_of = [&](size_t cap) { return (2 * nt + 64 + (size_t)a.n_tiles * (cap + 4)) * 4; };
-    if (a.bin_shape == 3 && lds_of(256) <= 74 * 1024) {
-        launch_tile_bin_shape<8, 256>(a, blocks, lds_of(256), st);
-        return 8u << 16 | 256u;
-    } else if (lds_of(2048) <= 148 * 1024 && a.bin_shape == 0) {
-        launch_tile_bin_shape<16, 2048>(a, (blocks + 1) / 2, lds_of(2048), st);
-        return 16u << 16 | 2048u;
-    } else if (lds_of(1024) <= 148 * 1024 && a.bin_shape == 0) {
-        launch_tile_bin_shape<16, 1024>(a, (blocks + 1) / 2, lds_of(1024), st);
-        return 16u << 16 | 1024u;
-    } else if (lds_of(512) <= 148 * 1024 && a.bin_shape == 0) {
-        launch_tile_bin_shape<16, 512>(a, (blocks + 1) / 2, lds_of(512), st);
-        return 16u << 16 | 512u;
-    } else if (lds_of(256) <= 148 * 1024 && a.bin_shape != 1) {
-        launch_tile_bin_shape<16, 256>(a, (blocks + 1) / 2, lds_of(256), st);
-        return 16u << 16 | 256u;
-    } else if (lds_of(128) <= 148 * 1024) {
-        launch_tile_bin_shape<8, 128>(a, blocks, lds_of(128), st);
-        return 8u << 16 | 128u;
-    } else {
-        launch_tile_bin_shape<16, 60>(a, (blocks + 1) / 2, lds_of(60), st);
-        return 16u << 16 | 60u;
-    }
+    const uint32_t build = tile_bin_build(a);
+    const size_t lds = tile_bin_lds(a, build & 0xffffu);
+    switch (build) {
+    case 8u << 16 | 256u: launch_tile_bin_shape<8, 256>(a, blocks, lds, st); break;
+    case 16u << 16 | 2048u: launch_tile_bin_shape<16, 2048>(a, (blocks + 1) / 2, lds, st); break;
+    case 16u << 16 | 1024u: launch_tile_bin_shape<16, 1024>(a, (blocks + 1) / 2, lds, st); break;
+    case 16u << 16 | 512u: launch_tile_bin_shape<16, 512>(a, (blocks + 1) / 2, lds, st); break;
+    case 16u << 16 | 256u: launch_tile_bin_shape<16, 256>(a, (blocks + 1) / 2, lds, st); break;
+    case 8u << 16 | 128u: launch_tile_bin_shape<8, 128>(a, blocks, lds, st); break;
+    default: launch_tile_bin_shape<16, 60>(a, (blocks + 1) / 2, lds, st); break;
+    }
+    return build;
 }
 
 constexpr uint32_t TEST_LOADS = 4;
 constexpr uint32_t TEST_GROUP = 32;
-template <uint32_t MODE, uint32_t DEPTH = 0, bool CARRY = false>
+template <uint32_t MODE, uint32_t DEPTH = 0, bool CARRY = false, bool PACK = false>
 __global__ void __launch_bounds__(1024) k_tile_test(TileArgs a) {
+    static_assert(!PACK || MODE == 0, "packed entries are a format of MODE 0");
     constexpr bool SLOTS = DEPTH != 0;
     static_assert(!SLOTS || MODE == 0, "the slots-only build is a build of MODE 0");
     constexpr uint32_t NSET = SLOTS ? 3 : 2;
@@ -2227,8 +2282,15 @@
     __shared__ uint32_t s_pref[NSET][TG + 1], s_first[NSET][TG], s_misc[NSET][2], s_kbase[2][TG], s_mask[2][TG];
     const uint32_t n_cols = a.n_leaves;
     auto col_of = [&](uint32_t li) { return li; };
-    __shared__ uint32_t s_failed[COUNTS ? 1 : (BLK ? (TG << (CL - 2)) : (TG << (CL - 5)))];
-    constexpr uint32_t N_FAILED = COUNTS ? 0 : (BLK ? (TG << (CL - 2)) : (TG << (CL - 5)));
+    constexpr uint32_t PACK_KEY_LOG2 = 12;
+    static_assert(PACK_ROUNDS * PACK_PAIRS == 1u << PACK_KEY_LOG2, "a key of the packed build is (round : 8, pair of the round : 4)");
+    constexpr uint32_t N_FAILED = COUNTS ? 0 : (BLK ? (TG << (CL - 2)) : (PACK ? (TG << (PACK_KEY_LOG2 - 5)) : (TG << (CL - 5))));
+    __shared__ uint32_t s_failed[COUNTS ? 1 : N_FAILED];
+    auto report_packed = [&](uint32_t set, uint32_t b, uint32_t rho, uint32_t e) {
+        const uint32_t id = e >> TL, fb = (b << PACK_KEY_LOG2) | (rho << 4) | id;
+        if (!(atomicOr(&s_failed[fb >> 5], 1u << (fb & 31u)) & (1u << (fb & 31u))))
+            a.round_fail[((uint64_t)(s_misc[set][1] + b) * PACK_ROUNDS + rho) * PACK_PAIRS + id] = 1;
+    };
     __shared__ uint32_t s_rk0[COUNTS ? TG : 1][RK];
     __shared__ unsigned long long s_base[NSET][TG];
     const uint32_t tile_words = TILE_BYTES / 4u;
@@ -2249,7 +2311,8 @@
         const bool mine = i < TG && c < n_chunks && (dsc = a.chunks[c], dsc.leaf == leaf);
         const bool usable = mine && dsc.cap != 0 && dsc.pass == a.pass;
         uint32_t fill = usable ? a.gfill[(uint64_t)c * a.n_tiles + t] : 0u;
-        if (fill > dsc.cap) fill = dsc.cap;
+        const uint32_t capw = PACK ? pack_bucket_words(dsc.cap) : dsc.cap;
+        if (fill > capw) fill = capw;
         uint32_t incl = fill;
         for (uint32_t sft = 1; sft < TG; sft <<= 1) {
             const uint32_t o = (uint32_t)__shfl_up((int)incl, (int)sft);
@@ -2266,6 +2329,7 @@
         if (i == 0) {
             s_pref[buf][0] = 0;
             s_misc[buf][0] = (uint32_t)__popcll(mm);
+            s_misc[buf][1] = g0;
         }
     };
     auto tile_loads = [&](uint32_t leaf, uint32_t t, uint2 (&v)[TV]) {
@@ -2413,6 +2477,15 @@
                             }
                         }
                     }
+                } else if (PACK) {
+                    if (!have[u]) continue;
+                    const uint32_t e5[5] = {ev[0] & 0xffffffu, (ev[0] >> 24) | ((ev[1] & 0xffffu) << 8), (ev[1] >> 16) | ((ev[2] & 0xffu) << 16), ev[2] >> 8,
+                                            ev[3] & 0xffffffu};
+#pragma unroll
+                    for (uint32_t c = 0; c < 5; ++c) {
+                        const uint32_t off = e5[c] & ((1u << TL) - 1u);
+                        if (!((s_tile[off >> 5] >> (off & 31u)) & 1u)) report_packed(buf, cidx[u] >> CL, ev[3] >> 24, e5[c]);
+                    }
                 } else {
 #pragma unroll
                     for (uint32_t c = 0; c < 4; ++c) {
@@ -2458,6 +2531,16 @@
                 const uint32_t w = pk[j] >> (8u * u);
                 if (!(w & 0x80u)) continue;
                 const uint32_t ev[4] = {en[j][u].x, en[j][u].y, en[j][u].z, en[j][u].w};
+                if constexpr (PACK) {
+                    const uint32_t e5[5] = {ev[0] & 0xffffffu, (ev[0] >> 24) | ((ev[1] & 0xffffu) << 8), (ev[1] >> 16) | ((ev[2] & 0xffu) << 16), ev[2] >> 8,
+                                            ev[3] & 0xffffffu};
+#pragma unroll
+                    for (uint32_t c = 0; c < 5; ++c) {
+                        const uint32_t off = e5[c] & ((1u << TL) - 1u);
+                        if (!((s_tile[off >> 5] >> (off & 31u)) & 1u)) report_packed(set, w & 31u, ev[3] >> 24, e5[c]);
+                    }
+                    continue;
+                }
 #pragma unroll
                 for (uint32_t c = 0; c < 4; ++c) {
                     const uint32_t off = ev[c] & ((1u << TL) - 1u);
@@ -2487,12 +2570,13 @@
             d.fill = a.gfill[(uint64_t)c * a.n_tiles + t];
             return d;
         };
-        auto describe_put = [&](uint32_t set, uint32_t leaf, uint32_t t, const Described &d) {
+        auto describe_put = [&](uint32_t set, uint32_t leaf, uint32_t t, uint32_t g, const Described &d) {
             const uint32_t i = threadIdx.x;
             const bool mine = d.in && d.leaf == leaf;
             const bool usable = mine && d.cap != 0 && d.pass == a.pass;
             uint32_t fill = usable ? d.fill : 0u;
-            if (fill > d.cap) fill = d.cap;
+            const uint32_t capw = PACK ? pack_bucket_words(d.cap) : d.cap;
+            if (fill > capw) fill = capw;
             uint32_t incl = fill;
             for (uint32_t sft = 1; sft < TG; sft <<= 1) {
                 const uint32_t o = (uint32_t)__shfl_up((int)incl, (int)sft);
@@ -2510,6 +2594,7 @@
             if (i == 0) {
                 s_pref[set][0] = 0;
                 s_misc[set][0] = (uint32_t)__popcll(mm);
+                s_misc[set][1] = g;
             }
         };
         auto unit_after = [&](uint64_t task, uint32_t g, bool more, uint64_t &ntask, uint32_t &ng) {
@@ -2528,12 +2613,12 @@
             uint2 v[TV];
             list_loads(leaf_of(task0), tile_of(task0), v);
             const Described d = describe_loads(tile_of(task0), g0);
-            if (threadIdx.x < 64) describe_put(d0, leaf_of(task0), tile_of(task0), d);
+            if (threadIdx.x < 64) describe_put(d0, leaf_of(task0), tile_of(task0), g0, d);
             list_store(v);
             __syncthreads();
             have1 = unit_after(task0, g0, s_misc[d0][0] == TG, task1, g1);
             const Described d1st = describe_loads(have1 ? tile_of(task1) : 0u, have1 ? g1 : 0u);
-            if (have1 && threadIdx.x < 64) describe_put(d1, leaf_of(task1), tile_of(task1), d1st);
+            if (have1 && threadIdx.x < 64) describe_put(d1, leaf_of(task1), tile_of(task1), g1, d1st);
             __syncthreads();
         }
         uint32_t total0 = s_pref[d0][TG];
@@ -2556,7 +2641,7 @@
                     issue(j, last ? d1 : d0, last ? j : s + DEPTH + j, last ? total1 : total0);
                 }
             }
-            if (have2 && threadIdx.x < 64) describe_put(d2, leaf_of(task2), tile_of(task2), dn);
+            if (have2 && threadIdx.x < 64) describe_put(d2, leaf_of(task2), tile_of(task2), g2, dn);
             __syncthreads();
             if (!have1) break;
             if (tile1) list_store(vn);
@@ -2639,9 +2724,12 @@
 void launch_tile_test(const TileArgs &a, int blocks, hipStream_t st) {
     static std::atomic<uint64_t> attr_done{0};
     const auto k_stream = k_tile_test<0, PFQ_STREAM_DEPTH, PFQ_STREAM_CARRY != 0>;
+    const auto k_packed = k_tile_test<0, 0, false, true>, k_stream_packed = k_tile_test<0, PFQ_STREAM_DEPTH, PFQ_STREAM_CARRY != 0, true>;
     if (first_on_device(attr_done)) {
         (void)hipFuncSetAttribute(reinterpret_cast<const void *>(k_tile_test<0>), hipFuncAttributeMaxDynamicSharedMemorySize, 150 * 1024);
         (void)hipFuncSetAttribute(reinterpret_cast<const void *>(k_stream), hipFuncAttributeMaxDynamicSharedMemorySize, 150 * 1024);
+        (void)hipFuncSetAttribute(reinterpret_cast<const void *>(k_packed), hipFuncAttributeMaxDynamicSharedMemorySize, 1 << (TILE_LOG2 - 3));
+        (void)hipFuncSetAttribute(reinterpret_cast<const void *>(k_stream_packed), hipFuncAttributeMaxDynamicSharedMemorySize, 1 << (TILE_LOG2 - 3));
         (void)hipFuncSetAttribute(reinterpret_cast<const void *>(k_tile_test<1>), hipFuncAttributeMaxDynamicSharedMemorySize, 1 << (TILE_LOG2_COUNTS - 3));
         (void)hipFuncSetAttribute(reinterpret_cast<const void *>(k_tile_test<2>), hipFuncAttributeMaxDynamicSharedMemorySize, 1 << TILE_LOG2_BLOCK);
         (void)hipFuncSetAttribute(reinterpret_cast<const void *>(k_tile_test<3>), hipFuncAttributeMaxDynamicSharedMemorySize, 1 << TILE_LOG2_BLOCK);
@@ -2650,8 +2738,26 @@
     if (a.counts && a.blocks) hipLaunchKernelGGL(k_tile_test<3>, g, b, (size_t)(1u << TILE_LOG2_BLOCK), st, a);
     else if (a.counts) hipLaunchKernelGGL(k_tile_test<1>, g, b, (size_t)(1u << (TILE_LOG2_COUNTS - 3)), st, a);
     else if (a.blocks) hipLaunchKernelGGL(k_tile_test<2>, g, b, (size_t)(1u << TILE_LOG2_BLOCK), st, a);
-    else if (a.tile_stream && a.tile_list_row && a.tile_lists) hipLaunchKernelGGL(k_stream, g, b, (size_t)(1u << (TILE_LOG2 - 3)), st, a);
+    else if (a.tile_stream && a.tile_list_row && a.tile_lists)
+        hipLaunchKernelGGL(a.entry_pack ? k_stream_packed : k_stream, g, b, (size_t)(1u << (TILE_LOG2 - 3)), st, a);
+    else if (a.entry_pack) hipLaunchKernelGGL(k_packed, g, b, (size_t)(1u << (TILE_LOG2 - 3)), st, a);
     else hipLaunchKernelGGL(k_tile_test<0>, g, b, (size_t)(1u << (TILE_LOG2 - 3)), st, a);
+}
+
+__global__ void __launch_bounds__(PACK_ROUNDS) k_pack_fail(TileArgs a) {
+    const uint32_t n_chunks = *a.n_chunks < a.max_chunks ? *a.n_chunks : a.max_chunks;
+    for (uint32_t c = blockIdx.x; c < n_chunks; c += gridDim.x) {
+        if (threadIdx.x >= a.n_rounds[c]) continue;
+        const uint64_t r = (uint64_t)c * PACK_ROUNDS + threadIdx.x;
+        const uint4 f = *reinterpret_cast<const uint4 *>(a.round_fail + r * PACK_PAIRS);
+        if (!(f.x | f.y | f.z | f.w)) continue;
+        const uint32_t at = a.chunks[c].first + a.round_p0[r], w[4] = {f.x, f.y, f.z, f.w};
+        for (uint32_t id = 0; id < PACK_PAIRS; ++id)
+            if ((w[id >> 2] >> (8u * (id & 3u))) & 0xffu) atomicOr(&a.fail[at + id], 1u);
+    }
+}
+void launch_pack_fail(const TileArgs &a, hipStream_t st) {
+    if (a.entry_pack) hipLaunchKernelGGL(k_pack_fail, dim3(1024), dim3(PACK_ROUNDS), 0, st, a);
 }
 
 __global__ void __launch_bounds__(256) k_collect_open(const uint32_t *fail, const uint32_t *n_pairs_ptr, uint32_t *list,
diff --git a/phagefilter_amd/query.py b/phagefilter_amd/query.py
--- a/phagefilter_amd/query.py
+++ b/phagefilter_amd/query.py
@@ -189,6 +189,16 @@
         out = np.zeros(self.TILE_LIST_CAP, dtype=np.uint32)
         _ffi.check(_ffi.lib().pfq_debug_tile_list(self._h, col, tile, out.ctypes.data, out.size))
         return out
+
+    TILE_BUCKET_WORDS = 1296
+
+    def tile_bucket(self, chunk: int, tile: int, max_words: int = 1 << 20) -> dict:
+        out = np.zeros(self.TILE_BUCKET_WORDS + max_words, dtype=np.uint32)
+        _ffi.check(_ffi.lib().pfq_debug_tile_bucket(self._h, chunk, tile, out.ctypes.data, out.size))
+        fill, cap, first, n, leaf, pas, packed, n_chunks, n_rounds = (int(v) for v in out[:9])
+        return dict(fill=fill, cap=cap, first=first, n=n, leaf=leaf, **{"pass": pas}, packed=bool(packed), n_chunks=n_chunks, n_rounds=n_rounds,
+                    round_p0=out[16:16 + n_rounds].astype(np.int64), reads=out[272:272 + n].astype(np.int64),
+                    words=out[self.TILE_BUCKET_WORDS:self.TILE_BUCKET_WORDS + min(fill, cap, max_words)].copy())
 
     def profile_begin(self, max_calls: int) -> None:
         _ffi.check(_ffi.lib().pfq_profile_begin(self._h, max_calls))
```
